# FrozenWolf-Cyber/Indic-CL-ASR

Measured on AMD Instinct MI355X. Metric: utterances/sec (15 s @16 kHz) Conformer-M RNNT-CTC+EWC train step, higher is better.
Workload: dtype bf16; 1 GPU; BASELINE configs[1]: Conformer-medium (d=256, 16L, H=640) hybrid RNNT-CTC + EWC, bs=32/GPU x 15 s, bf16 projections, freeze_encoder_till=12, 22x257 heads, fused_batch_size=4; global_batch=32, parallelism=dp1

## Files before the change

include/indicasr.h:

```cpp
#ifndef INDICASR_H
#define INDICASR_H

#include <stddef.h>
#include <stdint.h>

#ifdef __cplusplus
extern "C" {
#endif

typedef void* ia_stream_t;

enum ia_status {
    IA_OK = 0,
    IA_INVALID_VALUE = -1,
    IA_WORKSPACE_TOO_SMALL = -2,
    IA_LAUNCH_FAILED = -3,
    IA_UNSUPPORTED = -4,
};

const char* ia_version(void);

size_t ia_rnnt_workspace_bytes(int B, int T, int U1);
int ia_rnnt_loss(const float* logits, const int64_t* labels, const int64_t* act_lens, const int64_t* label_lens,
                 int B, int T, int U1, int V, int blank, float fastemit_lambda, float clamp,
// ... 76 lines not shown
int ia_quantize_mxfp8(const void* x, int is_f32, int ld, int64_t M, int K, void* q, int ldq, void* scales, int lds, ia_stream_t stream);
int ia_gemm_mxfp8(const void* Aq, int lda, const void* a_scales, int ldsa, const void* Wq, int ldw, const void* w_scales, int ldsw,
                  int M, int N, int K, const float* bias, int act, float dropout_p, unsigned seed, float alpha, const float* R, int ldr,
                  float* outF, int ldof, void* outH, int ldoh, ia_stream_t stream);

int ia_greedy_decode_lds_bytes(int Hp, int Hj, int V);
int ia_greedy_rnnt_decode(const float* f_all, const int64_t* out_len, const float* EW, const float* Whh, const float* Wpred,
                          const float* bpred, const float* Whead, const float* bhead, int B, int T, int Hp, int Hj, int V,
                          int blank, int row_blank, int row_sos, int max_symbols, int* tokens, int cap, int* counts,
                          int* overflow, ia_stream_t stream);
int ia_greedy_rnnt_decode_bf16w(const float* f_all, const int64_t* out_len, const float* EW, const void* Whh_bf16,
                                const void* Wpred_bf16, const float* bpred, const void* Whead_bf16, const float* bhead, int B, int T,
                                int Hp, int Hj, int V, int blank, int row_blank, int row_sos, int max_symbols, int* tokens, int cap,
                                int* counts, int* overflow, ia_stream_t stream);
size_t ia_greedy_decode_scratch_bytes(int B, int Hp, int Hj);
int ia_greedy_decode_cluster(int B, int Hp, int Hj);
int ia_greedy_rnnt_decode_bf16w_ex(const float* f_all, const int64_t* out_len, const float* EW, const void* Whh_bf16,
                                   const void* Wpred_bf16, const float* bpred, const void* Whead_bf16, const float* bhead, int B,
                                   int T, int Hp, int Hj, int V, int blank, int row_blank, int row_sos, int max_symbols, int* tokens,
                                   int cap, int* counts, int* overflow, int cluster, void* scratch, size_t scratch_bytes,
                                   ia_stream_t stream);

int ia_edit_distance_batch(const int32_t* a, const int64_t* a_off, const int32_t* b, const int64_t* b_off, int n, int64_t* out);

int ia_quantize_fp8_rows(const void* x, int is_f32, int ld, int64_t M, int K, void* q, int ldq, float* scale, ia_stream_t stream);
int ia_gemm_fp8(const void* Aq, int lda, const float* a_scale, const void* Wq, int ldw, const float* w_scale, int M, int N, int K,
                const float* bias, int act, float dropout_p, unsigned seed, float alpha, const float* R, int ldr, float* outF,
                int ldof, void* outH, int ldoh, ia_stream_t stream);
int ia_subsample_conv1(const float* feats, int B, int Fm, int Tm, int C, const float* w1, const float* b1, void* out,
                       ia_stream_t stream);
int ia_subsample_conv2(const void* in_cl, int B, int T1, int F1, int C, const void* w2r, const float* b2, int N, void* out,
                       ia_stream_t stream);
int ia_gemm_bf16_ln_supported(int N, int K);
int ia_gemm_bf16_ln(const void* A, int lda, const void* W, int ldw, int M, int N, int K, const float* bias, float dropout_p,
                    unsigned seed, float alpha, const float* R, int ldr, float* outF, int ldof, const float* ln_g,
                    const float* ln_b, float ln_eps, void* outH, int ldoh, ia_stream_t stream);
int ia_layernorm(const float* x, int ldx, int N, int d, const float* g1, const float* b1, float eps, float* outF,
                 int ldf, const float* g2, const float* b2, void* outH, int ldh, ia_stream_t stream);
int ia_glu_dwconv(const void* x2, const int64_t* lens, int B, int T, int d, int ksz, const float* w, const float* bias,
                  float* z, float* bn_sum, float* bn_sumsq, float* scratch, ia_stream_t stream);
int64_t ia_dwconv_scratch_elems(int B, int T, int d, int ksz);
int ia_colsum_bf16(const void* x, int M, int N, int ld, float* out, ia_stream_t stream);
int ia_dwconv_time(const float* x, int B, int T, int d, int ksz, const float* w, const float* bias, int flip, float* y,
                   ia_stream_t stream);
int ia_dwconv_time_wgrad(const float* x, const float* dy, int B, int T, int d, int ksz, float* dw, float* db,
                         float* scratch, ia_stream_t stream);
int ia_dwconv_glu_bwd(const float* dz, const void* c2, const int64_t* lens, int B, int T, int d, int ksz, const float* w, void* dc2,
                      ia_stream_t stream);
int ia_dwconv_glu_wgrad(const void* c2, const int64_t* lens, const float* dy, int B, int T, int d, int ksz, float* dw, float* db,
                        float* scratch, ia_stream_t stream);
int ia_bn_silu(const float* z, int64_t n_rows, int d, const float* bn_sum, const float* bn_sumsq, const float* gamma,
               const float* beta, float* running_mean, float* running_var, int64_t* num_batches_tracked,
               float momentum, float eps, int training, void* out, ia_stream_t stream);

int ia_gemm_bnsilu_supported(int K);
int ia_gemm_bnsilu_bf16(const float* z, int ldz, int64_t n_rows, const float* bn_sum, const float* bn_sumsq,
                        const float* gamma, const float* beta, float* running_mean, float* running_var,
                        int64_t* num_batches_tracked, float momentum, float eps, int training, const void* W, int ldw, int M,
                        int N, int K, const float* bias, float dropout_p, unsigned seed, float alpha, const float* R, int ldr,
                        float* outF, int ldof, void* outH, int ldoh, const long long* bn_sums_fixed, ia_stream_t stream);
int ia_gemm_bnsilu_bf16_keep(const float* z, int ldz, int64_t n_rows, const float* bn_sum, const float* bn_sumsq,
                             const float* gamma, const float* beta, float* running_mean, float* running_var,
                             int64_t* num_batches_tracked, float momentum, float eps, int training, const void* W, int ldw, int M,
                             int N, int K, const float* bias, float dropout_p, unsigned seed, float alpha, const float* R, int ldr,
                             float* outF, int ldof, void* outH, int ldoh, const long long* bn_sums_fixed, void* outA, int ldoa,
                             ia_stream_t stream);
int ia_dwconv_gated_fixed(const void* g, const int64_t* lens, int B, int T, int d, int ksz, const float* w, const float* bias,
                          float* z, long long* bn_sums_fixed, ia_stream_t stream);
int ia_glu_dwconv_fixed(const void* x2, const int64_t* lens, int B, int T, int d, int ksz, const float* w, const float* bias,
                        float* z, long long* bn_sums_fixed, ia_stream_t stream);

int ia_relpos_attention_flash_supported(int T, int dk);
int ia_relpos_attention_flash(const void* qkv, const void* pos_proj, const float* bias_u, const float* bias_v,
                              const int64_t* lens, int B, int T, int H, int dk, float dropout_p, unsigned seed, void* ctx,
                              ia_stream_t stream);
int ia_relpos_attention_flash_lse(const void* qkv, const void* pos_proj, const float* bias_u, const float* bias_v,
                                  const int64_t* lens, int B, int T, int H, int dk, float dropout_p, unsigned seed, void* ctx,
                                  float* lse, ia_stream_t stream);
int ia_relpos_attention_local_supported(int T, int dk, int window);
int ia_relpos_attention_local(const void* qkv, const void* pos_proj, const float* bias_u, const float* bias_v,
                              const int64_t* lens, int B, int T, int H, int dk, int window, float dropout_p, unsigned seed,
                              void* ctx, ia_stream_t stream);
int ia_relpos_attention_local_lse(const void* qkv, const void* pos_proj, const float* bias_u, const float* bias_v,
                                  const int64_t* lens, int B, int T, int H, int dk, int window, float dropout_p, unsigned seed,
                                  void* ctx, float* lse, ia_stream_t stream);
int ia_relpos_attention_flash_bwd_dims(int T, int* Rs, int* pad0);
int64_t ia_relpos_attention_flash_bwd_ws_elems(int B, int T, int H, int dk);
int ia_relpos_attention_flash_bwd(const void* qkv, const void* pos_proj, const float* bias_u, const float* bias_v,
                                  const int64_t* lens, const void* ctx, const void* dctx, const float* lse, int B, int T, int H,
                                  int dk, float dropout_p, unsigned seed, void* dqkv, void* dpl, int pl_rows, float* dbias_u,
                                  float* dbias_v, void* dBand, void* QvHM, float* ws, ia_stream_t stream);
int ia_relpos_attention_local_bwd_dims(int T, int window, int* Rs, int* pad0);
int64_t ia_relpos_attention_local_bwd_ws_elems(int B, int T, int H, int dk, int window);
int ia_relpos_attention_local_bwd(const void* qkv, const void* pos_proj, const float* bias_u, const float* bias_v,
                                  const int64_t* lens, const void* ctx, const void* dctx, const float* lse, int B, int T, int H,
                                  int dk, int window, float dropout_p, unsigned seed, void* dqkv, void* dpl, int pl_rows,
                                  float* dbias_u, float* dbias_v, void* dBand, void* QvHM, float* ws, ia_stream_t stream);
int ia_relpos_attention_context_supported(int T, int dk, int style, int left, int right);
int ia_relpos_attention_context(const void* qkv, const void* pos_proj, const float* bias_u, const float* bias_v,
                                const int64_t* lens, int B, int T, int H, int dk, int style, int left, int right,
                                float dropout_p, unsigned seed, void* ctx, ia_stream_t stream);
int ia_relpos_attention_context_lse(const void* qkv, const void* pos_proj, const float* bias_u, const float* bias_v,
                                    const int64_t* lens, int B, int T, int H, int dk, int style, int left, int right,
                                    float dropout_p, unsigned seed, void* ctx, float* lse, ia_stream_t stream);
int ia_relpos_attention_context_bwd_dims(int T, int style, int left, int right, int* Rs, int* pad0);
int64_t ia_relpos_attention_context_bwd_ws_elems(int B, int T, int H, int dk, int style, int left, int right);
int ia_relpos_attention_context_bwd(const void* qkv, const void* pos_proj, const float* bias_u, const float* bias_v,
                                    const int64_t* lens, const void* ctx, const void* dctx, const float* lse, int B, int T, int H,
                                    int dk, int style, int left, int right, float dropout_p, unsigned seed, void* dqkv, void* dpl,
                                    int pl_rows, float* dbias_u, float* dbias_v, void* dBand, void* QvHM, float* ws,
                                    ia_stream_t stream);
size_t ia_attn_vt_elems(int B, int T, int H);
int ia_relpos_attention(const void* qkv, const void* pos_proj, const float* bias_u, const float* bias_v,
                        const int64_t* lens, int B, int T, int H, int dk, float dropout_p, unsigned seed,
                        void* vt_scratch, void* ctx, ia_stream_t stream);

size_t ia_lstm_scratch_bytes(int B, int H);
int ia_lstm_lds_bytes(int H, int backward);
int ia_lstm_forward(const float* Gx, const void* Whh_bf16, float* Hout, float* gates, float* Cs, int U, int B, int H,
                    void* scratch, size_t scratch_bytes, ia_stream_t stream);
int ia_lstm_backward(const float* dHout, const float* gates, const float* Cs, const void* WhhT_bf16, float* dG, int U,
                     int B, int H, void* scratch, size_t scratch_bytes, ia_stream_t stream);

int ia_feat_frames(const float* audio, int B, int L, int Tm, int win, int n_fft, int hop, float preemph, float dither,
                   unsigned seed, float* frames, int ldf, ia_stream_t stream);
int ia_gemm_f32(const float* A, int lda, const float* W, int ldw, int M, int N, int K, float* C, int ldc,
                ia_stream_t stream);
int ia_feat_power(const float* spec, int64_t M, int lds, int half, int nbins, float* power, int ldp, ia_stream_t stream);
int ia_feat_logmel_t(const float* mel, int B, int Tm, int F, int ldm, float guard, float* out, ia_stream_t stream);
int ia_feat_preemph(const float* audio, int B, int L, float preemph, float dither, unsigned seed, float* y,
                    ia_stream_t stream);
int ia_feat_logmel_fft_supported(int n_fft, int win, int n_mels, int n_chunks);
int ia_feat_logmel_fft(const float* y, int B, int L, int Tm, const float* window, int win, int n_fft, int hop,
                       const float* twiddle, const int* chunk_start, const float* chunk_vals, const int* filt_chunks,
                       int n_mels, int n_chunks, float guard, float* out, ia_stream_t stream);
int ia_feat_normalize(const float* x, const int64_t* seq_len, int B, int F, int T, float eps, const int* freq_starts,
                      const int* freq_widths, int n_freq_masks, const int* time_starts, const int* time_widths,
                      int n_time_masks, float mask_value, float* y, ia_stream_t stream);

size_t ia_ctc_workspace_bytes(int B, int T, int S);
int ia_ctc_forward(const float* log_probs, const int64_t* targets, const int64_t* input_lens, const int64_t* target_lens,
                   int B, int T, int V, int S, int blank, int zero_infinity, float* nll, void* workspace,
                   size_t workspace_bytes, ia_stream_t stream);
int ia_ctc_backward(const float* log_probs, const int64_t* targets, const int64_t* input_lens, const int64_t* target_lens,
                    int B, int T, int V, int S, int blank, const float* nll_grad, float* grad, void* workspace,
                    size_t workspace_bytes, ia_stream_t stream);

typedef struct ia_tn_problem {
    const void* dY; const void* X; float* dW; float* db;
    int ldy, ldx, M, n, k;
} ia_tn_problem;
int64_t ia_gemm_tn_grouped_scratch_elems(const ia_tn_problem* problems, int count);
int ia_gemm_tn_bf16_grouped(const ia_tn_problem* problems, int count, float* scratch, ia_stream_t stream);
int64_t ia_gemm_tn_scratch_elems(int M, int n, int k);
int ia_gemm_tn_bf16(const void* dY, int ldy, const void* X, int ldx, int M, int n, int k, float* dW, float* db,
                    float* scratch, ia_stream_t stream);

int ia_ffn_fused_supported(int d, int d_ff);
int ia_ffn_fused(float* x, int N, int d, int d_ff, const float* ln_g, const float* ln_b, float eps, const void* W1,
                 const float* b1, const void* W2, const float* b2, float alpha, float p_ff, unsigned seed_ff, float p_res,
                 unsigned seed_res, const float* ln2_g, const float* ln2_b, void* y_out, int ln2_to_y_only,
                 ia_stream_t stream);
int ia_ffn_fused_tail_supported(int d, int d_ff, int nt);
int ia_ffn_fused_tail(float* x, int N, int d, int d_ff, const float* ln_g, const float* ln_b, float eps, const void* W1,
                      const float* b1, const void* W2, const float* b2, float alpha, float p_ff, unsigned seed_ff, float p_res,
                      unsigned seed_res, const float* ln2_g, const float* ln2_b, void* y_out, int ln2_to_y_only, const void* Wt,
                      const float* bt, void* t_out, int nt, ia_stream_t stream);

typedef struct ia_block_params {
    const void *w_ff1a, *w_ff1b, *w_qkv, *w_pos, *w_out, *w_pw1, *w_pw2, *w_ff2a, *w_ff2b;
    const float *b_ff1a, *b_ff1b, *b_qkv, *b_out, *b_pw1, *b_pw2, *b_ff2a, *b_ff2b;
    const float *ln_ff1_g, *ln_ff1_b, *ln_att_g, *ln_att_b, *ln_conv_g, *ln_conv_b, *ln_ff2_g, *ln_ff2_b, *ln_out_g, *ln_out_b;
    const float *pos_u, *pos_v, *dw_w, *dw_b, *bn_g, *bn_b;
    float *bn_rm, *bn_rv;
    int64_t* bn_nbt;
    float ln_eps, bn_eps, bn_momentum, p_drop, p_ff, p_att, fc_factor;
    int d, d_ff, n_heads, ksz;
    const void* pl_cached;
    const void* w_pw1_glu;
    const float* b_pw1_glu;
    int att_window;
    int att_style;
    int att_left, att_right;
} ia_block_params;
size_t ia_conformer_prefix_ws_bytes(int B, int T, int d, int d_ff, int H, int ksz, int pos_rows);
int ia_conformer_prefix_fwd(const ia_block_params* layers, int n_layers, float* x, const void* pos_emb, int pos_rows,
                            const int64_t* lens, int B, int T, unsigned seed_base, unsigned seed_stride, int training,
                            void* workspace, size_t workspace_bytes, ia_stream_t stream);
size_t ia_conformer_prefix_ws_sums_offset(int B, int T, int d, int d_ff, int H, int ksz, int pos_rows);
int ia_conformer_prefix_fwd_seg(const ia_block_params* layers, int n_layers, float* x, const void* pos_emb, int pos_rows,
                                const int64_t* lens, int B, int T, unsigned seed_base, unsigned seed_stride, int training,
                                int seg_begin, int seg_end, int bn_synced, void* workspace, size_t workspace_bytes,
                                ia_stream_t stream);

typedef struct ia_block_saved {
    void *y1, *h1p, *h1; float* x1;
    void *y2, *qkv, *pl, *ctxv; float* x2;
    void *y3, *c2; float *z, *sums; void* c3; float* x3;
    void *y4, *h4p, *h4; float* x4;
    float* lse;
} ia_block_saved;
typedef struct ia_block_grads {
    float *w_ff1a, *b_ff1a, *w_ff1b, *b_ff1b, *w_qkv, *b_qkv, *w_pos, *w_out, *b_out, *w_pw1, *b_pw1, *w_pw2, *b_pw2;
    float *w_ff2a, *b_ff2a, *w_ff2b, *b_ff2b;
    float *ln_ff1_g, *ln_ff1_b, *ln_att_g, *ln_att_b, *ln_conv_g, *ln_conv_b, *ln_ff2_g, *ln_ff2_b, *ln_out_g, *ln_out_b;
    float *dw_w, *dw_b, *bn_g, *bn_b;
} ia_block_grads;
struct ia_block_params;
int ia_conformer_block_supported(int d, int d_ff, int H, int ksz, int T);
size_t ia_conformer_block_bwd_ws_bytes(int B, int T, int d, int d_ff, int ksz);
int ia_conformer_block_fwd(const struct ia_block_params* layer, const float* x0, const void* pos_emb, int pos_rows,
                           const int64_t* lens, int B, int T, unsigned seed, const ia_block_saved* saved, float* out,
                           float* dw_scratch, ia_stream_t stream);
int ia_conformer_block_bwd_a(const struct ia_block_params* layer, const ia_block_saved* saved, const ia_block_grads* grads,
                             const float* dout, const int64_t* lens, int B, int T, unsigned seed, void* workspace,
                             size_t workspace_bytes, float** dx2_out, void** dctx_out, ia_stream_t stream);
int ia_conformer_block_fwd_phase(const struct ia_block_params* layer, const float* x0, const void* pos_emb, int pos_rows,
                                 const int64_t* lens, int B, int T, unsigned seed, const ia_block_saved* saved, float* out,
                                 float* dw_scratch, int phase, ia_stream_t stream);
int ia_conformer_block_bwd_a_phase(const struct ia_block_params* layer, const ia_block_saved* saved, const ia_block_grads* grads,
                                   const float* dout, const int64_t* lens, int B, int T, unsigned seed, void* workspace,
                                   size_t workspace_bytes, float** dx2_out, void** dctx_out, int phase, const float* bn_S12,
                                   ia_stream_t stream);
int ia_conformer_block_bwd_b(const struct ia_block_params* layer, const ia_block_saved* saved, const ia_block_grads* grads,
                             const float* x0, const void* pos_emb, int pos_rows, const void* dqkv, const void* dpl, int B,
                             int T, unsigned seed, void* workspace, size_t workspace_bytes, float* dx0,
                             const void* add_table, int n_add, ia_stream_t stream);

int ia_layernorm_bwd(const float* x, int ldx, const float* dy_f32, const void* dy_bf16, int ldy, int N, int d,
                     const float* gamma, float eps, const float* dx_in, float* dx_out, int lddx, float* dgamma,
                     float* dbeta, float* scratch, ia_stream_t stream);
int ia_layernorm_bwd_drop(const float* x, int ldx, const float* dy_f32, const void* dy_bf16, int ldy, int N, int d,
                          const float* gamma, float eps, const float* dx_in, float* dx_out, int lddx, float* dgamma,
                          float* dbeta, float alpha, float dropout_p, unsigned seed, void* dx_bf16, int lddxh, float* scratch,
                          ia_stream_t stream);
typedef struct ia_finish_job { const float* part; int G, C, C0; float* out0; float* out1; } ia_finish_job;
int ia_layernorm_bwd_partial_rows(int N);
int ia_partials_finish_multi(const ia_finish_job* jobs, int count, ia_stream_t stream);
int64_t ia_layernorm_bwd_scratch_elems(int N, int d);
int ia_silu_dropout(const void* h_pre, int64_t M, int N, float dropout_p, unsigned seed, void* out, ia_stream_t stream);
int ia_silu_dropout_bwd(const void* h_pre, const void* dh, int64_t M, int N, float dropout_p, unsigned seed, void* out,
                        ia_stream_t stream);
int ia_scale_dropout_bf16(const float* dy, int64_t M, int N, float alpha, float dropout_p, unsigned seed, void* out,
                          ia_stream_t stream);
int ia_cast_pad_bf16(const float* src, int lds, int64_t M, int N, void* dst, int ldd, ia_stream_t stream);
int ia_bn_silu_bwd(const float* z, const void* dc3, int64_t n_rows, int d, const float* bn_sum, const float* bn_sumsq,
                   const float* gamma, const float* beta, float eps, float* S1, float* S2, float* dz, float* scratch,
                   ia_stream_t stream);
int64_t ia_bn_silu_bwd_scratch_elems(int64_t n_rows, int d);
int ia_bn_sync_finish(float* sums_and_count, int d, int64_t n_local_rows, float* running_mean, float* running_var,
                      int64_t* num_batches_tracked, float momentum, ia_stream_t stream);
int ia_bn_silu_bwd_reduce(const float* z, const void* dc3, int64_t n_rows, int d, const float* bn_sum, const float* bn_sumsq,
                          const float* gamma, const float* beta, float eps, float* S1, float* S2, float* scratch,
                          ia_stream_t stream);
int ia_bn_silu_bwd_apply(const float* z, const void* dc3, int64_t n_rows, int d, const float* bn_sum, const float* bn_sumsq,
                         const float* gamma, const float* beta, float eps, const float* S1, const float* S2, float* dz,
                         ia_stream_t stream);
int ia_glu_mask(const void* c2, const int64_t* lens, int B, int T, int d, float* G, ia_stream_t stream);
int ia_glu_bwd(const void* c2, const float* dG, const int64_t* lens, int B, int T, int d, void* dc2, ia_stream_t stream);

int ia_cl_chunk_elems(void);
int ia_cl_penalty(const float* theta, const float* theta_star, const float* weight, float coef, float* grad,
                  int accumulate, const int32_t* chunk_table, int nchunks, const float* seg_inv_numel,
                  float* seg_abs_mean, float* penalty_sum, ia_stream_t stream);
int ia_cl_fisher_accumulate(float* fisher, const float* grad, const float* loss_scalar, int64_t n, ia_stream_t stream);
int ia_cl_abs_accumulate(float* omega, const float* grad, int64_t n, ia_stream_t stream);
int ia_adamw_step(float* theta, const float* grad, float* exp_avg, float* exp_avg_sq, int64_t n, float lr, float beta1,
                  float beta2, float eps, float weight_decay, int step, float grad_scale, void* shadow_bf16,
                  ia_stream_t stream);
int ia_adamw_step_segmented(float* theta, const float* grad, float* exp_avg, float* exp_avg_sq, const int32_t* chunk_table,
                            int nchunks, int32_t* seg_active, int32_t* seg_step, int nseg, int all_active, float lr,
                            float beta1, float beta2, float eps, float weight_decay, float grad_scale, void* shadow_bf16,
                            ia_stream_t stream);
size_t ia_grad_norm_workspace_bytes(int nchunks);
int ia_grad_norm(const float* grad, const int32_t* chunk_table, int nchunks, const int32_t* seg_chunk_begin, int nseg,
                 float grad_scale, float max_norm, int32_t* seg_active, float* seg_norm, float* norm_state, void* workspace,
                 size_t workspace_bytes, ia_stream_t stream);
int ia_adamw_step_segmented_clipped(float* theta, const float* grad, float* exp_avg, float* exp_avg_sq,
                                    const int32_t* chunk_table, int nchunks, int32_t* seg_active, int32_t* seg_step, int nseg,
                                    int all_active, float lr, float beta1, float beta2, float eps, float weight_decay,
                                    float grad_scale, void* shadow_bf16, const float* norm_state, int skip_nonfinite,
                                    int32_t* counters, ia_stream_t stream);
int ia_adamw_step_segmented_si(float* theta, const float* grad, float* exp_avg, float* exp_avg_sq, const int32_t* chunk_table,
                               int nchunks, int32_t* seg_active, int32_t* seg_step, int nseg, int all_active, float lr,
                               float beta1, float beta2, float eps, float weight_decay, float grad_scale, void* shadow_bf16,
                               const float* norm_state, int skip_nonfinite, int32_t* counters, float* path_w,
                               const float* omega, const float* theta_star, float penalty_coef, ia_stream_t stream);
int ia_si_consolidate(const float* theta, float* theta_star, float* path_w, float* omega, float xi, int64_t n,
                      ia_stream_t stream);
size_t ia_agem_workspace_bytes(int nchunks);
int ia_agem_dots(const float* grad, const float* ref, const int32_t* chunk_table, int nchunks, int nseg, float grad_scale,
                 int32_t* seg_active, float* proj_state, void* workspace, size_t workspace_bytes, ia_stream_t stream);
int ia_grad_norm_projected(const float* grad, const int32_t* chunk_table, int nchunks, const int32_t* seg_chunk_begin, int nseg,
                           float grad_scale, float max_norm, const int32_t* seg_active, float* seg_norm, float* norm_state,
                           void* workspace, size_t workspace_bytes, const float* ref, const float* proj_state,
                           ia_stream_t stream);
int ia_adamw_step_segmented_projected(float* theta, const float* grad, float* exp_avg, float* exp_avg_sq,
                                      const int32_t* chunk_table, int nchunks, int32_t* seg_active, int32_t* seg_step, int nseg,
                                      int all_active, float lr, float beta1, float beta2, float eps, float weight_decay,
                                      float grad_scale, void* shadow_bf16, const float* norm_state, int skip_nonfinite,
                                      int32_t* counters, const float* ref, const float* proj_state, int32_t* proj_counters,
                                      ia_stream_t stream);
#define IA_GEM_MAX_TASKS 16
#define IA_GEM_STATE_FLOATS 20
#define IA_GEM_SUMS_DOUBLES 272
size_t ia_gem_workspace_bytes(int nchunks, int max_tasks);
int ia_gem_dots(const float* x, const float* refs, int64_t stride, int ntasks, const int32_t* chunk_table, int nchunks, int nseg,
                float grad_scale, int32_t* seg_active, int gram_row, double* gem_sums, void* workspace, size_t workspace_bytes,
                ia_stream_t stream);
int ia_gem_solve(const double* gem_sums, float* gem_state, int ntasks, float memory_strength, float eps, ia_stream_t stream);
int ia_grad_norm_gem(const float* grad, const int32_t* chunk_table, int nchunks, const int32_t* seg_chunk_begin, int nseg,
                     float grad_scale, float max_norm, const int32_t* seg_active, float* seg_norm, float* norm_state,
                     void* workspace, size_t workspace_bytes, const float* refs, int64_t stride, int ntasks,
                     const float* gem_state, ia_stream_t stream);
int ia_adamw_step_segmented_gem(float* theta, const float* grad, float* exp_avg, float* exp_avg_sq, const int32_t* chunk_table,
                                int nchunks, int32_t* seg_active, int32_t* seg_step, int nseg, int all_active, float beta1,
                                float beta2, float eps, float grad_scale, void* shadow_bf16, const int32_t* seg_group, int ngroups,
                                const float* group_lr, const float* group_weight_decay, const float* norm_state,
                                int skip_nonfinite, int32_t* counters, const float* refs, int64_t stride, int ntasks,
                                const float* gem_state, int32_t* gem_counters, ia_stream_t stream);
#define IA_MAX_PARAM_GROUPS 64
int ia_adamw_step_segmented_grouped(float* theta, const float* grad, float* exp_avg, float* exp_avg_sq,
                                    const int32_t* chunk_table, int nchunks, int32_t* seg_active, int32_t* seg_step, int nseg,
                                    int all_active, float beta1, float beta2, float eps, float grad_scale, void* shadow_bf16,
                                    const int32_t* seg_group, int ngroups, const float* group_lr,
                                    const float* group_weight_decay, const float* norm_state, int skip_nonfinite,
                                    int32_t* counters, float* path_w, const float* omega, const float* theta_star,
                                    float penalty_coef, const float* ref, const float* proj_state, int32_t* proj_counters,
                                    ia_stream_t stream);
#define IA_MASK_FREE 0
#define IA_MASK_MASKED 1
#define IA_MASK_FROZEN 2
int ia_adamw_step_segmented_masked(float* theta, const float* grad, float* exp_avg, float* exp_avg_sq, const int32_t* chunk_table,
                                   int nchunks, int32_t* seg_active, int32_t* seg_step, int nseg, int all_active, float beta1,
                                   float beta2, float eps, float grad_scale, void* shadow_bf16, const int32_t* seg_group,
                                   int ngroups, const float* group_lr, const float* group_weight_decay, const float* norm_state,
                                   int skip_nonfinite, int32_t* counters, const float* base, float* scores,
                                   const int32_t* seg_kind, float threshold, ia_stream_t stream);
int ia_mask_pack(const float* scores, const int32_t* chunk_table, int nchunks, const int32_t* seg_kind, int nseg, float threshold,
                 uint64_t* bits, int64_t nwords, int32_t* seg_kept, ia_stream_t stream);
int ia_mask_apply(float* theta, const float* base, const uint64_t* bits, int64_t nwords, const int32_t* chunk_table, int nchunks,
                  const int32_t* seg_kind, int nseg, void* shadow_bf16, ia_stream_t stream);
int ia_adamw_step_segmented_packed(float* theta, const float* grad, float* exp_avg, float* exp_avg_sq, const int32_t* chunk_table,
                                   int nchunks, int32_t* seg_active, int32_t* seg_step, int nseg, int all_active, float beta1,
                                   float beta2, float eps, float grad_scale, void* shadow_bf16, const int32_t* seg_group,
                                   int ngroups, const float* group_lr, const float* group_weight_decay, const float* norm_state,
                                   int skip_nonfinite, int32_t* counters, const uint8_t* owner, const int32_t* seg_kind,
                                   int train_owner, ia_stream_t stream);
int ia_grad_norm_packed(const float* grad, const int32_t* chunk_table, int nchunks, const int32_t* seg_chunk_begin, int nseg,
                        float grad_scale, float max_norm, int32_t* seg_active, float* seg_norm, float* norm_state,
                        void* workspace, size_t workspace_bytes, const uint8_t* owner, const int32_t* seg_kind, int train_owner,
                        ia_stream_t stream);
size_t ia_pack_prune_workspace_bytes(int nseg);
int ia_pack_prune(float* theta, float* exp_avg, float* exp_avg_sq, uint8_t* owner, const int32_t* chunk_table, int nchunks,
                  const int32_t* seg_kind, int nseg, float fraction, int task, void* shadow_bf16, int32_t* seg_counts,
                  void* workspace, size_t workspace_bytes, ia_stream_t stream);
int ia_pack_apply(float* theta, const float* base, const uint8_t* owner, const int32_t* chunk_table, int nchunks,
                  const int32_t* seg_kind, int nseg, int lo, int hi, void* shadow_bf16, ia_stream_t stream);
#define IA_LORA_MAX_RANK 64
int ia_lora_tile_rows(void);
int ia_lora_tile_cols(void);
size_t ia_lora_workspace_bytes(int64_t m, int64_t n, int rank);
int ia_lora_grad(const float* grad, const float* factors, float* factor_grad, const int64_t* tensors, int ntensors,
                 const int32_t* tiles, int ntiles, const int32_t* factor_chunk_table, int nfchunks, int rank, float scale,
                 float grad_scale, const float* norm_state, int skip_nonfinite, int all_active, int32_t* factor_active,
                 void* workspace, size_t workspace_bytes, size_t workspace_needed, ia_stream_t stream);
int ia_lora_apply(float* theta, const float* base, const float* factors, const int64_t* tensors, int ntensors,
                  const int32_t* seg_tensor, const int32_t* chunk_table, int nchunks, int nseg, int rank, float scale,
                  void* shadow_bf16, const float* norm_state, int skip_nonfinite, ia_stream_t stream);
int ia_adamw_step_segmented_kinds(float* theta, const float* grad, float* exp_avg, float* exp_avg_sq, const int32_t* chunk_table,
                                  int nchunks, int32_t* seg_active, int32_t* seg_step, int nseg, int all_active, float beta1,
                                  float beta2, float eps, float grad_scale, void* shadow_bf16, const int32_t* seg_group,
                                  int ngroups, const float* group_lr, const float* group_weight_decay, const float* norm_state,
                                  int skip_nonfinite, int32_t* counters, const int32_t* seg_kind, int flags_preset,
                                  ia_stream_t stream);
#define IA_MERGE_MAX_TASKS 32
int ia_merge_linear(float* theta, const float* base, const float* vectors, int64_t stride, int ntasks, const float* coef,
                    float scale, const int32_t* chunk_table, int nchunks, void* shadow_bf16, ia_stream_t stream);
size_t ia_merge_trim_workspace_bytes(int ntasks, int nscope);
int ia_merge_trim(const float* vectors, int64_t stride, int ntasks, const int32_t* chunk_table, int nchunks,
// ... 70 lines not shown
```

indic_cl_asr_amd/_lib.py:

```python
import ctypes
import os
import subprocess

_HERE = os.path.dirname(os.path.abspath(__file__))
LIB_PATH = os.environ.get("IA_LIB_PATH") or os.path.join(_HERE, "libindicasr_hip.so")

IA_OK = 0
_STATUS = {-1: "IA_INVALID_VALUE", -2: "IA_WORKSPACE_TOO_SMALL", -3: "IA_LAUNCH_FAILED", -4: "IA_UNSUPPORTED"}

_c = ctypes
_vp, _i, _f, _sz = _c.c_void_p, _c.c_int, _c.c_float, _c.c_size_t
_i64 = _c.c_int64

class BlockParams(_c.Structure):
    _fields_ = ([(n, _c.c_void_p) for n in (
        "w_ff1a", "w_ff1b", "w_qkv", "w_pos", "w_out", "w_pw1", "w_pw2", "w_ff2a", "w_ff2b",
        "b_ff1a", "b_ff1b", "b_qkv", "b_out", "b_pw1", "b_pw2", "b_ff2a", "b_ff2b",
        "ln_ff1_g", "ln_ff1_b", "ln_att_g", "ln_att_b", "ln_conv_g", "ln_conv_b", "ln_ff2_g", "ln_ff2_b", "ln_out_g", "ln_out_b",
        "pos_u", "pos_v", "dw_w", "dw_b", "bn_g", "bn_b", "bn_rm", "bn_rv", "bn_nbt")]
        + [(n, _c.c_float) for n in ("ln_eps", "bn_eps", "bn_momentum", "p_drop", "p_ff", "p_att", "fc_factor")]
        + [(n, _c.c_int) for n in ("d", "d_ff", "n_heads", "ksz")]
        + [("pl_cached", _c.c_void_p), ("w_pw1_glu", _c.c_void_p), ("b_pw1_glu", _c.c_void_p), ("att_window", _c.c_int),
           ("att_style", _c.c_int), ("att_left", _c.c_int), ("att_right", _c.c_int)])


class BlockSaved(_c.Structure):
    _fields_ = [(n, _c.c_void_p) for n in ("y1", "h1p", "h1", "x1", "y2", "qkv", "pl", "ctxv", "x2", "y3", "c2", "z", "sums",
                                           "c3", "x3", "y4", "h4p", "h4", "x4", "lse")]


class TnProblem(_c.Structure):
    _fields_ = [("dY", _c.c_void_p), ("X", _c.c_void_p), ("dW", _c.c_void_p), ("db", _c.c_void_p),
                ("ldy", _c.c_int), ("ldx", _c.c_int), ("M", _c.c_int), ("n", _c.c_int), ("k", _c.c_int)]


class BlockGrads(_c.Structure):
    _fields_ = [(n, _c.c_void_p) for n in (
        "w_ff1a", "b_ff1a", "w_ff1b", "b_ff1b", "w_qkv", "b_qkv", "w_pos", "w_out", "b_out", "w_pw1", "b_pw1", "w_pw2", "b_pw2",
        "w_ff2a", "b_ff2a", "w_ff2b", "b_ff2b",
        "ln_ff1_g", "ln_ff1_b", "ln_att_g", "ln_att_b", "ln_conv_g", "ln_conv_b", "ln_ff2_g", "ln_ff2_b", "ln_out_g", "ln_out_b",
        "dw_w", "dw_b", "bn_g", "bn_b")]


class WaveParams(_c.Structure):
    _fields_ = ([(n, _c.c_int32) for n in ("n_in", "n_out", "new_sr", "shift_pre", "shift_post", "noise_shift", "noise_stage")]
                + [("noise_seed", _c.c_uint32), ("gain", _c.c_float), ("noise_amp", _c.c_float), ("pad", _c.c_int32 * 2)])


SIGNATURES = {
    "ia_version": (_c.c_char_p, []),
    "ia_wave_augment_tile": (_i, []),
    "ia_wave_augment": (_i, [_vp, _i, _i, _vp, _i, _vp, _vp, _i, _i, _i, _vp]),
    "ia_gemm_bf16_ex2": (_i, [_vp, _i, _vp, _i, _i, _i, _i, _vp, _i, _f, _c.c_uint, _f, _vp, _i, _vp, _i, _vp, _i, _vp, _i, _vp, _i, _i, _vp]),
    "ia_transpose16_multi": (_i, [_vp, _i, _vp]),
    "ia_swap01_cast": (_i, [_vp, _i, _i, _i, _i, _vp, _i, _vp]),
    "ia_ctc_row_lse": (_i, [_vp, _i, _i64, _i, _vp, _vp]),
    "ia_ctc_forward_logits": (_i, [_vp, _i, _vp, _vp, _vp, _vp, _i, _i, _i, _i, _i, _i, _vp, _vp, _sz, _vp]),
    "ia_ctc_backward_logits": (_i, [_vp, _i, _vp, _vp, _vp, _vp, _i, _i, _i, _i, _i, _vp, _f, _vp, _i, _vp, _sz, _vp]),
    "ia_select_rows_cast": (_i, [_vp, _i, _vp, _i, _i, _i, _i, _i, _f, _i, _vp, _vp, _i, _vp, _vp]),
    "ia_rows_scatter_add": (_i, [_vp, _i, _vp, _i, _i, _i, _i, _i, _f, _vp, _vp, _vp]),
    "ia_loss_combine": (_i, [_vp, _vp, _i, _f, _vp, _vp, _vp, _vp, _vp, _vp, _vp]),
    "ia_loss_combine_bwd": (_i, [_vp, _i, _f, _vp, _vp, _vp]),
    "ia_embed_sos": (_i, [_vp, _vp, _i, _i, _i, _i, _i, _i, _vp, _vp]),
    "ia_embed_sos_bwd": (_i, [_vp, _i, _vp, _i, _i, _i, _i, _i, _i, _f, _vp, _vp]),
    "ia_multi_axpy": (_i, [_vp, _i, _i, _vp]),
    "ia_peak_stream_copy": (_i, [_vp, _vp, _sz, _vp]),
    "ia_peak_mfma_bf16": (_i, [_vp, _i, _i, _vp]),
    "ia_peak_mfma_bf16_flops": (_c.c_double, [_i, _i]),
    "ia_rnnt_workspace_bytes": (_sz, [_i, _i, _i]),
    "ia_rnnt_loss": (_i, [_vp, _vp, _vp, _vp, _i, _i, _i, _i, _i, _f, _f, _vp, _vp, _vp, _sz, _vp]),
    "ia_rnnt_forward": (_i, [_vp, _vp, _vp, _vp, _i, _i, _i, _i, _i, _f, _i, _vp, _vp, _sz, _vp]),
    "ia_rnnt_backward": (_i, [_vp, _vp, _vp, _vp, _i, _i, _i, _i, _i, _f, _f, _vp, _vp, _vp, _sz, _vp, _vp, _vp]),
    "ia_rnnt_export_alphas_betas": (_i, [_vp, _sz, _vp, _vp, _i, _i, _i, _vp, _vp, _vp]),
    "ia_joint_ld": (_i, [_i]),
    "ia_joint_fwd": (_i, [_vp, _vp, _vp, _vp, _vp, _vp, _vp, _i, _i, _i, _i, _i, _i, _f, _c.c_uint, _vp, _i, _vp, _sz, _vp]),
    "ia_joint_fwd_box": (_i, [_vp, _vp, _vp, _vp, _vp, _vp, _vp, _vp, _vp, _i, _i, _i, _i, _i, _i, _f, _c.c_uint, _vp, _i, _vp, _sz, _vp]),
    "ia_joint_extra_scratch_elems": (_i64, []),
    "ia_joint_extra_reduce": (_i, [_vp, _vp, _vp, _vp, _vp, _vp, _i, _i, _i, _i, _i, _vp, _vp, _vp]),
    "ia_joint_extra_grad": (_i, [_vp, _vp, _vp, _vp, _vp, _vp, _vp, _i, _i, _i, _i, _i, _vp, _vp]),
    "ia_lattice_add_f16": (_i, [_vp, _vp, _i64, _vp]),
    "ia_relpos_attention_flash_lse": (_i, [_vp, _vp, _vp, _vp, _vp, _i, _i, _i, _i, _f, _c.c_uint, _vp, _vp, _vp]),
    "ia_relpos_attention_flash_bwd_dims": (_i, [_i, _c.POINTER(_c.c_int), _c.POINTER(_c.c_int)]),
    "ia_relpos_attention_flash_bwd_ws_elems": (_i64, [_i, _i, _i, _i]),
    "ia_relpos_attention_flash_bwd": (_i, [_vp, _vp, _vp, _vp, _vp, _vp, _vp, _vp, _i, _i, _i, _i, _f, _c.c_uint, _vp, _vp, _i, _vp,
                                           _vp, _vp, _vp, _vp, _vp]),
    "ia_relpos_attention_local_lse": (_i, [_vp, _vp, _vp, _vp, _vp, _i, _i, _i, _i, _i, _f, _c.c_uint, _vp, _vp, _vp]),
    "ia_relpos_attention_local_bwd_dims": (_i, [_i, _i, _c.POINTER(_c.c_int), _c.POINTER(_c.c_int)]),
    "ia_relpos_attention_local_bwd_ws_elems": (_i64, [_i, _i, _i, _i, _i]),
    "ia_relpos_attention_local_bwd": (_i, [_vp, _vp, _vp, _vp, _vp, _vp, _vp, _vp, _i, _i, _i, _i, _i, _f, _c.c_uint, _vp, _vp, _i, _vp,
                                           _vp, _vp, _vp, _vp, _vp]),
    "ia_relpos_attention_context_lse": (_i, [_vp, _vp, _vp, _vp, _vp, _i, _i, _i, _i, _i, _i, _i, _f, _c.c_uint, _vp, _vp, _vp]),
    "ia_relpos_attention_context_bwd_dims": (_i, [_i, _i, _i, _i, _c.POINTER(_c.c_int), _c.POINTER(_c.c_int)]),
    "ia_relpos_attention_context_bwd_ws_elems": (_i64, [_i, _i, _i, _i, _i, _i, _i]),
    "ia_relpos_attention_context_bwd": (_i, [_vp, _vp, _vp, _vp, _vp, _vp, _vp, _vp, _i, _i, _i, _i, _i, _i, _i, _f, _c.c_uint, _vp, _vp,
                                             _i, _vp, _vp, _vp, _vp, _vp, _vp]),
    "ia_quantize_fp8_rows": (_i, [_vp, _i, _i, _i64, _i, _vp, _i, _vp, _vp]),
    "ia_gemm_fp8": (_i, [_vp, _i, _vp, _vp, _i, _vp, _i, _i, _i, _vp, _i, _f, _c.c_uint, _f, _vp, _i, _vp, _i, _vp, _i, _vp]),
    "ia_gemm_tn_grouped_scratch_elems": (_i64, [_vp, _i]),
    "ia_gemm_tn_bf16_grouped": (_i, [_vp, _i, _vp, _vp]),
    "ia_greedy_decode_lds_bytes": (_i, [_i, _i, _i]),
    "ia_greedy_rnnt_decode": (_i, [_vp, _vp, _vp, _vp, _vp, _vp, _vp, _vp, _i, _i, _i, _i, _i, _i, _i, _i, _i, _vp, _i, _vp, _vp, _vp]),
    "ia_greedy_rnnt_decode_bf16w": (_i, [_vp, _vp, _vp, _vp, _vp, _vp, _vp, _vp, _i, _i, _i, _i, _i, _i, _i, _i, _i, _vp, _i, _vp, _vp, _vp]),
    "ia_edit_distance_batch": (_i, [_vp, _vp, _vp, _vp, _i, _vp]),
    "ia_greedy_decode_scratch_bytes": (_sz, [_i, _i, _i]),
    "ia_greedy_decode_cluster": (_i, [_i, _i, _i]),
    "ia_greedy_rnnt_decode_bf16w_ex": (_i, [_vp, _vp, _vp, _vp, _vp, _vp, _vp, _vp, _i, _i, _i, _i, _i, _i, _i, _i, _i, _vp, _i, _vp, _vp, _i, _vp, _sz, _vp]),
    "ia_quantize_mxfp8": (_i, [_vp, _i, _i, _i64, _i, _vp, _i, _vp, _i, _vp]),
    "ia_gemm_mxfp8": (_i, [_vp, _i, _vp, _i, _vp, _i, _vp, _i, _i, _i, _i, _vp, _i, _f, _c.c_uint, _f, _vp, _i, _vp, _i, _vp, _i, _vp]),
    "ia_cast_pad_bf16": (_i, [_vp, _i, _i64, _i, _vp, _i, _vp]),
    "ia_rnnt_lattice": (_i, [_vp, _vp, _i, _i, _i, _f, _i, _vp, _vp, _sz, _vp]),
    "ia_joint_backward_g": (_i, [_vp, _vp, _vp, _vp, _i, _i, _i, _i, _i, _i, _f, _vp, _f, _vp, _i, _i, _vp, _vp, _vp, _sz, _vp, _vp,
                                 _vp]),
    "ia_joint_backward_g_skip": (_i, [_vp, _vp, _vp, _vp, _i, _i, _i, _i, _i, _i, _f, _vp, _f, _vp, _i, _i, _vp, _vp, _vp, _sz, _i, _vp,
                                      _vp, _vp]),
    "ia_joint_backward_g_dbias_scratch_elems": (_i64, [_i]),
    "ia_joint_hidden_t": (_i, [_vp, _vp, _vp, _i, _i, _i, _i, _i, _i, _i, _f, _c.c_uint, _vp]),
    "ia_joint_hidden": (_i, [_vp, _vp, _vp, _i, _i, _i, _i, _i, _f, _c.c_uint, _vp]),
    "ia_joint_dh_reduce": (_i, [_vp, _vp, _vp, _vp, _vp, _vp, _vp, _i, _i, _i, _i, _f, _f, _c.c_uint, _vp, _vp]),
    "ia_joint_dh_reduce_scratch_bytes": (_sz, [_i, _i, _i, _i]),
    "ia_joint_dh_fused_supported": (_i, [_i, _i, _i]),
    "ia_joint_dh_k": (_i, []),
    "ia_joint_dh_fused": (_i, [_vp, _vp, _vp, _vp, _vp, _vp, _vp, _vp, _i, _i, _i, _i, _i, _f, _f, _c.c_uint, _vp, _vp]),
    "ia_joint_dh_fused_ex": (_i, [_vp, _vp, _vp, _vp, _vp, _vp, _vp, _vp, _vp, _vp, _i, _i, _i, _i, _i, _i, _f, _f, _c.c_uint, _vp, _vp]),
    "ia_joint_dh_fused_scratch_bytes": (_sz, [_i, _i, _i, _i]),
    "ia_joint_dw_fused_supported": (_i, [_i, _i, _i]),
    "ia_joint_dw_fused_scratch_elems": (_i64, [_i, _i, _i, _i, _i]),
    "ia_joint_dw_fused": (_i, [_vp, _vp, _vp, _vp, _i, _i, _i, _i, _i, _f, _c.c_uint, _vp, _vp, _vp]),
    "ia_gemm_bf16_ln_supported": (_i, [_i, _i]),
    "ia_gemm_bf16_ln": (_i, [_vp, _i, _vp, _i, _i, _i, _i, _vp, _f, _c.c_uint, _f, _vp, _i, _vp, _i, _vp, _vp, _f, _vp, _i, _vp]),
    "ia_joint_dw_fused_ex": (_i, [_vp, _vp, _vp, _vp, _vp, _i, _i, _i, _i, _i, _f, _c.c_uint, _vp, _vp, _vp]),
    "ia_gemm_bf16": (_i, [_vp, _i, _vp, _i, _i, _i, _i, _vp, _i, _f, _c.c_uint, _f, _vp, _i, _vp, _i, _vp, _i, _vp]),
    "ia_gemm_bf16_ex": (_i, [_vp, _i, _vp, _i, _i, _i, _i, _vp, _i, _f, _c.c_uint, _f, _vp, _i, _vp, _i, _vp, _i, _vp, _i, _vp, _i, _vp]),
    "ia_subsample_conv1": (_i, [_vp, _i, _i, _i, _i, _vp, _vp, _vp, _vp]),
    "ia_subsample_conv2": (_i, [_vp, _i, _i, _i, _i, _vp, _vp, _i, _vp, _vp]),
    "ia_layernorm": (_i, [_vp, _i, _i, _i, _vp, _vp, _f, _vp, _i, _vp, _vp, _vp, _i, _vp]),
    "ia_glu_dwconv": (_i, [_vp, _vp, _i, _i, _i, _i, _vp, _vp, _vp, _vp, _vp, _vp, _vp]),
    "ia_dwconv_scratch_elems": (_i64, [_i, _i, _i, _i]),
    "ia_colsum_bf16": (_i, [_vp, _i, _i, _i, _vp, _vp]),
    "ia_dwconv_time": (_i, [_vp, _i, _i, _i, _i, _vp, _vp, _i, _vp, _vp]),
    "ia_dwconv_time_wgrad": (_i, [_vp, _vp, _i, _i, _i, _i, _vp, _vp, _vp, _vp]),
    "ia_dwconv_glu_bwd": (_i, [_vp, _vp, _vp, _i, _i, _i, _i, _vp, _vp, _vp]),
    "ia_dwconv_glu_wgrad": (_i, [_vp, _vp, _vp, _i, _i, _i, _i, _vp, _vp, _vp, _vp]),
    "ia_bn_silu": (_i, [_vp, _i64, _i, _vp, _vp, _vp, _vp, _vp, _vp, _vp, _f, _f, _i, _vp, _vp]),
    "ia_gemm_bnsilu_supported": (_i, [_i]),
    "ia_gemm_bnsilu_bf16": (_i, [_vp, _i, _i64, _vp, _vp, _vp, _vp, _vp, _vp, _vp, _f, _f, _i, _vp, _i, _i, _i, _i, _vp, _f, _c.c_uint, _f,
                                 _vp, _i, _vp, _i, _vp, _i, _vp, _vp]),
    "ia_gemm_bnsilu_bf16_keep": (_i, [_vp, _i, _i64, _vp, _vp, _vp, _vp, _vp, _vp, _vp, _f, _f, _i, _vp, _i, _i, _i, _i, _vp, _f, _c.c_uint,
                                      _f, _vp, _i, _vp, _i, _vp, _i, _vp, _vp, _i, _vp]),
    "ia_glu_dwconv_fixed": (_i, [_vp, _vp, _i, _i, _i, _i, _vp, _vp, _vp, _vp, _vp]),
    "ia_dwconv_gated_fixed": (_i, [_vp, _vp, _i, _i, _i, _i, _vp, _vp, _vp, _vp, _vp]),
    "ia_attn_vt_elems": (_sz, [_i, _i, _i]),
    "ia_relpos_attention": (_i, [_vp, _vp, _vp, _vp, _vp, _i, _i, _i, _i, _f, _c.c_uint, _vp, _vp, _vp]),
    "ia_relpos_attention_flash_supported": (_i, [_i, _i]),
    "ia_relpos_attention_flash": (_i, [_vp, _vp, _vp, _vp, _vp, _i, _i, _i, _i, _f, _c.c_uint, _vp, _vp]),
    "ia_relpos_attention_local_supported": (_i, [_i, _i, _i]),
    "ia_relpos_attention_context_supported": (_i, [_i, _i, _i, _i, _i]),
    "ia_relpos_attention_context": (_i, [_vp, _vp, _vp, _vp, _vp, _i, _i, _i, _i, _i, _i, _i, _f, _c.c_uint, _vp, _vp]),
    "ia_relpos_attention_local": (_i, [_vp, _vp, _vp, _vp, _vp, _i, _i, _i, _i, _i, _f, _c.c_uint, _vp, _vp]),
    "ia_lstm_scratch_bytes": (_sz, [_i, _i]),
    "ia_lstm_lds_bytes": (_i, [_i, _i]),
    "ia_lstm_forward": (_i, [_vp, _vp, _vp, _vp, _vp, _i, _i, _i, _vp, _sz, _vp]),
    "ia_lstm_backward": (_i, [_vp, _vp, _vp, _vp, _vp, _i, _i, _i, _vp, _sz, _vp]),
    "ia_feat_frames": (_i, [_vp, _i, _i, _i, _i, _i, _i, _f, _f, _c.c_uint, _vp, _i, _vp]),
    "ia_gemm_f32": (_i, [_vp, _i, _vp, _i, _i, _i, _i, _vp, _i, _vp]),
    "ia_feat_power": (_i, [_vp, _i64, _i, _i, _i, _vp, _i, _vp]),
    "ia_feat_logmel_t": (_i, [_vp, _i, _i, _i, _i, _f, _vp, _vp]),
    "ia_feat_preemph": (_i, [_vp, _i, _i, _f, _f, _c.c_uint, _vp, _vp]),
    "ia_feat_logmel_fft_supported": (_i, [_i, _i, _i, _i]),
    "ia_feat_logmel_fft": (_i, [_vp, _i, _i, _i, _vp, _i, _i, _i, _vp, _vp, _vp, _vp, _i, _i, _f, _vp, _vp]),
    "ia_feat_normalize": (_i, [_vp, _vp, _i, _i, _i, _f, _vp, _vp, _i, _vp, _vp, _i, _f, _vp, _vp]),
    "ia_ctc_workspace_bytes": (_sz, [_i, _i, _i]),
    "ia_ctc_forward": (_i, [_vp, _vp, _vp, _vp, _i, _i, _i, _i, _i, _i, _vp, _vp, _sz, _vp]),
    "ia_ctc_backward": (_i, [_vp, _vp, _vp, _vp, _i, _i, _i, _i, _i, _vp, _vp, _vp, _sz, _vp]),
    "ia_ctc_align_max_targets": (_i, []),
    "ia_ctc_align_workspace_bytes": (_sz, [_i, _i, _i]),
    "ia_ctc_align": (_i, [_vp, _i, _vp, _vp, _vp, _vp, _i, _i, _i, _i, _i, _vp, _vp, _vp, _vp, _sz, _vp]),
    "ia_gemm_tn_scratch_elems": (_i64, [_i, _i, _i]),
    "ia_gemm_tn_bf16": (_i, [_vp, _i, _vp, _i, _i, _i, _i, _vp, _vp, _vp, _vp]),
    "ia_ffn_fused_supported": (_i, [_i, _i]),
    "ia_ffn_fused": (_i, [_vp, _i, _i, _i, _vp, _vp, _f, _vp, _vp, _vp, _vp, _f, _f, _c.c_uint, _f, _c.c_uint, _vp, _vp, _vp, _i, _vp]),
    "ia_ffn_fused_tail_supported": (_i, [_i, _i, _i]),
    "ia_ffn_fused_tail": (_i, [_vp, _i, _i, _i, _vp, _vp, _f, _vp, _vp, _vp, _vp, _f, _f, _c.c_uint, _f, _c.c_uint, _vp, _vp, _vp, _i,
                               _vp, _vp, _vp, _i, _vp]),
    "ia_conformer_prefix_ws_bytes": (_sz, [_i, _i, _i, _i, _i, _i, _i]),
    "ia_conformer_prefix_ws_sums_offset": (_sz, [_i, _i, _i, _i, _i, _i, _i]),
    "ia_conformer_prefix_fwd_seg": (_i, [_vp, _i, _vp, _vp, _i, _vp, _i, _i, _c.c_uint, _c.c_uint, _i, _i, _i, _i, _vp, _sz, _vp]),
    "ia_conformer_prefix_fwd": (_i, [_vp, _i, _vp, _vp, _i, _vp, _i, _i, _c.c_uint, _c.c_uint, _i, _vp, _sz, _vp]),
    "ia_conformer_block_supported": (_i, [_i, _i, _i, _i, _i]),
    "ia_conformer_block_bwd_ws_bytes": (_sz, [_i, _i, _i, _i, _i]),
    "ia_conformer_block_fwd": (_i, [_vp, _vp, _vp, _i, _vp, _i, _i, _c.c_uint, _vp, _vp, _vp, _vp]),
    "ia_conformer_block_fwd_phase": (_i, [_vp, _vp, _vp, _i, _vp, _i, _i, _c.c_uint, _vp, _vp, _vp, _i, _vp]),
    "ia_conformer_block_bwd_a": (_i, [_vp, _vp, _vp, _vp, _vp, _i, _i, _c.c_uint, _vp, _sz, _vp, _vp, _vp]),
    "ia_conformer_block_bwd_a_phase": (_i, [_vp, _vp, _vp, _vp, _vp, _i, _i, _c.c_uint, _vp, _sz, _vp, _vp, _i, _vp, _vp]),
    "ia_conformer_block_bwd_b": (_i, [_vp, _vp, _vp, _vp, _vp, _i, _vp, _vp, _i, _i, _c.c_uint, _vp, _sz, _vp, _vp, _i, _vp]),
    "ia_layernorm_bwd": (_i, [_vp, _i, _vp, _vp, _i, _i, _i, _vp, _f, _vp, _vp, _i, _vp, _vp, _vp, _vp]),
    "ia_layernorm_bwd_drop": (_i, [_vp, _i, _vp, _vp, _i, _i, _i, _vp, _f, _vp, _vp, _i, _vp, _vp, _f, _f, _c.c_uint, _vp, _i, _vp, _vp]),
    "ia_layernorm_bwd_partial_rows": (_i, [_i]),
    "ia_partials_finish_multi": (_i, [_vp, _i, _vp]),
    "ia_layernorm_bwd_scratch_elems": (_i64, [_i, _i]),
    "ia_silu_dropout": (_i, [_vp, _i64, _i, _f, _c.c_uint, _vp, _vp]),
    "ia_silu_dropout_bwd": (_i, [_vp, _vp, _i64, _i, _f, _c.c_uint, _vp, _vp]),
    "ia_scale_dropout_bf16": (_i, [_vp, _i64, _i, _f, _f, _c.c_uint, _vp, _vp]),
    "ia_bn_silu_bwd": (_i, [_vp, _vp, _i64, _i, _vp, _vp, _vp, _vp, _f, _vp, _vp, _vp, _vp, _vp]),
    "ia_bn_silu_bwd_scratch_elems": (_i64, [_i64, _i]),
    "ia_bn_sync_finish": (_i, [_vp, _i, _i64, _vp, _vp, _vp, _f, _vp]),
    "ia_bn_silu_bwd_reduce": (_i, [_vp, _vp, _i64, _i, _vp, _vp, _vp, _vp, _f, _vp, _vp, _vp, _vp]),
    "ia_bn_silu_bwd_apply": (_i, [_vp, _vp, _i64, _i, _vp, _vp, _vp, _vp, _f, _vp, _vp, _vp, _vp]),
    "ia_glu_mask": (_i, [_vp, _vp, _i, _i, _i, _vp, _vp]),
    "ia_glu_bwd": (_i, [_vp, _vp, _vp, _i, _i, _i, _vp, _vp]),
    "ia_cl_chunk_elems": (_i, []),
    "ia_cl_penalty": (_i, [_vp, _vp, _vp, _f, _vp, _i, _vp, _i, _vp, _vp, _vp, _vp]),
    "ia_cl_fisher_accumulate": (_i, [_vp, _vp, _vp, _i64, _vp]),
    "ia_cl_abs_accumulate": (_i, [_vp, _vp, _i64, _vp]),
    "ia_adamw_step": (_i, [_vp, _vp, _vp, _vp, _i64, _f, _f, _f, _f, _f, _i, _f, _vp, _vp]),
    "ia_adamw_step_segmented": (_i, [_vp, _vp, _vp, _vp, _vp, _i, _vp, _vp, _i, _i, _f, _f, _f, _f, _f, _f, _vp, _vp]),
    "ia_grad_norm_workspace_bytes": (_sz, [_i]),
    "ia_grad_norm": (_i, [_vp, _vp, _i, _vp, _i, _f, _f, _vp, _vp, _vp, _vp, _sz, _vp]),
    "ia_adamw_step_segmented_clipped": (_i, [_vp, _vp, _vp, _vp, _vp, _i, _vp, _vp, _i, _i, _f, _f, _f, _f, _f, _f, _vp, _vp, _i,
                                             _vp, _vp]),
    "ia_adamw_step_segmented_si": (_i, [_vp, _vp, _vp, _vp, _vp, _i, _vp, _vp, _i, _i, _f, _f, _f, _f, _f, _f, _vp, _vp, _i,
                                        _vp, _vp, _vp, _vp, _f, _vp]),
    "ia_si_consolidate": (_i, [_vp, _vp, _vp, _vp, _f, _i64, _vp]),
    "ia_agem_workspace_bytes": (_sz, [_i]),
    "ia_agem_dots": (_i, [_vp, _vp, _vp, _i, _i, _f, _vp, _vp, _vp, _sz, _vp]),
    "ia_grad_norm_projected": (_i, [_vp, _vp, _i, _vp, _i, _f, _f, _vp, _vp, _vp, _vp, _sz, _vp, _vp, _vp]),
    "ia_adamw_step_segmented_projected": (_i, [_vp, _vp, _vp, _vp, _vp, _i, _vp, _vp, _i, _i, _f, _f, _f, _f, _f, _f, _vp, _vp, _i,
                                               _vp, _vp, _vp, _vp, _vp]),
    "ia_gem_workspace_bytes": (_sz, [_i, _i]),
    "ia_gem_dots": (_i, [_vp, _vp, _i64, _i, _vp, _i, _i, _f, _vp, _i, _vp, _vp, _sz, _vp]),
    "ia_gem_solve": (_i, [_vp, _vp, _i, _f, _f, _vp]),
    "ia_grad_norm_gem": (_i, [_vp, _vp, _i, _vp, _i, _f, _f, _vp, _vp, _vp, _vp, _sz, _vp, _i64, _i, _vp, _vp]),
    "ia_adamw_step_segmented_gem": (_i, [_vp, _vp, _vp, _vp, _vp, _i, _vp, _vp, _i, _i, _f, _f, _f, _f, _vp, _vp, _i, _vp, _vp,
                                         _vp, _i, _vp, _vp, _i64, _i, _vp, _vp, _vp]),
    "ia_adamw_step_segmented_grouped": (_i, [_vp, _vp, _vp, _vp, _vp, _i, _vp, _vp, _i, _i, _f, _f, _f, _f, _vp, _vp, _i, _vp, _vp,
                                             _vp, _i, _vp, _vp, _vp, _vp, _f, _vp, _vp, _vp, _vp]),
    "ia_adamw_step_segmented_masked": (_i, [_vp, _vp, _vp, _vp, _vp, _i, _vp, _vp, _i, _i, _f, _f, _f, _f, _vp, _vp, _i, _vp, _vp,
                                            _vp, _i, _vp, _vp, _vp, _vp, _f, _vp]),
    "ia_mask_pack": (_i, [_vp, _vp, _i, _vp, _i, _f, _vp, _i64, _vp, _vp]),
    "ia_mask_apply": (_i, [_vp, _vp, _vp, _i64, _vp, _i, _vp, _i, _vp, _vp]),
    "ia_adamw_step_segmented_packed": (_i, [_vp, _vp, _vp, _vp, _vp, _i, _vp, _vp, _i, _i, _f, _f, _f, _f, _vp, _vp, _i, _vp, _vp,
                                            _vp, _i, _vp, _vp, _vp, _i, _vp]),
    "ia_grad_norm_packed": (_i, [_vp, _vp, _i, _vp, _i, _f, _f, _vp, _vp, _vp, _vp, _sz, _vp, _vp, _i, _vp]),
    "ia_pack_prune_workspace_bytes": (_sz, [_i]),
    "ia_pack_prune": (_i, [_vp, _vp, _vp, _vp, _vp, _i, _vp, _i, _f, _i, _vp, _vp, _vp, _sz, _vp]),
    "ia_pack_apply": (_i, [_vp, _vp, _vp, _vp, _i, _vp, _i, _i, _i, _vp, _vp]),
    "ia_lora_tile_rows": (_i, []),
    "ia_lora_tile_cols": (_i, []),
    "ia_lora_workspace_bytes": (_sz, [_i64, _i64, _i]),
    "ia_lora_grad": (_i, [_vp, _vp, _vp, _vp, _i, _vp, _i, _vp, _i, _i, _f, _f, _vp, _i, _i, _vp, _vp, _sz, _sz, _vp]),
    "ia_lora_apply": (_i, [_vp, _vp, _vp, _vp, _i, _vp, _vp, _i, _i, _i, _f, _vp, _vp, _i, _vp]),
    "ia_adamw_step_segmented_kinds": (_i, [_vp, _vp, _vp, _vp, _vp, _i, _vp, _vp, _i, _i, _f, _f, _f, _f, _vp, _vp, _i, _vp, _vp,
                                           _vp, _i, _vp, _vp, _i, _vp]),
    "ia_merge_linear": (_i, [_vp, _vp, _vp, _i64, _i, _vp, _f, _vp, _i, _vp, _vp]),
    "ia_merge_trim_workspace_bytes": (_sz, [_i, _i]),
    "ia_merge_trim": (_i, [_vp, _i64, _i, _vp, _i, _vp, _i, _f, _vp, _vp, _sz, _vp]),
    "ia_merge_ties": (_i, [_vp, _vp, _vp, _i64, _i, _vp, _vp, _i, _f, _vp, _i, _i, _vp, _vp, _vp]),
    "ia_merge_fisher": (_i, [_vp, _vp, _vp, _vp, _i64, _i, _vp, _f, _f, _vp, _i, _i, _vp, _vp, _vp]),
    "ia_merge_linear_dare": (_i, [_vp, _vp, _vp, _i64, _i, _vp, _f, _vp, _i, _vp, _c.c_uint32, _c.c_uint32, _f, _vp]),
    "ia_merge_ties_dare": (_i, [_vp, _vp, _vp, _i64, _i, _f, _vp, _i, _i, _vp, _vp, _c.c_uint32, _c.c_uint32, _f, _vp]),
}

_lib = None


def build(verbose=False):
    out = None if verbose else subprocess.DEVNULL
    subprocess.check_call(["make", "-C", os.path.join(_HERE, "csrc")], stdout=out)


def lib():
    global _lib
    if _lib is None:
        if not os.path.exists(LIB_PATH):
            raise RuntimeError(
                f"{LIB_PATH} is missing: the HIP extension is the product path and has no fallback. "
                "Build it with `python -c 'import __graft_entry__ as g; g.build()'` or `make -C indic_cl_asr_amd/csrc`.")
        import torch
        l = ctypes.CDLL(LIB_PATH)
        for name, (res, args) in SIGNATURES.items():
            fn = getattr(l, name)
            fn.restype, fn.argtypes = res, args
        _lib = l
    return _lib


def check(status, what):
    if status != IA_OK:
        raise RuntimeError(f"{what} failed with status {status} ({_STATUS.get(status, 'unknown')})")


def version():
    return lib().ia_version().decode()


def stream_ptr():
    import torch
    return ctypes.c_void_p(torch.cuda.current_stream().cuda_stream)


def ptr(t):
    return ctypes.c_void_p(t.data_ptr()) if t is not None else None
```

indic_cl_asr_amd/csrc/block_train.hip:

```cpp
#include <hip/hip_bf16.h>
#include <hip/hip_runtime.h>

#include <cstdint>

#include <cstdlib>

#include "ia_common.h"

namespace {

inline size_t up256(size_t x) { return (x + 255) / 256 * 256; }

#define IA_TRY(call)                  \
    do {                              \
        const int rc_ = (call);       \
        if (rc_ != IA_OK) return rc_; \
    } while (0)

__global__ __launch_bounds__(256) void transpose_bf16_kernel(const unsigned short* __restrict__ in, int rows, int cols,
                                                             unsigned short* __restrict__ out) {
    __shared__ unsigned short tile[64][72];
    const int tiles_c = (cols + 63) / 64;
    const int tr = blockIdx.x / tiles_c, tc = blockIdx.x - tr * tiles_c;
    const int r0 = tr * 64, c0 = tc * 64;
    for (int i = threadIdx.x; i < 64 * 8; i += 256) {
        const int r = i >> 3, v = i & 7;
        uint4 x = make_uint4(0, 0, 0, 0);
        if (r0 + r < rows && c0 + v * 8 < cols) x = *reinterpret_cast<const uint4*>(in + (size_t)(r0 + r) * cols + c0 + v * 8);
        *reinterpret_cast<uint4*>(&tile[r][v * 8]) = x;
    }
    __syncthreads();
    for (int i = threadIdx.x; i < 64 * 8; i += 256) {
        const int c = i >> 3, v = i & 7;
        if (c0 + c < cols && r0 + v * 8 < rows) {
            union { uint4 u; unsigned short h[8]; } o;
#pragma unroll
            for (int j = 0; j < 8; ++j) o.h[j] = tile[v * 8 + j][c];
            *reinterpret_cast<uint4*>(out + (size_t)(c0 + c) * rows + r0 + v * 8) = o.u;
        }
    }
}

int transpose_bf16(const void* in, int rows, int cols, void* out, hipStream_t st) {
    if (rows % 8 != 0 || cols % 8 != 0) return IA_UNSUPPORTED;
    const int grid = ((rows + 63) / 64) * ((cols + 63) / 64);
    hipLaunchKernelGGL(transpose_bf16_kernel, dim3(grid), dim3(256), 0, st, (const unsigned short*)in, rows, cols, (unsigned short*)out);
    IA_RETURN_IF_LAUNCH_FAILED();
    return IA_OK;
}

struct TrJob { const unsigned short* in; unsigned short* out; int rows, cols, tile_begin, tiles_c; };
struct TrJobs { TrJob j[8]; int count; };
__global__ __launch_bounds__(256) void transpose_bf16_multi_kernel(TrJobs jobs) {
    __shared__ unsigned short tile[64][72];
    int ji = 0;
#pragma unroll
    for (int i = 1; i < 8; ++i)
        if (i < jobs.count && (int)blockIdx.x >= jobs.j[i].tile_begin) ji = i;
    const TrJob& J = jobs.j[ji];
    const int local = blockIdx.x - J.tile_begin;
    const int tr = local / J.tiles_c, tc = local - tr * J.tiles_c;
    const int r0 = tr * 64, c0 = tc * 64, rows = J.rows, cols = J.cols;
    for (int i = threadIdx.x; i < 64 * 8; i += 256) {
        const int r = i >> 3, v = i & 7;
        uint4 x = make_uint4(0, 0, 0, 0);
        if (r0 + r < rows && c0 + v * 8 < cols) x = *reinterpret_cast<const uint4*>(J.in + (size_t)(r0 + r) * cols + c0 + v * 8);
        *reinterpret_cast<uint4*>(&tile[r][v * 8]) = x;
    }
    __syncthreads();
    for (int i = threadIdx.x; i < 64 * 8; i += 256) {
        const int c = i >> 3, v = i & 7;
        if (c0 + c < cols && r0 + v * 8 < rows) {
            union { uint4 u; unsigned short h[8]; } o;
#pragma unroll
            for (int j = 0; j < 8; ++j) o.h[j] = tile[v * 8 + j][c];
            *reinterpret_cast<uint4*>(J.out + (size_t)(c0 + c) * rows + r0 + v * 8) = o.u;
        }
    }
}
struct TrList { TrJobs jobs; int tiles; };
inline void tr_add(TrList* l, const void* in, int rows, int cols, void* out) {
    TrJob& J = l->jobs.j[l->jobs.count++];
    J.in = (const unsigned short*)in; J.out = (unsigned short*)out; J.rows = rows; J.cols = cols;
    J.tile_begin = l->tiles; J.tiles_c = (cols + 63) / 64;
    l->tiles += ((rows + 63) / 64) * J.tiles_c;
}
int tr_launch(const TrList& l, hipStream_t st) {
    for (int i = 0; i < l.jobs.count; ++i)
        if (l.jobs.j[i].rows % 8 != 0 || l.jobs.j[i].cols % 8 != 0) return IA_UNSUPPORTED;
    hipLaunchKernelGGL(transpose_bf16_multi_kernel, dim3(l.tiles), dim3(256), 0, st, l.jobs);
    IA_RETURN_IF_LAUNCH_FAILED();
    return IA_OK;
}

struct AddRow { float* dst; const float* src; int64_t n; };
__global__ __launch_bounds__(256) void multi_add_kernel(const AddRow* __restrict__ table, int rows) {
    for (int k = blockIdx.y; k < rows; k += gridDim.y) {
        const AddRow r = table[k];
        const int64_t n4 = ((reinterpret_cast<uintptr_t>(r.dst) | reinterpret_cast<uintptr_t>(r.src)) & 15) ? 0 : (r.n >> 2);
        for (int64_t i = (int64_t)blockIdx.x * 256 + threadIdx.x; i < n4; i += (int64_t)gridDim.x * 256) {
            float4 a = reinterpret_cast<float4*>(r.dst)[i];
            const float4 b = reinterpret_cast<const float4*>(r.src)[i];
            a.x += b.x; a.y += b.y; a.z += b.z; a.w += b.w;
            reinterpret_cast<float4*>(r.dst)[i] = a;
        }
        for (int64_t i = (n4 << 2) + (int64_t)blockIdx.x * 256 + threadIdx.x; i < r.n; i += (int64_t)gridDim.x * 256) r.dst[i] += r.src[i];
    }
}

struct BwdWs {
    size_t dxa, dxb, dB, dB1, dB2, dB3, dh, dhp, dy, dc3, dz, dG, dc2, dctx, wt, scr, total;
};

size_t max3(size_t a, size_t b, size_t c) { return a > b ? (a > c ? a : c) : (b > c ? b : c); }

BwdWs bwd_ws(int B, int T, int d, int d_ff, int ksz) {
    const size_t N = (size_t)B * T;
    BwdWs w;
    size_t o = 0;
    w.dxa = o;  o = up256(o + N * d * 4);
    w.dxb = o;  o = up256(o + N * d * 4);
    w.dB = o;   o = up256(o + N * d * 2);
    w.dB1 = o;  o = up256(o + N * d * 2);
    w.dB2 = o;  o = up256(o + N * d * 2);
    w.dB3 = o;  o = up256(o + N * d * 2);
    w.dh = o;   o = up256(o + N * d_ff * 2);
    w.dhp = o;  o = up256(o + N * d_ff * 2);
    w.dy = o;   o = up256(o + N * d * 2);
    w.dc3 = o;  o = up256(o + N * d * 2);
    w.dz = o;   o = up256(o + N * d * 4);
    w.dG = o;   o = up256(o + (size_t)5 * (size_t)ia_layernorm_bwd_scratch_elems((int)N, d) * 4);
    w.dc2 = o;  o = up256(o + N * 2 * d * 2);
    w.dctx = o; o = up256(o + N * d * 2);
    w.wt = o;   o = up256(o + ((size_t)4 * d_ff * d + (size_t)7 * d * d) * 2);
    size_t scr = (size_t)ia_layernorm_bwd_scratch_elems((int)N, d);
    const int shapes[5][2] = {{d, d_ff}, {d_ff, d}, {d, d}, {2 * d, d}, {3 * d, d}};
    for (int i = 0; i < 5; ++i) {
        const size_t e = (size_t)ia_gemm_tn_scratch_elems((int)N, shapes[i][0], shapes[i][1]);
        scr = e > scr ? e : scr;
    }
    scr = max3(scr, (size_t)ia_bn_silu_bwd_scratch_elems((int64_t)N, d), (size_t)ia_dwconv_scratch_elems(B, T, d, ksz));
    {
        const ia_tn_problem ga[5] = {{nullptr, nullptr, nullptr, nullptr, d, d_ff, (int)N, d, d_ff},
                                     {nullptr, nullptr, nullptr, nullptr, d_ff, d, (int)N, d_ff, d},
                                     {nullptr, nullptr, nullptr, nullptr, d, d, (int)N, d, d},
                                     {nullptr, nullptr, nullptr, nullptr, 2 * d, d, (int)N, 2 * d, d},
                                     {nullptr, nullptr, nullptr, nullptr, d, d, (int)N, d, d}};
        const ia_tn_problem gb[4] = {{nullptr, nullptr, nullptr, nullptr, 3 * d, d, (int)N, 3 * d, d},
                                     {nullptr, nullptr, nullptr, nullptr, d, d, (int)(N > (size_t)64 * 512 ? N : (size_t)64 * 512), d, d},
                                     {nullptr, nullptr, nullptr, nullptr, d, d_ff, (int)N, d, d_ff},
                                     {nullptr, nullptr, nullptr, nullptr, d_ff, d, (int)N, d_ff, d}};
        scr = max3(scr, (size_t)ia_gemm_tn_grouped_scratch_elems(ga, 5), (size_t)ia_gemm_tn_grouped_scratch_elems(gb, 4));
        scr = max3(scr, (size_t)ia_gemm_tn_grouped_scratch_elems(gb, 2), (size_t)ia_gemm_tn_grouped_scratch_elems(gb + 2, 2));
        ia_tn_problem gall[9];
        for (int i = 0; i < 5; ++i) gall[i] = ga[i];
        for (int i = 0; i < 4; ++i) gall[5 + i] = gb[i];
        scr = scr > (size_t)ia_gemm_tn_grouped_scratch_elems(gall, 9) ? scr : (size_t)ia_gemm_tn_grouped_scratch_elems(gall, 9);
    }
    w.scr = o;  o = up256(o + scr * 4);
    w.total = o;
    return w;
}

int linear_bwd(const void* dY, const void* X, const void* W, int M, int n, int k, void* dX, float* dW, float* db, void* wt,
               float* scr, ia_stream_t stream) {
    if (dX) {
        IA_TRY(transpose_bf16(W, n, k, wt, (hipStream_t)stream));
        IA_TRY(ia_gemm_bf16(dY, n, wt, n, M, k, n, nullptr, 0, 0.f, 0, 1.f, nullptr, 0, nullptr, 0, dX, k, stream));
    }
    return ia_gemm_tn_bf16(dY, n, X, k, M, n, k, dW, db, scr, stream);
}

bool tn_grouping_enabled() {
    static const bool on = [] { const char* e = getenv("IA_TN_GROUPED"); return !(e && e[0] == '0'); }();
    return on;
}
int flush_group(const ia_tn_problem* grp, int ngrp, float* scr, ia_stream_t stream) {
    if (tn_grouping_enabled()) return ia_gemm_tn_bf16_grouped(grp, ngrp, scr, stream);
    for (int i = 0; i < ngrp; ++i)
        IA_TRY(ia_gemm_tn_bf16(grp[i].dY, grp[i].ldy, grp[i].X, grp[i].ldx, grp[i].M, grp[i].n, grp[i].k, grp[i].dW, grp[i].db, scr, stream));
    return IA_OK;
}
int linear_bwd_deferred(const void* dY, const void* X, const void* W, int M, int n, int k, void* dX, float* dW, float* db, const void* wt,
                        ia_tn_problem* grp, int* ngrp, ia_stream_t stream) {
    (void)W;
    if (dX) IA_TRY(ia_gemm_bf16(dY, n, wt, n, M, k, n, nullptr, 0, 0.f, 0, 1.f, nullptr, 0, nullptr, 0, dX, k, stream));
    grp[*ngrp] = ia_tn_problem{dY, X, dW, db, n, k, M, n, k};
    ++*ngrp;
    return IA_OK;
}

struct SideCtx {
    hipStream_t s = nullptr;
    hipEvent_t ev[8] = {};
    bool ok = false, tried = false;
    bool a_pending = false;
};
SideCtx* side_ctx() {
    static SideCtx ctx[16];
    const char* e = getenv("IA_WGRAD_SIDE");
    if (!(e && e[0] == '1')) return nullptr;
    int dev = 0;
    if (hipGetDevice(&dev) != hipSuccess || dev < 0 || dev >= 16) return nullptr;
    SideCtx& c = ctx[dev];
    if (!c.tried) {
        c.tried = true;
        bool ok = hipStreamCreateWithFlags(&c.s, hipStreamNonBlocking) == hipSuccess;
        for (int i = 0; ok && i < 8; ++i) ok = hipEventCreateWithFlags(&c.ev[i], hipEventDisableTiming) == hipSuccess;
        c.ok = ok;
    }
    return c.ok ? &c : nullptr;
}
struct PendingGroup { ia_tn_problem grp[8]; int n = 0; const void* ws = nullptr; };
PendingGroup* pending_group() {
    static PendingGroup pg[16];
    int dev = 0;
    if (hipGetDevice(&dev) != hipSuccess || dev < 0 || dev >= 16) return nullptr;
    return &pg[dev];
}
bool merged_wgrads() {
    const char* e = getenv("IA_TN_MERGE");
    return !(e && e[0] == '0') && tn_grouping_enabled();
}

int stream_after(hipStream_t from, hipStream_t to, hipEvent_t ev) {
    if (hipEventRecord(ev, from) != hipSuccess || hipStreamWaitEvent(to, ev, 0) != hipSuccess) return IA_LAUNCH_FAILED;
    return IA_OK;
}

}

extern "C" size_t ia_conformer_block_bwd_ws_bytes(int B, int T, int d, int d_ff, int ksz) {
    if (B <= 0 || T <= 0 || d <= 0 || d_ff <= 0 || ksz <= 0) return 0;
    return bwd_ws(B, T, d, d_ff, ksz).total;
}

extern "C" int ia_conformer_block_supported(int d, int d_ff, int H, int ksz, int T) {
    if (d <= 0 || H <= 0 || d % H != 0) return 0;
    const int dk = d / H;
    return (d % 8 == 0 && d <= 1024 && d_ff % 8 == 0 && ksz <= 31 && (ksz & 1) == 1 && dk <= 64 && dk % 4 == 0 && T >= 1) ? 1 : 0;
}

extern "C" int ia_conformer_block_fwd(const ia_block_params* Lp, const float* x0, const void* pos_emb, int pos_rows,
                                      const int64_t* lens, int B, int T, unsigned seed, const ia_block_saved* Sp, float* out,
                                      float* dw_scratch, ia_stream_t stream) {
    return ia_conformer_block_fwd_phase(Lp, x0, pos_emb, pos_rows, lens, B, T, seed, Sp, out, dw_scratch, 0, stream);
}

extern "C" int ia_conformer_block_fwd_phase(const ia_block_params* Lp, const float* x0, const void* pos_emb, int pos_rows,
                                            const int64_t* lens, int B, int T, unsigned seed, const ia_block_saved* Sp,
                                            float* out, float* dw_scratch, int phase, ia_stream_t stream) {
    if (phase < 0 || phase > 2) return IA_INVALID_VALUE;
    if (!Lp || !x0 || !pos_emb || !lens || !Sp || !out || !dw_scratch || B <= 0 || T <= 0) return IA_INVALID_VALUE;
    const ia_block_params& L = *Lp;
    const ia_block_saved& S = *Sp;
    const int d = L.d, d_ff = L.d_ff, H = L.n_heads, dk = d / (H > 0 ? H : 1), ksz = L.ksz, N = B * T;
    if (!ia_conformer_block_supported(d, d_ff, H, ksz, T) || pos_rows < 2 * T - 1 || L.att_window != 0 || L.att_style != 0) return IA_UNSUPPORTED;
    const float p = L.p_drop, pff = L.p_ff, patt = L.p_att;
    if (phase != 2) {
    IA_TRY(ia_layernorm(x0, d, N, d, L.ln_ff1_g, L.ln_ff1_b, L.ln_eps, nullptr, 0, nullptr, nullptr, S.y1, d, stream));
    IA_TRY(ia_gemm_bf16_ex(S.y1, d, L.w_ff1a, d, N, d_ff, d, L.b_ff1a, 1, pff, seed + 1, 1.f, nullptr, 0, nullptr, 0, S.h1, d_ff,
                           S.h1p, d_ff, nullptr, 0, stream));
    IA_TRY(ia_gemm_bf16(S.h1, d_ff, L.w_ff1b, d_ff, N, d, d_ff, L.b_ff1b, 0, p, seed + 2, L.fc_factor, x0, d, S.x1, d, nullptr, 0, stream));
    IA_TRY(ia_layernorm(S.x1, d, N, d, L.ln_att_g, L.ln_att_b, L.ln_eps, nullptr, 0, nullptr, nullptr, S.y2, d, stream));
    IA_TRY(ia_gemm_bf16(S.y2, d, L.w_qkv, d, N, 3 * d, d, L.b_qkv, 0, 0.f, 0, 1.f, nullptr, 0, nullptr, 0, S.qkv, 3 * d, stream));
    IA_TRY(ia_gemm_bf16(pos_emb, d, L.w_pos, d, pos_rows, d, d, nullptr, 0, 0.f, 0, 1.f, nullptr, 0, nullptr, 0, S.pl, d, stream));
    IA_TRY(ia_relpos_attention_flash_lse(S.qkv, S.pl, L.pos_u, L.pos_v, lens, B, T, H, dk, patt, seed + 7, S.ctxv, S.lse, stream));
    IA_TRY(ia_gemm_bf16(S.ctxv, d, L.w_out, d, N, d, d, L.b_out, 0, p, seed + 3, 1.f, S.x1, d, S.x2, d, nullptr, 0, stream));
    IA_TRY(ia_layernorm(S.x2, d, N, d, L.ln_conv_g, L.ln_conv_b, L.ln_eps, nullptr, 0, nullptr, nullptr, S.y3, d, stream));
    IA_TRY(ia_gemm_bf16(S.y3, d, L.w_pw1, d, N, 2 * d, d, L.b_pw1, 0, 0.f, 0, 1.f, nullptr, 0, nullptr, 0, S.c2, 2 * d, stream));
    IA_TRY(ia_glu_dwconv(S.c2, lens, B, T, d, ksz, L.dw_w, L.dw_b, S.z, S.sums, S.sums + d, dw_scratch, stream));
    }
    if (phase == 1) return IA_OK;
    const bool synced = phase == 2;
    if (ia_gemm_bnsilu_supported(d)) {
        IA_TRY(ia_gemm_bnsilu_bf16_keep(S.z, d, N, S.sums, S.sums + d, L.bn_g, L.bn_b, synced ? nullptr : L.bn_rm,
                                        synced ? nullptr : L.bn_rv, synced ? nullptr : L.bn_nbt, L.bn_momentum, L.bn_eps, 1, L.w_pw2,
                                        d, N, d, d, L.b_pw2, p, seed + 4, 1.f, S.x2, d, S.x3, d, nullptr, 0, nullptr, S.c3, d, stream));
    } else {
        IA_TRY(ia_bn_silu(S.z, N, d, S.sums, S.sums + d, L.bn_g, L.bn_b, synced ? nullptr : L.bn_rm, synced ? nullptr : L.bn_rv,
                          synced ? nullptr : L.bn_nbt, L.bn_momentum, L.bn_eps, 1, S.c3, stream));
        IA_TRY(ia_gemm_bf16(S.c3, d, L.w_pw2, d, N, d, d, L.b_pw2, 0, p, seed + 4, 1.f, S.x2, d, S.x3, d, nullptr, 0, stream));
    }
    IA_TRY(ia_layernorm(S.x3, d, N, d, L.ln_ff2_g, L.ln_ff2_b, L.ln_eps, nullptr, 0, nullptr, nullptr, S.y4, d, stream));
    IA_TRY(ia_gemm_bf16_ex(S.y4, d, L.w_ff2a, d, N, d_ff, d, L.b_ff2a, 1, pff, seed + 5, 1.f, nullptr, 0, nullptr, 0, S.h4, d_ff,
                           S.h4p, d_ff, nullptr, 0, stream));
    IA_TRY(ia_gemm_bf16(S.h4, d_ff, L.w_ff2b, d_ff, N, d, d_ff, L.b_ff2b, 0, p, seed + 6, L.fc_factor, S.x3, d, S.x4, d, nullptr, 0, stream));
    return ia_layernorm(S.x4, d, N, d, L.ln_out_g, L.ln_out_b, L.ln_eps, out, d, nullptr, nullptr, nullptr, 0, stream);
}

extern "C" int ia_conformer_block_bwd_a(const ia_block_params* Lp, const ia_block_saved* Sp, const ia_block_grads* Gp,
                                        const float* dout, const int64_t* lens, int B, int T, unsigned seed, void* workspace,
                                        size_t workspace_bytes, float** dx2_out, void** dctx_out, ia_stream_t stream) {
    return ia_conformer_block_bwd_a_phase(Lp, Sp, Gp, dout, lens, B, T, seed, workspace, workspace_bytes, dx2_out, dctx_out, 0, nullptr,
                                          stream);
}

extern "C" int ia_conformer_block_bwd_a_phase(const ia_block_params* Lp, const ia_block_saved* Sp, const ia_block_grads* Gp,
                                              const float* dout, const int64_t* lens, int B, int T, unsigned seed,
                                              void* workspace, size_t workspace_bytes, float** dx2_out, void** dctx_out,
                                              int phase, const float* bn_S12, ia_stream_t stream) {
    if (phase < 0 || phase > 2 || (phase == 2 && !bn_S12)) return IA_INVALID_VALUE;
    if (!Lp || !Sp || !Gp || !dout || !lens || !workspace || !dx2_out || !dctx_out || B <= 0 || T <= 0) return IA_INVALID_VALUE;
    const ia_block_params& L = *Lp;
    const ia_block_saved& S = *Sp;
    const ia_block_grads& G = *Gp;
    const int d = L.d, d_ff = L.d_ff, ksz = L.ksz, N = B * T;
    const BwdWs w = bwd_ws(B, T, d, d_ff, ksz);
    if (workspace_bytes < w.total) return IA_WORKSPACE_TOO_SMALL;
    char* ws = (char*)workspace;
    float *dxa = (float*)(ws + w.dxa), *dxb = (float*)(ws + w.dxb), *dz = (float*)(ws + w.dz), *scr = (float*)(ws + w.scr);
    float* lnp = (float*)(ws + w.dG);
    const size_t lnp_set = (size_t)ia_layernorm_bwd_scratch_elems(N, d);
    void *dB = ws + w.dB, *dB1 = ws + w.dB1, *dB2 = ws + w.dB2, *dhp = ws + w.dhp, *dy = ws + w.dy, *dc3 = ws + w.dc3, *dc2 = ws + w.dc2,
         *dctx = ws + w.dctx, *wt = ws + w.wt;
    const float p = L.p_drop, pff = L.p_ff;
    ia_tn_problem grp[8];
    int ngrp = 0;
    char* wtb = (char*)wt;
    void *wt_ff2b = wtb, *wt_ff2a = wtb + (size_t)d * d_ff * 2, *wt_pw2 = wtb + (size_t)2 * d * d_ff * 2,
         *wt_pw1 = wtb + ((size_t)2 * d * d_ff + (size_t)d * d) * 2, *wt_out = wtb + ((size_t)2 * d * d_ff + (size_t)3 * d * d) * 2;
    if (phase != 2) {
        TrList tl{};
        tr_add(&tl, L.w_ff2b, d, d_ff, wt_ff2b); tr_add(&tl, L.w_ff2a, d_ff, d, wt_ff2a); tr_add(&tl, L.w_pw2, d, d, wt_pw2);
        tr_add(&tl, L.w_pw1, 2 * d, d, wt_pw1); tr_add(&tl, L.w_out, d, d, wt_out);
        IA_TRY(tr_launch(tl, (hipStream_t)stream));
    }
    if (phase != 2) {
    IA_TRY(ia_layernorm_bwd_drop(S.x4, d, dout, nullptr, d, N, d, L.ln_out_g, L.ln_eps, nullptr, dxa, d, nullptr, nullptr,
                                 L.fc_factor, p, seed + 6, dB, d, lnp + 0 * lnp_set, stream));
    IA_TRY(ia_gemm_bf16_ex(dB, d, wt_ff2b, d, N, d_ff, d, nullptr, 3, pff, seed + 5, 1.f, nullptr, 0, nullptr, 0, dhp, d_ff, nullptr, 0,
                           S.h4p, d_ff, stream));
    IA_TRY(linear_bwd_deferred(dB, S.h4, L.w_ff2b, N, d, d_ff, nullptr, G.w_ff2b, G.b_ff2b, wt_ff2b, grp, &ngrp, stream));
    IA_TRY(linear_bwd_deferred(dhp, S.y4, L.w_ff2a, N, d_ff, d, dy, G.w_ff2a, G.b_ff2a, wt_ff2a, grp, &ngrp, stream));
    IA_TRY(ia_layernorm_bwd_drop(S.x3, d, nullptr, dy, d, N, d, L.ln_ff2_g, L.ln_eps, dxa, dxb, d, nullptr, nullptr, 1.f, p,
                                 seed + 4, dB1, d, lnp + 1 * lnp_set, stream));
    IA_TRY(linear_bwd_deferred(dB1, S.c3, L.w_pw2, N, d, d, dc3, G.w_pw2, G.b_pw2, wt_pw2, grp, &ngrp, stream));
    if (phase == 0)
        IA_TRY(ia_bn_silu_bwd(S.z, dc3, N, d, S.sums, S.sums + d, L.bn_g, L.bn_b, L.bn_eps, G.bn_b, G.bn_g, dz, scr, stream));
    else
        IA_TRY(ia_bn_silu_bwd_reduce(S.z, dc3, N, d, S.sums, S.sums + d, L.bn_g, L.bn_b, L.bn_eps, G.bn_b, G.bn_g, scr, stream));
    }
    if (phase == 1) {
        IA_TRY(flush_group(grp, ngrp, scr, stream));
        return IA_OK;
    }
    if (phase == 2)
        IA_TRY(ia_bn_silu_bwd_apply(S.z, dc3, N, d, S.sums, S.sums + d, L.bn_g, L.bn_b, L.bn_eps, bn_S12, bn_S12 + d, dz, stream));
    IA_TRY(ia_dwconv_glu_bwd(dz, S.c2, lens, B, T, d, ksz, L.dw_w, dc2, stream));
    SideCtx* side = phase == 0 ? side_ctx() : nullptr;
    hipStream_t main = (hipStream_t)stream;
    if (side) {
        IA_TRY(stream_after(main, side->s, side->ev[0]));
        IA_TRY(ia_dwconv_glu_wgrad(S.c2, lens, dz, B, T, d, ksz, G.dw_w, G.dw_b, scr, (ia_stream_t)side->s));
    } else {
        IA_TRY(ia_dwconv_glu_wgrad(S.c2, lens, dz, B, T, d, ksz, G.dw_w, G.dw_b, scr, stream));
    }
    IA_TRY(linear_bwd_deferred(dc2, S.y3, L.w_pw1, N, 2 * d, d, dy, G.w_pw1, G.b_pw1, wt_pw1, grp, &ngrp, stream));
    IA_TRY(ia_layernorm_bwd_drop(S.x2, d, nullptr, dy, d, N, d, L.ln_conv_g, L.ln_eps, dxb, dxa, d, nullptr, nullptr, 1.f, p,
                                 seed + 3, dB2, d, lnp + 2 * lnp_set, stream));
    IA_TRY(linear_bwd_deferred(dB2, S.ctxv, L.w_out, N, d, d, dctx, G.w_out, G.b_out, wt_out, grp, &ngrp, stream));
    if (side) {
        IA_TRY(stream_after(main, side->s, side->ev[1]));
        IA_TRY(flush_group(grp, ngrp, scr, (ia_stream_t)side->s));
        if (hipEventRecord(side->ev[2], side->s) != hipSuccess) return IA_LAUNCH_FAILED;
        side->a_pending = true;
    } else if (phase == 0 && merged_wgrads() && pending_group()) {
        PendingGroup* pg = pending_group();
        for (int i = 0; i < ngrp; ++i) pg->grp[i] = grp[i];
        pg->n = ngrp; pg->ws = workspace;
    } else {
        IA_TRY(flush_group(grp, ngrp, scr, stream));
    }
    *dx2_out = dxa;
    *dctx_out = dctx;
    return IA_OK;
}

extern "C" int ia_conformer_block_bwd_b(const ia_block_params* Lp, const ia_block_saved* Sp, const ia_block_grads* Gp,
                                        const float* x0, const void* pos_emb, int pos_rows, const void* dqkv, const void* dpl,
                                        int B, int T, unsigned seed, void* workspace, size_t workspace_bytes, float* dx0,
                                        const void* add_table, int n_add, ia_stream_t stream) {
    if (!Lp || !Sp || !Gp || !x0 || !pos_emb || !dqkv || !dpl || !workspace || !dx0 || B <= 0 || T <= 0) return IA_INVALID_VALUE;
    const ia_block_params& L = *Lp;
    const ia_block_saved& S = *Sp;
    const ia_block_grads& G = *Gp;
    const int d = L.d, d_ff = L.d_ff, ksz = L.ksz, N = B * T;
    const BwdWs w = bwd_ws(B, T, d, d_ff, ksz);
    if (workspace_bytes < w.total) return IA_WORKSPACE_TOO_SMALL;
    char* ws = (char*)workspace;
    float *dxa = (float*)(ws + w.dxa), *dxb = (float*)(ws + w.dxb), *scr = (float*)(ws + w.scr);
    float* lnp = (float*)(ws + w.dG);
    const size_t lnp_set = (size_t)ia_layernorm_bwd_scratch_elems(N, d);
    PendingGroup* pg = pending_group();
    const bool carried = pg && pg->n > 0 && pg->ws == workspace;
    void *dB = ws + (carried ? w.dB3 : w.dB), *dhp = ws + (carried ? w.dh : w.dhp), *dy = ws + w.dy, *wt = ws + w.wt;
    const float p = L.p_drop, pff = L.p_ff;
    ia_tn_problem grp[12];
    int ngrp = 0;
    if (carried) {
        for (int i = 0; i < pg->n; ++i) grp[ngrp++] = pg->grp[i];
        pg->n = 0;
    }
    char* wtb = (char*)wt + ((size_t)2 * d * d_ff + (size_t)4 * d * d) * 2;
    void *wt_qkv = wtb, *wt_ff1b = wtb + (size_t)3 * d * d * 2, *wt_ff1a = wtb + ((size_t)3 * d * d + (size_t)d * d_ff) * 2;
    {
        TrList tl{};
        tr_add(&tl, L.w_qkv, 3 * d, d, wt_qkv); tr_add(&tl, L.w_ff1b, d, d_ff, wt_ff1b); tr_add(&tl, L.w_ff1a, d_ff, d, wt_ff1a);
        IA_TRY(tr_launch(tl, (hipStream_t)stream));
    }
    SideCtx* side = carried ? nullptr : side_ctx();
    hipStream_t main = (hipStream_t)stream;
    IA_TRY(linear_bwd_deferred(dqkv, S.y2, L.w_qkv, N, 3 * d, d, dy, G.w_qkv, G.b_qkv, wt_qkv, grp, &ngrp, stream));
    grp[ngrp++] = ia_tn_problem{dpl, pos_emb, G.w_pos, nullptr, d, d, pos_rows, d, d};
    if (side) {
        IA_TRY(stream_after(main, side->s, side->ev[3]));
        IA_TRY(flush_group(grp, ngrp, scr, (ia_stream_t)side->s));
        ngrp = 0;
        if (side->a_pending) {
            if (hipStreamWaitEvent(main, side->ev[2], 0) != hipSuccess) return IA_LAUNCH_FAILED;
            side->a_pending = false;
        }
    }
    IA_TRY(ia_layernorm_bwd_drop(S.x1, d, nullptr, dy, d, N, d, L.ln_att_g, L.ln_eps, dxa, dxb, d, nullptr, nullptr, L.fc_factor,
                                 p, seed + 2, dB, d, lnp + 3 * lnp_set, stream));
    IA_TRY(ia_gemm_bf16_ex(dB, d, wt_ff1b, d, N, d_ff, d, nullptr, 3, pff, seed + 1, 1.f, nullptr, 0, nullptr, 0, dhp, d_ff, nullptr, 0,
                           S.h1p, d_ff, stream));
    IA_TRY(linear_bwd_deferred(dB, S.h1, L.w_ff1b, N, d, d_ff, nullptr, G.w_ff1b, G.b_ff1b, wt_ff1b, grp, &ngrp, stream));
    if (side) {
        grp[ngrp++] = ia_tn_problem{dhp, S.y1, G.w_ff1a, G.b_ff1a, d_ff, d, N, d_ff, d};
        IA_TRY(stream_after(main, side->s, side->ev[4]));
        IA_TRY(flush_group(grp, ngrp, scr, (ia_stream_t)side->s));
        ngrp = 0;
        IA_TRY(ia_gemm_bf16(dhp, d_ff, wt_ff1a, d_ff, N, d, d_ff, nullptr, 0, 0.f, 0, 1.f, nullptr, 0, nullptr, 0, dy, d, stream));
    } else {
        IA_TRY(linear_bwd_deferred(dhp, S.y1, L.w_ff1a, N, d_ff, d, dy, G.w_ff1a, G.b_ff1a, wt_ff1a, grp, &ngrp, stream));
    }
    IA_TRY(ia_layernorm_bwd(x0, d, nullptr, dy, d, N, d, L.ln_ff1_g, L.ln_eps, dxb, dx0, d, nullptr, nullptr, lnp + 4 * lnp_set, stream));
    if (side) {
        IA_TRY(stream_after(main, side->s, side->ev[5]));
        stream = (ia_stream_t)side->s;
    } else {
        IA_TRY(flush_group(grp, ngrp, scr, stream));
    }
    {
        const int rows = ia_layernorm_bwd_partial_rows(N);
        const ia_finish_job jobs[5] = {{lnp + 0 * lnp_set, rows, 2 * d, d, G.ln_out_g, G.ln_out_b},
                                       {lnp + 1 * lnp_set, rows, 2 * d, d, G.ln_ff2_g, G.ln_ff2_b},
                                       {lnp + 2 * lnp_set, rows, 2 * d, d, G.ln_conv_g, G.ln_conv_b},
                                       {lnp + 3 * lnp_set, rows, 2 * d, d, G.ln_att_g, G.ln_att_b},
                                       {lnp + 4 * lnp_set, rows, 2 * d, d, G.ln_ff1_g, G.ln_ff1_b}};
        IA_TRY(ia_partials_finish_multi(jobs, 5, stream));
    }
    if (add_table && n_add > 0) {
        hipLaunchKernelGGL(multi_add_kernel, dim3(64, n_add < 64 ? n_add : 64), dim3(256), 0, (hipStream_t)stream,
                           (const AddRow*)add_table, n_add);
        IA_RETURN_IF_LAUNCH_FAILED();
    }
    if (side) IA_TRY(stream_after(side->s, main, side->ev[6]));
    return IA_OK;
}
```

indic_cl_asr_amd/csrc/gemm_tn.hip:

```cpp
#include <hip/hip_bf16.h>

#include "ia_common.h"
#include "lds_transpose.h"
#include "partials.h"

namespace {

typedef __bf16 bf8 __attribute__((ext_vector_type(8)));
typedef __bf16 bf4 __attribute__((ext_vector_type(4)));
typedef float f4 __attribute__((ext_vector_type(4)));

constexpr int TN_BN = 128;
constexpr int TN_BK = 128;
constexpr int TN_MS = 64;
constexpr int TN_ROWB = 256;
constexpr int TN_TILE = TN_MS * TN_ROWB;


__device__ __forceinline__ bool tn_map(int local, int tiles, int S, int* tile, int* split) {
    const int xcd = local & 7, slot = local >> 3;
    if (S >= 8) {
        *split = (slot / tiles) * 8 + xcd; *tile = slot % tiles;
        return *split < S;
    }
// ... 18 lines not shown
                                             int n, int k, int rows_per_split, float* __restrict__ part,
                                             float* __restrict__ part_b, size_t row_stride, int tile, int split,
                                             unsigned char* smem) {
    unsigned char* sY = smem;
    unsigned char* sX = smem + TN_TILE;
    const unsigned ldsY = (unsigned)(size_t)((__attribute__((address_space(3))) unsigned char*)sY);
    const unsigned ldsX = ldsY + TN_TILE;
    const int tid = threadIdx.x, lane = tid & 63, wave = tid >> 6;
    const int c = lane & 15, q4 = lane >> 4;
    const int wn = wave >> 1, wk = wave & 1;
    const int ntk = (k + TN_BK - 1) / TN_BK;
    const int n0 = (tile / ntk) * TN_BN, k0 = (tile % ntk) * TN_BK;
    const int m_beg = split * rows_per_split;
    int m_end = m_beg + rows_per_split; m_end = m_end < M ? m_end : M;
    const bool do_bias = part_b != nullptr && k0 == 0 && wk == 0;

    f4 acc[4][4], accb[4];
#pragma unroll
    for (int i = 0; i < 4; ++i) {
        accb[i] = (f4){0.f, 0.f, 0.f, 0.f};
#pragma unroll
        for (int j = 0; j < 4; ++j) acc[i][j] = (f4){0.f, 0.f, 0.f, 0.f};
    }
    bf8 ones;
#pragma unroll
    for (int j = 0; j < 8; ++j) ones[j] = (__bf16)1.f;

    auto multiply_stage = [&](unsigned lY, unsigned lX) {
#pragma unroll
        for (int ks = 0; ks < TN_MS / 32; ++ks) {
            bf4 alo[4], ahi[4], blo[4], bhi[4];
#pragma unroll
            for (int i = 0; i < 4; ++i) {
                unsigned a0, a1;
                trl_frag_addr<false>(lY, TN_ROWB, ks * 32 + q4 * 8, wn * 64 + i * 16, lane, &a0, &a1);
                alo[i] = trl_read<bf4>(a0); ahi[i] = trl_read<bf4>(a1);
                trl_frag_addr<false>(lX, TN_ROWB, ks * 32 + q4 * 8, wk * 64 + i * 16, lane, &a0, &a1);
                blo[i] = trl_read<bf4>(a0); bhi[i] = trl_read<bf4>(a1);
            }
            asm volatile("s_waitcnt lgkmcnt(0)"
                         : "+v"(alo[0]), "+v"(alo[1]), "+v"(alo[2]), "+v"(alo[3]), "+v"(ahi[0]), "+v"(ahi[1]), "+v"(ahi[2]),
                           "+v"(ahi[3]), "+v"(blo[0]), "+v"(blo[1]), "+v"(blo[2]), "+v"(blo[3]), "+v"(bhi[0]), "+v"(bhi[1]),
                           "+v"(bhi[2]), "+v"(bhi[3])
                         :
                         : "memory");
            bf8 af[4], bfr[4];
#pragma unroll
            for (int i = 0; i < 4; ++i) { af[i] = trl_join(alo[i], ahi[i]); bfr[i] = trl_join(blo[i], bhi[i]); }
#pragma unroll
            for (int i = 0; i < 4; ++i) {
#pragma unroll
                for (int j = 0; j < 4; ++j) acc[i][j] = __builtin_amdgcn_mfma_f32_16x16x32_bf16(af[i], bfr[j], acc[i][j], 0, 0, 0);
                if (do_bias) accb[i] = __builtin_amdgcn_mfma_f32_16x16x32_bf16(af[i], ones, accb[i], 0, 0, 0);
            }
        }
    };

    const bool dma_path = n0 + TN_BN <= n && k0 + TN_BK <= k && (m_end - m_beg) % TN_MS == 0 && m_end > m_beg;
    if (dma_path) {
        const unsigned char* gy = reinterpret_cast<const unsigned char*>(dY + (size_t)m_beg * ldy + n0);
        const unsigned char* gx = reinterpret_cast<const unsigned char*>(X + (size_t)m_beg * ldx + k0);
        const int wv = __builtin_amdgcn_readfirstlane(wave);
        unsigned oy[4], ox[4];
#pragma unroll
        for (int i = 0; i < 4; ++i) {
            const int row = 4 * (wv * 4 + i) + (lane >> 4);
            const unsigned ch = (unsigned)((lane & 15) ^ (((lane >> 4) << 2) | i));
            oy[i] = (unsigned)row * (unsigned)(ldy * 2) + ch * 16u;
            ox[i] = (unsigned)row * (unsigned)(ldx * 2) + ch * 16u;
        }
        auto issue = [&](int st, int buf) {
            const unsigned char* py = gy + (size_t)st * TN_MS * ldy * 2;
            const unsigned char* px = gx + (size_t)st * TN_MS * ldx * 2;
            unsigned char* dy_ = smem + buf * 2 * TN_TILE + wv * 4096;
#pragma unroll
            for (int i = 0; i < 4; ++i) ia_lds_dma16(py + oy[i], dy_ + i * 1024);
#pragma unroll
            for (int i = 0; i < 4; ++i) ia_lds_dma16(px + ox[i], dy_ + TN_TILE + i * 1024);
        };
        const int nst = (m_end - m_beg) / TN_MS;
        issue(0, 0);
        for (int st = 0; st < nst; ++st) {
            asm volatile("s_waitcnt vmcnt(0)" ::: "memory");
            __builtin_amdgcn_s_barrier();
            if (st + 1 < nst) issue(st + 1, (st + 1) & 1);
            const unsigned base = ldsY + (unsigned)((st & 1) * 2 * TN_TILE);
            multiply_stage(base, base + TN_TILE);
        }
    } else {
    uint4 ry[4], rx[4];
#define TN_LOAD(m0_)                                                                                               \
    do {                                                                                                           \
        _Pragma("unroll") for (int i = 0; i < 4; ++i) {                                                            \
            const int idx_ = tid + 256 * i, row_ = idx_ >> 4, ch_ = idx_ & 15;                                     \
            const int m_ = (m0_) + row_;                                                                           \
            const bool okm_ = m_ < m_end;                                                                          \
            const int cy_ = n0 + ch_ * 8, cx_ = k0 + ch_ * 8;                                                      \
            ry[i] = (okm_ && cy_ < n) ? *reinterpret_cast<const uint4*>(dY + (size_t)m_ * ldy + cy_) : make_uint4(0, 0, 0, 0); \
            rx[i] = (okm_ && cx_ < k) ? *reinterpret_cast<const uint4*>(X + (size_t)m_ * ldx + cx_) : make_uint4(0, 0, 0, 0);  \
        }                                                                                                          \
    } while (0)
#define TN_STORE()                                                                                                 \
    do {                                                                                                           \
        _Pragma("unroll") for (int i = 0; i < 4; ++i) {                                                            \
            const int idx_ = tid + 256 * i, row_ = idx_ >> 4, ch_ = idx_ & 15;                                     \
            *reinterpret_cast<uint4*>(sY + trl_off<false>(TN_ROWB, row_, ch_)) = ry[i];                                             \
            *reinterpret_cast<uint4*>(sX + trl_off<false>(TN_ROWB, row_, ch_)) = rx[i];                                             \
        }                                                                                                          \
    } while (0)

    TN_LOAD(m_beg);
    for (int m0 = m_beg; m0 < m_end; m0 += TN_MS) {
        __syncthreads();
        TN_STORE();
        __syncthreads();
        if (m0 + TN_MS < m_end) TN_LOAD(m0 + TN_MS);
        multiply_stage(ldsY, ldsX);
    }
    }
#undef TN_LOAD
#undef TN_STORE
    float* prow = part + (size_t)split * row_stride;
#pragma unroll
    for (int i = 0; i < 4; ++i)
#pragma unroll
        for (int r = 0; r < 4; ++r) {
            const int gn = n0 + wn * 64 + i * 16 + q4 * 4 + r;
            if (gn < n) {
#pragma unroll
                for (int j = 0; j < 4; ++j) {
                    const int gk = k0 + wk * 64 + j * 16 + c;
                    if (gk < k) prow[(size_t)gn * k + gk] = acc[i][j][r];
                }
                if (do_bias && c == 0) part_b[(size_t)split * row_stride + gn] = accb[i][r];
            }
        }
}

__global__ __launch_bounds__(256, 2) void gemm_tn_kernel(const __bf16* __restrict__ dY, int ldy, const __bf16* __restrict__ X,
                                                         int ldx, int M, int n, int k, int rows_per_split,
                                                         float* __restrict__ part, float* __restrict__ part_b,
                                                         size_t row_stride) {
    __shared__ __attribute__((aligned(16))) unsigned char smem[4 * TN_TILE];
    const int tiles = ((n + TN_BN - 1) / TN_BN) * ((k + TN_BK - 1) / TN_BK);
    const int S = (M + rows_per_split - 1) / rows_per_split;
    int tile, split;
    if (!tn_map((int)blockIdx.x, tiles, S, &tile, &split)) return;
    tn_tile_body(dY, ldy, X, ldx, M, n, k, rows_per_split, part, part_b, row_stride, tile, split, smem);
}

constexpr int TN_MAX_GROUP = 12;
struct TnProblem {
    const __bf16* dY; const __bf16* X; float* part; float* part_b; float* dW; float* db;
    size_t row_stride; int ldy, ldx, M, n, k, rps, S, tiles, wg_begin; int64_t out_begin;
};
struct TnGroup { TnProblem p[TN_MAX_GROUP]; int count; };

__global__ __launch_bounds__(256, 2) void gemm_tn_grouped_kernel(TnGroup g) {
    __shared__ __attribute__((aligned(16))) unsigned char smem[4 * TN_TILE];
    int pi = 0;
#pragma unroll
    for (int i = 1; i < TN_MAX_GROUP; ++i)
        if (i < g.count && (int)blockIdx.x >= g.p[i].wg_begin) pi = i;
    pi = __builtin_amdgcn_readfirstlane(pi);
    const TnProblem& P = g.p[pi];
    int tile, split;
    if (!tn_map((int)blockIdx.x - P.wg_begin, P.tiles, P.S, &tile, &split)) return;
    tn_tile_body(P.dY, P.ldy, P.X, P.ldx, P.M, P.n, P.k, P.rps, P.part, P.part_b, P.row_stride, tile, split, smem);
}

__global__ __launch_bounds__(256) void gemm_tn_grouped_finish_kernel(TnGroup g, int64_t total4) {
    for (int64_t i = (int64_t)blockIdx.x * 256 + threadIdx.x; i < total4; i += (int64_t)gridDim.x * 256) {
        const int64_t e = i * 4;
        int pi = 0;
#pragma unroll
        for (int j = 1; j < TN_MAX_GROUP; ++j)
            if (j < g.count && e >= g.p[j].out_begin) pi = j;
        const TnProblem& P = g.p[pi];
        const int64_t off = e - P.out_begin;
        const int64_t nk = (int64_t)P.n * P.k;
        if (off >= nk && !P.db) continue;
        float4 a = make_float4(0.f, 0.f, 0.f, 0.f);
        const float* src = P.part + off;
        for (int s_ = 0; s_ < P.S; ++s_) {
            const float4 x = *reinterpret_cast<const float4*>(src + (size_t)s_ * P.row_stride);
            a.x += x.x; a.y += x.y; a.z += x.z; a.w += x.w;
        }
        float* dst = off < nk ? P.dW + off : P.db + (off - nk);
        *reinterpret_cast<float4*>(dst) = a;
    }
}

inline int tn_splits(int M, int n, int k) {
    const int tiles = ((n + TN_BN - 1) / TN_BN) * ((k + TN_BK - 1) / TN_BK);
    int s = (320 + tiles - 1) / tiles;
    const int cap = (M + TN_MS - 1) / TN_MS;
    s = s < 1 ? 1 : (s > cap ? cap : s);
    return s;
}
}

extern "C" int64_t ia_gemm_tn_scratch_elems(int M, int n, int k) {
    if (M <= 0 || n <= 0 || k <= 0) return 0;
    return (int64_t)tn_splits(M, n, k) * ((int64_t)n * k + n);
}

extern "C" int ia_gemm_tn_bf16(const void* dY, int ldy, const void* X, int ldx, int M, int n, int k, float* dW, float* db,
                               float* scratch, ia_stream_t stream) {
    if (!dY || !X || !dW || !scratch || M <= 0 || n <= 0 || k <= 0) return IA_INVALID_VALUE;
    if (n % 8 != 0 || k % 8 != 0 || ldy % 8 != 0 || ldx % 8 != 0 || !ia_is_aligned(dY, 16) || !ia_is_aligned(X, 16)) return IA_UNSUPPORTED;
    int rps;
    const int Seff = tn_plan_splits(M, tn_splits(M, n, k), &rps);
    const size_t row_stride = (size_t)n * k + n;
    float* part = scratch;
    float* part_b = db ? scratch + (size_t)n * k : nullptr;
    hipStream_t st = (hipStream_t)stream;
    const dim3 grid(tn_wgs(((n + TN_BN - 1) / TN_BN) * ((k + TN_BK - 1) / TN_BK), Seff)), blk(256);
    hipLaunchKernelGGL(gemm_tn_kernel, grid, blk, 0, st, (const __bf16*)dY, ldy, (const __bf16*)X, ldx, M, n, k, rps, part, part_b,
                       row_stride);
    IA_RETURN_IF_LAUNCH_FAILED();
    if (db == dW + (size_t)n * k) {
        ia_partials_finish_wide(part, Seff, (int64_t)row_stride, dW, st);
    } else {
        ia_partials_finish_wide_strided(part, Seff, (int64_t)n * k, (int64_t)row_stride, dW, st);
        if (db) {
            IA_RETURN_IF_LAUNCH_FAILED();
            ia_partials_finish_wide_strided(part_b, Seff, (int64_t)n, (int64_t)row_stride, db, st);
        }
    }
    IA_RETURN_IF_LAUNCH_FAILED();
    return IA_OK;
}

namespace {
inline int tn_group_plan(const ia_tn_problem* pr, int count, TnGroup* g, int64_t* scratch_elems, int64_t* out_elems, int* blocks) {
    if (!pr || count <= 0 || count > TN_MAX_GROUP) return IA_INVALID_VALUE;
    int tiles_total = 0;
    for (int i = 0; i < count; ++i) {
        const ia_tn_problem& q = pr[i];
        if (q.M <= 0 || q.n <= 0 || q.k <= 0) return IA_INVALID_VALUE;
        if (q.n % 8 != 0 || q.k % 8 != 0 || q.ldy % 8 != 0 || q.ldx % 8 != 0) return IA_UNSUPPORTED;
        tiles_total += ((q.n + TN_BN - 1) / TN_BN) * ((q.k + TN_BK - 1) / TN_BK);
    }
    int S0 = 512 / tiles_total;
    S0 = S0 < 1 ? 1 : S0;
    int64_t so = 0, oo = 0;
    int wg = 0;
    g->count = count;
    for (int i = 0; i < count; ++i) {
        const ia_tn_problem& q = pr[i];
        TnProblem& P = g->p[i];
        const int cap = (q.M + TN_MS - 1) / TN_MS;
        int rps;
        const int S = tn_plan_splits(q.M, S0 > cap ? cap : S0, &rps);
        P.dY = (const __bf16*)q.dY; P.X = (const __bf16*)q.X; P.ldy = q.ldy; P.ldx = q.ldx; P.M = q.M; P.n = q.n; P.k = q.k;
        P.rps = rps; P.S = S; P.tiles = ((q.n + TN_BN - 1) / TN_BN) * ((q.k + TN_BK - 1) / TN_BK);
        P.row_stride = (size_t)q.n * q.k + q.n;
        P.part = nullptr; P.part_b = nullptr;
        P.dW = q.dW; P.db = q.db;
        P.wg_begin = wg; wg += tn_wgs(P.tiles, S);
        P.out_begin = oo; oo += (int64_t)P.row_stride;
        P.part = reinterpret_cast<float*>(so * sizeof(float));
        so += (int64_t)S * (int64_t)P.row_stride;
        so = (so + 3) / 4 * 4;
    }
    *scratch_elems = so; *out_elems = oo; *blocks = wg;
    return IA_OK;
}
}

extern "C" int64_t ia_gemm_tn_grouped_scratch_elems(const ia_tn_problem* problems, int count) {
    TnGroup g; int64_t so = 0, oo = 0; int blocks = 0;
    if (tn_group_plan(problems, count, &g, &so, &oo, &blocks) != IA_OK) return 0;
    return so;
}

extern "C" int ia_gemm_tn_bf16_grouped(const ia_tn_problem* problems, int count, float* scratch, ia_stream_t stream) {
    if (!scratch) return IA_INVALID_VALUE;
    TnGroup g; int64_t so = 0, oo = 0; int blocks = 0;
    const int rc = tn_group_plan(problems, count, &g, &so, &oo, &blocks);
    if (rc != IA_OK) return rc;
    for (int i = 0; i < count; ++i) {
        TnProblem& P = g.p[i];
        if (!P.dY || !P.X || !P.dW || !ia_is_aligned(P.dY, 16) || !ia_is_aligned(P.X, 16) || !ia_is_aligned(P.dW, 16) ||
            (P.db && !ia_is_aligned(P.db, 16)))
            return IA_INVALID_VALUE;
        P.part = scratch + reinterpret_cast<size_t>(P.part) / sizeof(float);
        P.part_b = P.db ? P.part + (size_t)P.n * P.k : nullptr;
    }
    hipStream_t st = (hipStream_t)stream;
    hipLaunchKernelGGL(gemm_tn_grouped_kernel, dim3(blocks), dim3(256), 0, st, g);
    IA_RETURN_IF_LAUNCH_FAILED();
    const int64_t total4 = oo / 4;
    const int64_t fb = (total4 + 255) / 256;
    hipLaunchKernelGGL(gemm_tn_grouped_finish_kernel, dim3((unsigned)(fb < 2048 ? fb : 2048)), dim3(256), 0, st, g, total4);
    IA_RETURN_IF_LAUNCH_FAILED();
    return IA_OK;
}
```

indic_cl_asr_amd/ops/block.py:

```python
import torch

from .. import _lib
from . import fast


def _ptr(t):
    return _lib.ptr(t)


def _ln_bwd(x, ln, dy_f32=None, dy_bf16=None, dx_in=None):
    N, d = x.shape
    dev = x.device
    dx = torch.empty(N, d, dtype=torch.float32, device=dev)
    dgb = torch.empty(2, d, dtype=torch.float32, device=dev)
    dy = dy_f32 if dy_f32 is not None else dy_bf16
    L = _lib.lib()
    st = L.ia_layernorm_bwd(_ptr(x), x.stride(0), _ptr(dy_f32), _ptr(dy_bf16), dy.stride(0), N, d, _ptr(ln.weight),
                            float(ln.eps), _ptr(dx_in), _ptr(dx), d, _ptr(dgb[0]), _ptr(dgb[1]),
                            _ptr(fast.scratch(dev, L.ia_layernorm_bwd_scratch_elems(N, d))), _lib.stream_ptr())
    _lib.check(st, "ia_layernorm_bwd")
    return dx, dgb[0], dgb[1]


def _branch_grad(dxr, alpha, p, seed):
# ... 86 lines not shown
        elif window is None:
            ctxv, lse = fast.relpos_attention_flash(qkv, pl, att.pos_bias_u, att.pos_bias_v, lens, B, T, att.h, att.d_k, patt, seed + 7,
                                                    want_lse=True)
        else:
            ctxv, lse = fast.relpos_attention_local(qkv, pl, att.pos_bias_u, att.pos_bias_v, lens, B, T, att.h, att.d_k, window, patt,
                                                    seed + 7, want_lse=True)
        x2, _ = fast.gemm(ctxv, W["wo"], att.linear_out.bias, dropout_p=p, seed=seed + 3, residual=x1, out_f32=new(),
                          want_bf16=False)
        y3 = fast.layernorm(x2, layer.norm_conv.weight, layer.norm_conv.bias, layer.norm_conv.eps)
        _, c2 = fast.gemm(y3, W["wp1"], cv.pointwise_conv1.bias)
        bn = cv.batch_norm
        use_batch = bool(tr or not bn.track_running_stats)
        c3, z, sums = fast.glu_dwconv_bn_silu_fast(c2, lens, B, T, d, cv.depthwise_conv.weight, cv.depthwise_conv.bias, bn, tr,
                                                   keep=True)
        x3, _ = fast.gemm(c3, W["wp2"], cv.pointwise_conv2.bias, dropout_p=p, seed=seed + 4, residual=x2, out_f32=new(),
                          want_bf16=False)
        y4 = fast.layernorm(x3, layer.norm_feed_forward2.weight, layer.norm_feed_forward2.bias, layer.norm_feed_forward2.eps)
        _, h4p = fast.gemm(y4, W["w1b"], ff2.linear1.bias)
        h4 = _silu_dropout(h4p, pff2, seed + 5)
        x4, _ = fast.gemm(h4, W["w2b"], ff2.linear2.bias, dropout_p=p, seed=seed + 6, alpha=layer.fc_factor, residual=x3,
                          out_f32=new(), want_bf16=False)
        out = new()
        fast.layernorm(x4, layer.norm_out.weight, layer.norm_out.bias, layer.norm_out.eps, out_f32=out, want_bf16=False)
        if not use_batch:
            raise RuntimeError("trainable fused block expects train-mode BatchNorm (batch statistics)")
        ctx.S = dict(x0=x0, y1=y1, h1p=h1p, h1=h1, x1=x1, y2=y2, qkv=qkv, pl=pl, ctxv=ctxv, lse=lse, x2=x2, y3=y3, c2=c2, z=z, sums=sums,
                     c3=c3, x3=x3, y4=y4, h4p=h4p, h4=h4, x4=x4, W=W, pe=pe, lens=lens)
        ctx.meta = (layer, B, T, seed, p, pff1, pff2, patt, (window, context), [n for n, _ in layer.named_parameters()],
                    [q.requires_grad for q in params], params)
        return out

    @staticmethod
    def backward(ctx, dout):
        L = _lib.lib()
        S = ctx.S
        ctx.S = None
        layer, B, T, seed, p, pff1, pff2, patt, (window, context), names, req, params = ctx.meta
        W = S["W"]
        ff1, ff2, att, cv = layer.feed_forward1, layer.feed_forward2, layer.self_attn, layer.conv
        d = S["x0"].shape[1]
        N = B * T
        dev = dout.device
        G = {}
        dout = dout.float().contiguous()
        dx4, G["norm_out.weight"], G["norm_out.bias"] = _ln_bwd(S["x4"], layer.norm_out, dy_f32=dout)
        dB = _branch_grad(dx4, layer.fc_factor, p, seed + 6)
        dh, G["feed_forward2.linear2.weight"], G["feed_forward2.linear2.bias"] = _lin_bwd(dB, S["h4"], W["w2b"])
        dhp = _silu_dropout_bwd(S["h4p"], dh, pff2, seed + 5)
        dy, G["feed_forward2.linear1.weight"], G["feed_forward2.linear1.bias"] = _lin_bwd(dhp, S["y4"], W["w1b"])
        dx3, G["norm_feed_forward2.weight"], G["norm_feed_forward2.bias"] = _ln_bwd(S["x3"], layer.norm_feed_forward2,
                                                                                  dy_bf16=dy, dx_in=dx4)
        del dx4, dh, dhp
        dB = _branch_grad(dx3, 1.0, p, seed + 4)
        dc3, dWp2, G["conv.pointwise_conv2.bias"] = _lin_bwd(dB, S["c3"], W["wp2"])
        G["conv.pointwise_conv2.weight"] = dWp2.unsqueeze(-1)
        bn = cv.batch_norm
        S12 = torch.empty(2, d, dtype=torch.float32, device=dev)
        dz = torch.empty(N, d, dtype=torch.float32, device=dev)
        sums = S["sums"]
        group = fast.bn_sync_group(bn)
        bn_scr = _ptr(fast.scratch(dev, L.ia_bn_silu_bwd_scratch_elems(N, d)))
        if group is None:
            _lib.check(L.ia_bn_silu_bwd(_ptr(S["z"]), _ptr(dc3), N, d, _ptr(sums[:d]), _ptr(sums[d:2 * d]), _ptr(bn.weight),
                                        _ptr(bn.bias), float(bn.eps), _ptr(S12[0]), _ptr(S12[1]), _ptr(dz), bn_scr,
                                        _lib.stream_ptr()), "ia_bn_silu_bwd")
        else:
            import torch.distributed as dist
            _lib.check(L.ia_bn_silu_bwd_reduce(_ptr(S["z"]), _ptr(dc3), N, d, _ptr(sums[:d]), _ptr(sums[d:2 * d]), _ptr(bn.weight),
                                               _ptr(bn.bias), float(bn.eps), _ptr(S12[0]), _ptr(S12[1]), bn_scr,
                                               _lib.stream_ptr()), "ia_bn_silu_bwd_reduce")
            Sg = torch.cat([S12.reshape(-1), torch.full((1,), float(N), dtype=torch.float32, device=dev)])
            dist.all_reduce(Sg, group=group)
            Sg = Sg[:2 * d] * (float(N) / Sg[2 * d])
            _lib.check(L.ia_bn_silu_bwd_apply(_ptr(S["z"]), _ptr(dc3), N, d, _ptr(sums[:d]), _ptr(sums[d:2 * d]), _ptr(bn.weight),
                                              _ptr(bn.bias), float(bn.eps), _ptr(Sg[:d]), _ptr(Sg[d:]), _ptr(dz),
                                              _lib.stream_ptr()), "ia_bn_silu_bwd_apply")
        G["conv.batch_norm.bias"], G["conv.batch_norm.weight"] = S12[0], S12[1]
        ksz = cv.depthwise_conv.weight.shape[-1]
        w2 = cv.depthwise_conv.weight.detach().float().reshape(d, ksz).contiguous()
        dG = torch.empty(N, d, dtype=torch.float32, device=dev)
        _lib.check(L.ia_dwconv_time(_ptr(dz), B, T, d, ksz, _ptr(w2), None, 1, _ptr(dG), _lib.stream_ptr()), "ia_dwconv_time")
        Gm = torch.empty(N, d, dtype=torch.float32, device=dev)
        _lib.check(L.ia_glu_mask(_ptr(S["c2"]), _ptr(S["lens"]), B, T, d, _ptr(Gm), _lib.stream_ptr()), "ia_glu_mask")
        dwd = torch.empty(d, ksz, dtype=torch.float32, device=dev)
        dbd = torch.empty(d, dtype=torch.float32, device=dev)
        _lib.check(L.ia_dwconv_time_wgrad(_ptr(Gm), _ptr(dz), B, T, d, ksz, _ptr(dwd), _ptr(dbd),
                                          _ptr(fast.scratch(dev, L.ia_dwconv_scratch_elems(B, T, d, ksz))), _lib.stream_ptr()),
                   "ia_dwconv_time_wgrad")
        G["conv.depthwise_conv.weight"], G["conv.depthwise_conv.bias"] = dwd.view(d, 1, ksz), dbd
        dc2 = torch.empty(N, 2 * d, dtype=torch.bfloat16, device=dev)
        _lib.check(L.ia_glu_bwd(_ptr(S["c2"]), _ptr(dG), _ptr(S["lens"]), B, T, d, _ptr(dc2), _lib.stream_ptr()), "ia_glu_bwd")
        dy, dWp1, G["conv.pointwise_conv1.bias"] = _lin_bwd(dc2, S["y3"], W["wp1"])
        G["conv.pointwise_conv1.weight"] = dWp1.unsqueeze(-1)
        dx2, G["norm_conv.weight"], G["norm_conv.bias"] = _ln_bwd(S["x2"], layer.norm_conv, dy_bf16=dy, dx_in=dx3)
        del dx3, dz, dG, Gm, dc2, dc3
        dB = _branch_grad(dx2, 1.0, p, seed + 3)
        dctx, G["self_attn.linear_out.weight"], G["self_attn.linear_out.bias"] = _lin_bwd(dB, S["ctxv"], W["wo"])
        if context is not None:
            dqkv, dpl, du, dv = fast.relpos_attention_context_bwd(S["qkv"], S["pl"], att.pos_bias_u, att.pos_bias_v, S["lens"], S["ctxv"],
                                                                  dctx, S["lse"], B, T, att.h, att.d_k, context, patt, seed + 7)
        elif window is None:
            dqkv, dpl, du, dv = fast.relpos_attention_flash_bwd(S["qkv"], S["pl"], att.pos_bias_u, att.pos_bias_v, S["lens"], S["ctxv"],
                                                                dctx, S["lse"], B, T, att.h, att.d_k, patt, seed + 7)
        else:
            dqkv, dpl, du, dv = fast.relpos_attention_local_bwd(S["qkv"], S["pl"], att.pos_bias_u, att.pos_bias_v, S["lens"], S["ctxv"],
                                                                dctx, S["lse"], B, T, att.h, att.d_k, window, patt, seed + 7)
        G["self_attn.pos_bias_u"], G["self_attn.pos_bias_v"] = du, dv
        dy, dWqkv, dbqkv = _lin_bwd(dqkv, S["y2"], W["wqkv"])
        for i, nm in enumerate(("q", "k", "v")):
            G[f"self_attn.linear_{nm}.weight"] = dWqkv[i * d:(i + 1) * d]
            G[f"self_attn.linear_{nm}.bias"] = dbqkv[i * d:(i + 1) * d]
        G["self_attn.linear_pos.weight"] = _lin_bwd(dpl, S["pe"], None, need_dx=False)[1]
        dx1, G["norm_self_att.weight"], G["norm_self_att.bias"] = _ln_bwd(S["x1"], layer.norm_self_att, dy_bf16=dy, dx_in=dx2)
        del dx2, dqkv, dctx
        dB = _branch_grad(dx1, layer.fc_factor, p, seed + 2)
        dh, G["feed_forward1.linear2.weight"], G["feed_forward1.linear2.bias"] = _lin_bwd(dB, S["h1"], W["w2"])
        dhp = _silu_dropout_bwd(S["h1p"], dh, pff1, seed + 1)
        dy, G["feed_forward1.linear1.weight"], G["feed_forward1.linear1.bias"] = _lin_bwd(dhp, S["y1"], W["w1"])
        dx0, G["norm_feed_forward1.weight"], G["norm_feed_forward1.bias"] = _ln_bwd(S["x0"], layer.norm_feed_forward1,
                                                                                  dy_bf16=dy, dx_in=dx1)
        outs, dst, src = [], [], []
        for n, r, q in zip(names, req, params):
            if not r:
                outs.append(None)
            elif DIRECT_ACCUMULATE and q.grad is not None and q.grad.dtype == torch.float32:
                dst.append(q.grad); src.append(G[n].reshape(q.grad.shape)); outs.append(None)
            else:
                outs.append(G[n].reshape(q.shape))
        if dst:
            torch._foreach_add_(dst, src)
        return (dx0, None, None, None, None, None, None) + tuple(outs)


def pad_pos_emb(pos_emb, d):
    pe = pos_emb.detach().reshape(-1, d)
    rows = (pe.shape[0] + 7) // 8 * 8
    out = torch.zeros(rows, d, dtype=torch.bfloat16, device=pe.device)
    out[:pe.shape[0]] = pe
    return out


def conformer_block(x2d, layer, lens, pe_bf16, B, T, seed):
    if (USE_NATIVE_BLOCKS and layer.training and getattr(layer.self_attn, "att_window", None) is None
            and getattr(layer.self_attn, "att_context", None) is None):
        att = layer.self_attn
        if _lib.lib().ia_conformer_block_supported(x2d.shape[-1], layer.feed_forward1.linear1.weight.shape[0], att.h,
                                                   layer.conv.depthwise_conv.weight.shape[-1], T):
            return conformer_block_native(x2d, layer, lens, pe_bf16, B, T, seed)
    return _ConformerBlockFn.apply(x2d, layer, lens, pe_bf16, B, T, seed, *list(layer.parameters()))


USE_NATIVE_BLOCKS = True

_SAVED_FIELDS = ("y1", "h1p", "h1", "x1", "y2", "qkv", "pl", "ctxv", "x2", "y3", "c2", "z", "sums", "c3", "x3", "y4", "h4p", "h4", "x4", "lse")


def _saved_layout(N, d, dff, pos_rows, H):
    sizes = dict(y1=N * d * 2, h1p=N * dff * 2, h1=N * dff * 2, x1=N * d * 4, y2=N * d * 2, qkv=N * 3 * d * 2, pl=pos_rows * d * 2,
                 ctxv=N * d * 2, x2=N * d * 4, y3=N * d * 2, c2=N * 2 * d * 2, z=N * d * 4, sums=(2 * d + 64) * 4, c3=N * d * 2,
                 x3=N * d * 4, y4=N * d * 2, h4p=N * dff * 2, h4=N * dff * 2, x4=N * d * 4, lse=N * H * 4)
    lay, o = {}, 0
    for f in _SAVED_FIELDS:
        lay[f] = (o, sizes[f])
        o = (o + sizes[f] + 255) // 256 * 256
    return lay, o


class _BlockRuntime:

    def __init__(self, layer, dev):
        import ctypes
        d = layer.norm_out.weight.shape[0]
        dff = layer.feed_forward1.linear1.weight.shape[0]
        ksz = layer.conv.depthwise_conv.weight.shape[-1]
        self.d, self.dff, self.ksz = d, dff, ksz
        blocks = [("w_ff1a", dff * d), ("b_ff1a", dff), ("w_ff1b", d * dff), ("b_ff1b", d), ("w_qkv", 3 * d * d), ("b_qkv", 3 * d),
                  ("w_pos", d * d), ("w_out", d * d), ("b_out", d), ("w_pw1", 2 * d * d), ("b_pw1", 2 * d), ("w_pw2", d * d), ("b_pw2", d),
                  ("w_ff2a", dff * d), ("b_ff2a", dff), ("w_ff2b", d * dff), ("b_ff2b", d)]
        for nm in ("ln_ff1", "ln_att", "ln_conv", "ln_ff2", "ln_out"):
            blocks += [(nm + "_g", d), (nm + "_b", d)]
        blocks += [("dw_w", d * ksz), ("dw_b", d), ("bn_g", d), ("bn_b", d), ("pos_u", d), ("pos_v", d)]
        off, o = {}, 0
        for nm, n in blocks:
            off[nm] = (o, n)
            o += (n + 3) // 4 * 4
        self.arena = torch.zeros(o, dtype=torch.float32, device=dev)
        self.off = off
        base = self.arena.data_ptr()
        self.grads = _lib.BlockGrads()
        for nm, _ in _lib.BlockGrads._fields_:
            setattr(self.grads, nm, base + 4 * off[nm][0])
        self.pos_u = self.arena[off["pos_u"][0]:off["pos_u"][0] + d]
        self.pos_v = self.arena[off["pos_v"][0]:off["pos_v"][0] + d]
        att, cv, ff1, ff2 = layer.self_attn, layer.conv, layer.feed_forward1, layer.feed_forward2
        self.param_src = [
            (ff1.linear1.weight, "w_ff1a", 0), (ff1.linear1.bias, "b_ff1a", 0), (ff1.linear2.weight, "w_ff1b", 0), (ff1.linear2.bias, "b_ff1b", 0),
            (att.linear_q.weight, "w_qkv", 0), (att.linear_k.weight, "w_qkv", d * d), (att.linear_v.weight, "w_qkv", 2 * d * d),
            (att.linear_q.bias, "b_qkv", 0), (att.linear_k.bias, "b_qkv", d), (att.linear_v.bias, "b_qkv", 2 * d),
            (att.linear_pos.weight, "w_pos", 0), (att.linear_out.weight, "w_out", 0), (att.linear_out.bias, "b_out", 0),
            (att.pos_bias_u, "pos_u", 0), (att.pos_bias_v, "pos_v", 0),
            (cv.pointwise_conv1.weight, "w_pw1", 0), (cv.pointwise_conv1.bias, "b_pw1", 0), (cv.pointwise_conv2.weight, "w_pw2", 0),
            (cv.pointwise_conv2.bias, "b_pw2", 0), (cv.depthwise_conv.weight, "dw_w", 0), (cv.depthwise_conv.bias, "dw_b", 0),
            (cv.batch_norm.weight, "bn_g", 0), (cv.batch_norm.bias, "bn_b", 0),
            (ff2.linear1.weight, "w_ff2a", 0), (ff2.linear1.bias, "b_ff2a", 0), (ff2.linear2.weight, "w_ff2b", 0), (ff2.linear2.bias, "b_ff2b", 0),
            (layer.norm_feed_forward1.weight, "ln_ff1_g", 0), (layer.norm_feed_forward1.bias, "ln_ff1_b", 0),
            (layer.norm_self_att.weight, "ln_att_g", 0), (layer.norm_self_att.bias, "ln_att_b", 0),
            (layer.norm_conv.weight, "ln_conv_g", 0), (layer.norm_conv.bias, "ln_conv_b", 0),
            (layer.norm_feed_forward2.weight, "ln_ff2_g", 0), (layer.norm_feed_forward2.bias, "ln_ff2_b", 0),
            (layer.norm_out.weight, "ln_out_g", 0), (layer.norm_out.bias, "ln_out_b", 0)]
        self._table_key, self._table = None, None

    def add_table(self):
        key = tuple((q.grad.data_ptr() if (q.requires_grad and q.grad is not None) else 0) for q, _, _ in self.param_src)
        if key != self._table_key:
            rows = []
            base = self.arena.data_ptr()
            for (q, blk, sub), gp in zip(self.param_src, key):
                if gp:
                    rows.append((gp, base + 4 * (self.off[blk][0] + sub), q.numel()))
            self._table = torch.tensor(rows, dtype=torch.int64).to(self.arena.device) if rows else None
            self._table_key = key
            self._n_rows = len(rows)
        return self._table, (self._n_rows if self._table is not None else 0)


_RUNTIMES = {}
_BWD_WS = {}


def _runtime(layer, dev):
    rt = _RUNTIMES.get(id(layer))
    if rt is None or rt.arena.device != dev:
        import weakref
        rt = _RUNTIMES[id(layer)] = _BlockRuntime(layer, dev)
        weakref.finalize(layer, _RUNTIMES.pop, id(layer), None)
    return rt


class _ConformerBlockNativeFn(torch.autograd.Function):
    @staticmethod
    def forward(ctx, x, layer, lens, pe, B, T, seed, *params):
        import ctypes
        L = _lib.lib()
        N, d = x.shape
        dev = x.device
        rt = _runtime(layer, dev)
        tr = layer.training
        if not tr:
            raise RuntimeError("trainable fused block expects train-mode BatchNorm (batch statistics)")
        bp = fast._block_params(layer)
        x0 = x.contiguous()
        lay, nbytes = _saved_layout(N, d, rt.dff, pe.shape[0], layer.self_attn.h)
        arena = torch.empty(nbytes, dtype=torch.uint8, device=dev)
        saved = _lib.BlockSaved()
        base = arena.data_ptr()
        for f in _SAVED_FIELDS:
            setattr(saved, f, base + lay[f][0])
        out = torch.empty(N, d, dtype=torch.float32, device=dev)
        dw_scr = fast.scratch(dev, L.ia_dwconv_scratch_elems(B, T, d, rt.ksz))
        bn = layer.conv.batch_norm
        group = fast.bn_sync_group(bn)
        fwd_args = (ctypes.addressof(bp), _ptr(x0), _ptr(pe), pe.shape[0], _ptr(lens), B, T, int(seed) & 0xFFFFFFFF,
                    ctypes.addressof(saved), _ptr(out), _ptr(dw_scr))
        if group is None:
            _lib.check(L.ia_conformer_block_fwd(*fwd_args, _lib.stream_ptr()), "ia_conformer_block_fwd")
        else:
            _lib.check(L.ia_conformer_block_fwd_phase(*fwd_args, 1, _lib.stream_ptr()), "ia_conformer_block_fwd_phase")
            o = lay["sums"][0]
            fast.bn_sync_sums(arena[o:o + (2 * d + 1) * 4].view(torch.float32), N, d, bn, group)
            _lib.check(L.ia_conformer_block_fwd_phase(*fwd_args, 2, _lib.stream_ptr()), "ia_conformer_block_fwd_phase")
        ctx.group = group
        ctx.keep = (x0, arena, saved, lay, pe, lens, bp)
        ctx.meta = (layer, B, T, seed, [q.requires_grad for q in params], params)
        return out

    @staticmethod
    def backward(ctx, dout):
        import ctypes
        if ctx.keep is None:
            raise RuntimeError("fused Conformer block: trying to backward through the graph a second time (its saved "
                               "activations were released by the first backward)")
        L = _lib.lib()
        x0, arena, saved, lay, pe, lens, bp = ctx.keep
        ctx.keep = None
        layer, B, T, seed, req, params = ctx.meta
        N, d = x0.shape
        dev = x0.device
        rt = _runtime(layer, dev)
        att = layer.self_attn
        n_ws = L.ia_conformer_block_bwd_ws_bytes(B, T, d, rt.dff, rt.ksz)
        key = (dev.index, torch.cuda.current_stream(dev).cuda_stream)
        ws = _BWD_WS.get(key)
        if ws is None or ws.numel() < n_ws:
            ws = _BWD_WS[key] = torch.empty(n_ws, dtype=torch.uint8, device=dev)
        dout = dout.float().contiguous()
        dx2_p, dctx_p = ctypes.c_void_p(), ctypes.c_void_p()
        sp = _lib.stream_ptr()
        a_args = (ctypes.addressof(bp), ctypes.addressof(saved), ctypes.addressof(rt.grads), _ptr(dout), _ptr(lens), B, T,
                  int(seed) & 0xFFFFFFFF, _ptr(ws), n_ws, ctypes.addressof(dx2_p), ctypes.addressof(dctx_p))
        if ctx.group is None:
            _lib.check(L.ia_conformer_block_bwd_a(*a_args, sp), "ia_conformer_block_bwd_a")
        else:
            import torch.distributed as dist
            _lib.check(L.ia_conformer_block_bwd_a_phase(*a_args, 1, None, sp), "ia_conformer_block_bwd_a_phase")
            ob, og = rt.off["bn_b"][0], rt.off["bn_g"][0]
            Sg = torch.cat([rt.arena[ob:ob + d], rt.arena[og:og + d], torch.full((1,), float(N), dtype=torch.float32, device=dev)])
            fast.SYNC_BN_COLLECTIVES += 1
            dist.all_reduce(Sg, group=ctx.group)
            Sg = (Sg[:2 * d] * (float(N) / Sg[2 * d])).contiguous()
            _lib.check(L.ia_conformer_block_bwd_a_phase(*a_args, 2, _ptr(Sg), sp), "ia_conformer_block_bwd_a_phase")
        def view(buf, off, shape, dtype):
            n = 1
            for s_ in shape:
                n *= s_
            return buf[off:off + n * torch.empty(0, dtype=dtype).element_size()].view(dtype).view(*shape)
        qkv = view(arena, lay["qkv"][0], (N, 3 * d), torch.bfloat16)
        pl = view(arena, lay["pl"][0], (pe.shape[0], d), torch.bfloat16)
        ctxv = view(arena, lay["ctxv"][0], (N, d), torch.bfloat16)
        dctx = view(ws, dctx_p.value - ws.data_ptr(), (N, d), torch.bfloat16)
        lse = view(arena, lay["lse"][0], (B * att.h, T), torch.float32)
        patt = float(att.dropout_rate)
        dqkv, dpl, du, dv = fast.relpos_attention_flash_bwd(qkv, pl, att.pos_bias_u, att.pos_bias_v, lens, ctxv, dctx, lse, B, T, att.h,
                                                            att.d_k, patt, seed + 7, dub_out=(rt.pos_u, rt.pos_v))
        dx0 = torch.empty(N, d, dtype=torch.float32, device=dev)
        table, n_rows = rt.add_table() if DIRECT_ACCUMULATE else (None, 0)
        st = L.ia_conformer_block_bwd_b(ctypes.addressof(bp), ctypes.addressof(saved), ctypes.addressof(rt.grads), _ptr(x0), _ptr(pe), pe.shape[0],
                                        _ptr(dqkv), _ptr(dpl), B, T, int(seed) & 0xFFFFFFFF, _ptr(ws), n_ws, _ptr(dx0), _ptr(table),
                                        n_rows, sp)
        _lib.check(st, "ia_conformer_block_bwd_b")
        outs = []
        by_id = {id(q): (blk, sub) for q, blk, sub in rt.param_src}
        for r, q in zip(req, params):
            if not r:
                outs.append(None)
            elif DIRECT_ACCUMULATE and q.grad is not None and q.grad.dtype == torch.float32:
                outs.append(None)
            else:
                blk, sub = by_id[id(q)]
                o = rt.off[blk][0] + sub
                outs.append(rt.arena[o:o + q.numel()].view(q.shape).clone())
        return (dx0, None, None, None, None, None, None) + tuple(outs)


def conformer_block_native(x2d, layer, lens, pe_bf16, B, T, seed):
    return _ConformerBlockNativeFn.apply(x2d, layer, lens, pe_bf16, B, T, seed, *list(layer.parameters()))
```

indic_cl_asr_amd/ops/fast.py:

```python
import ctypes
import weakref

import torch

from .. import _lib

_SHADOW = {}
WEIGHT_EPOCH = 0


def bump_weight_epoch():
    global WEIGHT_EPOCH
    WEIGHT_EPOCH += 1


def invalidate_weight_caches():
    _SHADOW.clear(); _FLAT16.clear(); _BLOCK_PARAMS.clear(); _POS_PROJ.clear()
    bump_weight_epoch()


def _refs(cache, key, params):
    def drop(_ref, cache=cache, key=key):
        cache.pop(key, None)
    return tuple(weakref.ref(p, drop) for p in params)
# ... 352 lines not shown
    if keep:
        return out, z, sums
    return out


def attention_flash_supported(T, dk):
    return bool(_lib.lib().ia_relpos_attention_flash_supported(int(T), int(dk)))


def attention_local_supported(T, dk, window):
    return bool(_lib.lib().ia_relpos_attention_local_supported(int(T), int(dk), int(window)))


CONTEXT_STYLES = {"regular": 0, "chunked_limited": 1}


def context_args(context):
    style, left, right = context
    if isinstance(style, str):
        if style not in CONTEXT_STYLES:
            raise ValueError(f"Invalid att_context_style: {style}")
        style = CONTEXT_STYLES[style]
    return int(style), int(left), int(right)


def attention_context_supported(T, dk, context):
    return bool(_lib.lib().ia_relpos_attention_context_supported(int(T), int(dk), *context_args(context)))


def _span(window):
    if window is None:
        return "flash", ()
    if isinstance(window, (tuple, list)):
        return "context", context_args(window)
    return "local", (int(window),)


def _attention_fwd(window, qkv_bf16, pos_proj_bf16, bias_u, bias_v, lens, B, T, H, dk, dropout_p, seed, want_lse):
    kind, win = _span(window)
    ctx = torch.empty(B * T, H * dk, dtype=torch.bfloat16, device=qkv_bf16.device)
    lse = torch.empty(B * H, T, dtype=torch.float32, device=qkv_bf16.device) if want_lse else None
    name = f"ia_relpos_attention_{kind}_lse"
    st = getattr(_lib.lib(), name)(_lib.ptr(qkv_bf16), _lib.ptr(pos_proj_bf16), _lib.ptr(bias_u), _lib.ptr(bias_v), _lib.ptr(lens),
                                   B, T, H, dk, *win, float(dropout_p), int(seed) & 0xFFFFFFFF, _lib.ptr(ctx), _lib.ptr(lse),
                                   _lib.stream_ptr())
    _lib.check(st, name)
    return (ctx, lse) if want_lse else ctx


def relpos_attention_flash(qkv_bf16, pos_proj_bf16, bias_u, bias_v, lens, B, T, H, dk, dropout_p=0.0, seed=0, want_lse=False):
    return _attention_fwd(None, qkv_bf16, pos_proj_bf16, bias_u, bias_v, lens, B, T, H, dk, dropout_p, seed, want_lse)


def relpos_attention_local(qkv_bf16, pos_proj_bf16, bias_u, bias_v, lens, B, T, H, dk, window, dropout_p=0.0, seed=0, want_lse=False):
    if pos_proj_bf16.shape[0] < 2 * int(window) + 1:
        raise ValueError(f"relpos_attention_local: {pos_proj_bf16.shape[0]} position rows < 2 * {window} + 1")
    return _attention_fwd(window, qkv_bf16, pos_proj_bf16, bias_u, bias_v, lens, B, T, H, dk, dropout_p, seed, want_lse)


def relpos_attention_context(qkv_bf16, pos_proj_bf16, bias_u, bias_v, lens, B, T, H, dk, context, dropout_p=0.0, seed=0,
                             want_lse=False):
    if pos_proj_bf16.shape[0] < 2 * int(T) - 1:
        raise ValueError(f"relpos_attention_context: {pos_proj_bf16.shape[0]} position rows < 2 * {T} - 1")
    return _attention_fwd(tuple(context), qkv_bf16, pos_proj_bf16, bias_u, bias_v, lens, B, T, H, dk, dropout_p, seed, want_lse)


def _attention_bwd_dims(window, T):
    kind, win = _span(window)
    rs, p0 = ctypes.c_int(), ctypes.c_int()
    _lib.check(getattr(_lib.lib(), f"ia_relpos_attention_{kind}_bwd_dims")(int(T), *win, ctypes.byref(rs), ctypes.byref(p0)), "dims")
    return rs.value, p0.value


def attention_flash_bwd_dims(T):
    return _attention_bwd_dims(None, T)


def attention_local_bwd_dims(T, window):
    return _attention_bwd_dims(window, T)


def attention_context_bwd_dims(T, context):
    return _attention_bwd_dims(tuple(context), T)


def _attention_bwd(window, qkv, pl, bias_u, bias_v, lens, ctx, dctx, lse, B, T, H, dk, dropout_p, seed, dub_out):
    kind, win = _span(window)
    L = _lib.lib()
    dev = qkv.device
    d = H * dk
    bf = torch.bfloat16
    Rs, pad0 = _attention_bwd_dims(window, T)
    dqkv = torch.empty(B * T, 3 * d, dtype=bf, device=dev)
    dpl = torch.empty_like(pl)
    dBand = torch.empty(H * B * T * Rs, dtype=bf, device=dev)
    QvHM = torch.empty(H * B * T * 64, dtype=bf, device=dev)
    ws = torch.empty(getattr(L, f"ia_relpos_attention_{kind}_bwd_ws_elems")(B, T, H, dk, *win), dtype=torch.float32, device=dev)
    dub = dub_out if dub_out is not None else torch.empty(2, H, dk, dtype=torch.float32, device=dev)
    dctx = dctx.contiguous()
    name = f"ia_relpos_attention_{kind}_bwd"
    st = getattr(L, name)(_lib.ptr(qkv), _lib.ptr(pl), _lib.ptr(bias_u), _lib.ptr(bias_v), _lib.ptr(lens), _lib.ptr(ctx), _lib.ptr(dctx),
                          _lib.ptr(lse), B, T, H, dk, *win, float(dropout_p), int(seed) & 0xFFFFFFFF, _lib.ptr(dqkv), _lib.ptr(dpl),
                          pl.shape[0], _lib.ptr(dub[0]), _lib.ptr(dub[1]), _lib.ptr(dBand), _lib.ptr(QvHM), _lib.ptr(ws),
                          _lib.stream_ptr())
    _lib.check(st, name)
    return dqkv, dpl, dub[0], dub[1]


def relpos_attention_flash_bwd(qkv, pl, bias_u, bias_v, lens, ctx, dctx, lse, B, T, H, dk, dropout_p=0.0, seed=0, dub_out=None):
    return _attention_bwd(None, qkv, pl, bias_u, bias_v, lens, ctx, dctx, lse, B, T, H, dk, dropout_p, seed, dub_out)


def relpos_attention_local_bwd(qkv, pl, bias_u, bias_v, lens, ctx, dctx, lse, B, T, H, dk, window, dropout_p=0.0, seed=0, dub_out=None):
    return _attention_bwd(window, qkv, pl, bias_u, bias_v, lens, ctx, dctx, lse, B, T, H, dk, dropout_p, seed, dub_out)


def relpos_attention_context_bwd(qkv, pl, bias_u, bias_v, lens, ctx, dctx, lse, B, T, H, dk, context, dropout_p=0.0, seed=0, dub_out=None):
    return _attention_bwd(tuple(context), qkv, pl, bias_u, bias_v, lens, ctx, dctx, lse, B, T, H, dk, dropout_p, seed, dub_out)


def relpos_attention(qkv_bf16, pos_proj_bf16, bias_u, bias_v, lens, B, T, H, dk, dropout_p=0.0, seed=0):
    L = _lib.lib()
    dev = qkv_bf16.device
    vt = torch.empty(L.ia_attn_vt_elems(B, T, H), dtype=torch.bfloat16, device=dev)
    ctx = torch.empty(B * T, H * dk, dtype=torch.bfloat16, device=dev)
    st = L.ia_relpos_attention(_lib.ptr(qkv_bf16), _lib.ptr(pos_proj_bf16), _lib.ptr(bias_u), _lib.ptr(bias_v),
                               _lib.ptr(lens), B, T, H, dk, float(dropout_p), int(seed) & 0xFFFFFFFF, _lib.ptr(vt),
                               _lib.ptr(ctx), _lib.stream_ptr())
    _lib.check(st, "ia_relpos_attention")
    return ctx


def colsum(x_bf16):
    M, N = x_bf16.shape
    out = torch.zeros(N, dtype=torch.float32, device=x_bf16.device)
    st = _lib.lib().ia_colsum_bf16(_lib.ptr(x_bf16), M, N, x_bf16.stride(0), _lib.ptr(out), _lib.stream_ptr())
    _lib.check(st, "ia_colsum_bf16")
    return out


def gemm_tn(dy_bf16, x_bf16):
    L = _lib.lib()
    M, N = dy_bf16.shape
    K = x_bf16.shape[1]
    buf = torch.empty(N * K + N, dtype=torch.float32, device=dy_bf16.device)
    dW, db = buf[:N * K].view(N, K), buf[N * K:]
    st = L.ia_gemm_tn_bf16(_lib.ptr(dy_bf16), dy_bf16.stride(0), _lib.ptr(x_bf16), x_bf16.stride(0), M, N, K, _lib.ptr(dW),
                           _lib.ptr(db), _lib.ptr(scratch(dy_bf16.device, L.ia_gemm_tn_scratch_elems(M, N, K))),
                           _lib.stream_ptr())
    _lib.check(st, "ia_gemm_tn_bf16")
    return dW, db


def gemm_tn_grouped(pairs):
    import ctypes
    L = _lib.lib()
    n_ = len(pairs)
    arr = (_lib.TnProblem * n_)()
    outs = []
    dev = pairs[0][0].device
    for i, (dy, x) in enumerate(pairs):
        M, N = dy.shape
        K = x.shape[1]
        buf = torch.empty(N * K + N, dtype=torch.float32, device=dev)
        outs.append((buf[:N * K].view(N, K), buf[N * K:]))
        arr[i].dY, arr[i].X, arr[i].dW, arr[i].db = dy.data_ptr(), x.data_ptr(), buf.data_ptr(), buf.data_ptr() + 4 * N * K
        arr[i].ldy, arr[i].ldx, arr[i].M, arr[i].n, arr[i].k = dy.stride(0), x.stride(0), M, N, K
    scr = scratch(dev, L.ia_gemm_tn_grouped_scratch_elems(ctypes.addressof(arr), n_))
    st = L.ia_gemm_tn_bf16_grouped(ctypes.addressof(arr), n_, _lib.ptr(scr), _lib.stream_ptr())
    _lib.check(st, "ia_gemm_tn_bf16_grouped")
    return outs


def weight_t_shadow(weight):
    return _cached(("wT", id(weight)), (weight,), lambda: bf16_shadow(weight).t().contiguous())


def gemm_data_grad(dy_bf16, weight):
    return gemm(dy_bf16, weight_t_shadow(weight))[1]


class _LinearHip(torch.autograd.Function):

    @staticmethod
    def forward(ctx, x, weight, bias):
        shp = x.shape
        if x.dtype == torch.bfloat16 and x.is_contiguous():
            xb = x.detach().view(-1, shp[-1])
        elif x.is_contiguous():
            from . import tail
            xb = tail.bf16_of(x)
        else:
            xb = torch.empty(shp, dtype=torch.bfloat16, device=x.device)
            xb.copy_(x.detach())
            xb = xb.view(-1, shp[-1])
        wb = bf16_shadow(weight)
        _, y = gemm(xb, wb, bias.detach().float() if bias is not None else None)
        ctx.save_for_backward(xb, wb)
        ctx.weight = weight
        ctx.meta = (shp, x.dtype, weight.dtype, weight.shape, bias.dtype if bias is not None else None)
        return y.view(*shp[:-1], wb.shape[0])

    @staticmethod
    def backward(ctx, dy):
        xb, wb = ctx.saved_tensors
        shp, xdt, wdt, wshape, bdt = ctx.meta
        dyb = dy.reshape(-1, wb.shape[0]).to(torch.bfloat16).contiguous()
        M, N = dyb.shape
        K = xb.shape[1]
        dx = dW = db = None
        if ctx.needs_input_grad[0]:
            if gemm_supported(N, K):
                dx = gemm_data_grad(dyb, ctx.weight).view(shp).to(xdt)
            else:
                dx = torch.mm(dyb, wb).view(shp).to(xdt)
        if ctx.needs_input_grad[1] or (bdt is not None and ctx.needs_input_grad[2]):
            if N % 8 == 0 and K % 8 == 0:
                dWf, dbf = gemm_tn(dyb, xb)
            else:
                dWf = torch.mm(dyb.t(), xb, out_dtype=torch.float32)
                dbf = dyb.float().sum(0)
            if ctx.needs_input_grad[1]:
                dW = dWf.view(wshape).to(wdt)
            if bdt is not None and ctx.needs_input_grad[2]:
                db = dbf.to(bdt)
        return dx, dW, db


def linear(x, weight, bias=None):
    w2 = weight if weight.dim() == 2 else weight.reshape(weight.shape[0], -1)
    if (x.is_cuda and torch.is_autocast_enabled() and gemm_supported(w2.shape[1], w2.shape[0])
            and (x.requires_grad or weight.requires_grad)):
        return _LinearHip.apply(x, weight, bias)
    return torch.nn.functional.linear(x, w2, bias)


def _cached(key, params, make):
    ver = tuple(p._version for p in params) + tuple(p.data_ptr() for p in params) + \
        ((WEIGHT_EPOCH,) if any(p.requires_grad for p in params) else ())
    hit = _SHADOW.get(key)
    if hit is not None and hit[0] == ver and _same(hit[2], params):
        return hit[1]
    with torch.no_grad():
        val = make()
    _SHADOW[key] = (ver, val, _refs(_SHADOW, key, params))
    return val


def subsample_supported(C, d, feat_in):
    return (C % 8 == 0 and C <= 2048 and d % 8 == 0
            and (C * (((feat_in - 1) // 2 + 1 - 1) // 2 + 1)) % 8 == 0)


def conv_subsampling(feats_bft, conv1, conv2, lin, alpha=1.0, dropout_p=0.0, seed=0):
    L = _lib.lib()
    x = feats_bft.float().contiguous()
    B, Fm, Tm = x.shape
    C = conv1.weight.shape[0]
    T1, F1 = (Tm - 1) // 2 + 1, (Fm - 1) // 2 + 1
    T2, F2 = (T1 - 1) // 2 + 1, (F1 - 1) // 2 + 1
    dev = x.device
    w1 = _cached(("sub_w1", id(conv1.weight)), [conv1.weight], lambda: conv1.weight.detach().float().reshape(C, 9).contiguous())
    o1 = torch.empty(B * T1 * F1, C, dtype=torch.bfloat16, device=dev)
    _lib.check(L.ia_subsample_conv1(_lib.ptr(x), B, Fm, Tm, C, _lib.ptr(w1), _lib.ptr(conv1.bias), _lib.ptr(o1),
                                    _lib.stream_ptr()), "ia_subsample_conv1")
    N = conv2.weight.shape[0]
    w2r = _cached(("sub_w2", id(conv2.weight)), [conv2.weight],
                  lambda: conv2.weight.detach().permute(0, 2, 3, 1).reshape(N, 9 * C).to(torch.bfloat16).contiguous())
    o2 = torch.empty(B * T2 * F2, N, dtype=torch.bfloat16, device=dev)
    _lib.check(L.ia_subsample_conv2(_lib.ptr(o1), B, T1, F1, C, _lib.ptr(w2r), _lib.ptr(conv2.bias), N, _lib.ptr(o2),
                                    _lib.stream_ptr()), "ia_subsample_conv2")
    d = lin.weight.shape[0]
    wl = _cached(("sub_wl", id(lin.weight)), [lin.weight],
                 lambda: lin.weight.detach().view(d, N, F2).permute(0, 2, 1).reshape(d, F2 * N).to(torch.bfloat16).contiguous())
    y = torch.empty(B * T2, d, dtype=torch.float32, device=dev)
    gemm(o2.view(B * T2, F2 * N), wl, lin.bias, out_f32=y, want_bf16=False, alpha=float(alpha), dropout_p=float(dropout_p), seed=seed)
    return y.view(B, T2, d)


_BLOCK_PARAMS = {}


def _block_params(layer):
    ff1, ff2, att, cv, bn = layer.feed_forward1, layer.feed_forward2, layer.self_attn, layer.conv, layer.conv.batch_norm
    watch = (ff1.linear1.weight, ff1.linear2.weight, att.linear_q.weight, att.linear_k.weight, att.linear_v.weight,
             att.linear_pos.weight, att.linear_out.weight, cv.pointwise_conv1.weight, cv.pointwise_conv2.weight,
             ff2.linear1.weight, ff2.linear2.weight, att.linear_q.bias, att.linear_k.bias, att.linear_v.bias,
             cv.depthwise_conv.weight, cv.pointwise_conv1.bias)
    ver = tuple(p._version for p in watch) + tuple(p.data_ptr() for p in watch) + \
        ((WEIGHT_EPOCH,) if any(p.requires_grad for p in watch) else ()) + \
        (layer.dropout.p, ff1.dropout.p, ff2.dropout.p, att.dropout_rate)
    hit = _BLOCK_PARAMS.get(id(layer))
    if hit is not None and hit[0] == ver and _same(hit[3], watch):
        return hit[1]
    d = ff1.linear1.weight.shape[1]
    keep = dict(
        w_ff1a=bf16_shadow(ff1.linear1.weight), w_ff1b=bf16_shadow(ff1.linear2.weight),
        w_qkv=bf16_shadow(att.linear_q.weight, att.linear_k.weight, att.linear_v.weight), w_pos=bf16_shadow(att.linear_pos.weight),
        w_out=bf16_shadow(att.linear_out.weight), w_pw1=bf16_shadow(cv.pointwise_conv1.weight),
        w_pw2=bf16_shadow(cv.pointwise_conv2.weight), w_ff2a=bf16_shadow(ff2.linear1.weight), w_ff2b=bf16_shadow(ff2.linear2.weight),
        b_ff1a=ff1.linear1.bias, b_ff1b=ff1.linear2.bias, b_qkv=f32_cat(att.linear_q.bias, att.linear_k.bias, att.linear_v.bias),
        b_out=att.linear_out.bias, b_pw1=cv.pointwise_conv1.bias, b_pw2=cv.pointwise_conv2.bias, b_ff2a=ff2.linear1.bias,
        b_ff2b=ff2.linear2.bias,
        ln_ff1_g=layer.norm_feed_forward1.weight, ln_ff1_b=layer.norm_feed_forward1.bias, ln_att_g=layer.norm_self_att.weight,
        ln_att_b=layer.norm_self_att.bias, ln_conv_g=layer.norm_conv.weight, ln_conv_b=layer.norm_conv.bias,
        ln_ff2_g=layer.norm_feed_forward2.weight, ln_ff2_b=layer.norm_feed_forward2.bias, ln_out_g=layer.norm_out.weight,
        ln_out_b=layer.norm_out.bias, pos_u=att.pos_bias_u, pos_v=att.pos_bias_v, dw_w=cv.depthwise_conv.weight,
        dw_b=cv.depthwise_conv.bias, bn_g=bn.weight, bn_b=bn.bias, bn_rm=bn.running_mean, bn_rv=bn.running_var,
        bn_nbt=bn.num_batches_tracked)
    frozen_pw1 = not (cv.pointwise_conv1.weight.requires_grad or cv.pointwise_conv1.bias.requires_grad)
    glu = glu_regrouped(cv.pointwise_conv1.weight, cv.pointwise_conv1.bias) if frozen_pw1 else None
    if glu is not None:
        keep["w_pw1_glu"], keep["b_pw1_glu"] = glu
    bp = _lib.BlockParams()
    for k, t in keep.items():
        setattr(bp, k, t.data_ptr())
    bp.ln_eps, bp.bn_eps = float(layer.norm_out.eps), float(bn.eps)
    bp.bn_momentum = float(bn.momentum if bn.momentum is not None else 0.1)
    bp.p_drop, bp.p_ff, bp.p_att = float(layer.dropout.p), float(ff1.dropout.p), float(att.dropout_rate)
    bp.fc_factor = float(layer.fc_factor)
    bp.d, bp.d_ff, bp.n_heads, bp.ksz = d, ff1.linear1.weight.shape[0], att.h, cv.depthwise_conv.weight.shape[-1]
    _BLOCK_PARAMS[id(layer)] = (ver, bp, keep, _refs(_BLOCK_PARAMS, id(layer), watch))
    return bp
# ... 67 lines not shown
```

indic_cl_asr_amd/ops/joint.py:

```python
import math

import os

import torch

from .. import _lib

JOINT_MAX_V = 272
MFMA_PROFILE_HOOK = None
USE_FUSED_DH = True
DW_SKIP_DEAD_FRAMES = os.environ.get("IA_DW_SKIP", "1") != "0"
USE_FUSED_DW = True
LAST_GRAD_KERNEL_EVENT = None


def fused_joint_supported(H, V, device):
    return device.type == "cuda" and H % 64 == 0 and H >= 64 and V <= JOINT_MAX_V


def _kappa_for(scale_hint):
    s = abs(float(scale_hint)) if scale_hint else 1.0
    return float(2.0 ** math.floor(-math.log2(s))) if s > 0 else 1.0


# ... 176 lines not shown
                        _kappa_for(scale_hint), f.dtype, g.dtype, W.dtype, bias.dtype, nbytes)
        return costs, (torch.zeros((), dtype=torch.float32, device=dev) if stash is not None else None)

    @staticmethod
    def _rnnt_gradient(ctx, L, rl, gcosts, logits, ws, labels, act_lens, label_lens, fused_dw, kappa, skip_dead=False):
        B, T, U1, H, V, LD, blank, p, seed, fastemit, _, fdt, gdt, wdt, bdt, nbytes = ctx.meta
        dev = logits.device
        cells = B * T * U1
        cg = gcosts.reshape(-1).float().contiguous()
        GT, S, Kc = None, 0, 0
        if not fused_dw:
            S = 64
            Kc = ((cells + S - 1) // S + 63) // 64 * 64
            GT = torch.empty(S, LD, Kc, dtype=torch.float16, device=dev)
        hook = None
        if rl.PROFILE_HOOK is not None:
            hook = rl.PROFILE_HOOK(B, T, U1, V, 2, 2 if fused_dw else 3, "joint_grad_h_db_kernel" if fused_dw else "joint_grad_h_t_kernel",
                                   bool(skip_dead))
        ev0, ev1 = hook if hook is not None else (None, None)
        dbk = dbscr = None
        if fused_dw:
            dbk = torch.empty(LD, dtype=torch.float32, device=dev)
            dbscr = torch.empty(L.ia_joint_backward_g_dbias_scratch_elems(LD), dtype=torch.float32, device=dev)
        st = L.ia_joint_backward_g_skip(_lib.ptr(logits), _lib.ptr(labels), _lib.ptr(act_lens), _lib.ptr(label_lens), B, T, U1, V,
                                        LD, blank, fastemit, _lib.ptr(cg), kappa, _lib.ptr(GT), S, Kc, _lib.ptr(dbk), _lib.ptr(dbscr),
                                        _lib.ptr(ws), nbytes, int(bool(skip_dead)), _lib.stream_ptr(), ev0, ev1)
        _lib.check(st, "ia_joint_backward_g_skip")
        global LAST_GRAD_KERNEL_EVENT
        LAST_GRAD_KERNEL_EVENT = torch.cuda.Event()
        LAST_GRAD_KERNEL_EVENT.record()
        G = logits
        return G, dbk, GT, S, Kc

    @staticmethod
    def backward(ctx, gcosts, gtoken):
        from ..losses import rnnt as rl
        L = _lib.lib()
        stash = ctx.stash
        E = stash.pending_E if (stash is not None and gtoken is not None) else None
        if gcosts is None and E is None:
            return (None,) * 17
        if ctx.saved is None:
            raise RuntimeError("fused joint+loss: trying to backward through the graph a second time -- the saved lattice "
                               "was overwritten in place by the first backward (the fused path does not support "
                               "retain_graph=True; run the forward again)")
        f16, g16, Wp, logits, ws, labels, act_lens, label_lens = ctx.saved
        B, T, U1, H, V, LD, blank, p, seed, fastemit, kappa, fdt, gdt, wdt, bdt, nbytes = ctx.meta
        ctx.saved = None
        dev = f16.device
        cells = B * T * U1
        fused_dw = USE_FUSED_DW and cells < 2 ** 31 and L.ia_joint_dw_fused_supported(U1, H, LD)
        if stash is not None:
            stash.logits = None
        if E is not None:
            kappa = stash.kappa
            stash.pending_E = None
            if not (fused_dw and USE_FUSED_DH and L.ia_joint_dh_fused_supported(U1, H, LD)):
                raise RuntimeError("fused joint: the continual-learning terms need the fused hidden- and weight-gradient "
                                   "kernels (H % 320 == 0); set joint.use_fused = False for this shape")
        have_rnnt = gcosts is not None
        dbk = None
        if not have_rnnt:
            G = E
            dbk = torch.sum(E, 0, dtype=torch.float32)
            GT, S, Kc = None, 0, 0
        else:
            skip_dead = (E is None and fused_dw and DW_SKIP_DEAD_FRAMES and USE_FUSED_DH
                         and bool(L.ia_joint_dh_fused_supported(U1, H, LD)))
            G, dbk, GT, S, Kc = _FusedJointRNNT._rnnt_gradient(ctx, L, rl, gcosts, logits, ws, labels, act_lens, label_lens,
                                                               fused_dw, kappa, skip_dead)
            if E is not None:
                st = L.ia_lattice_add_f16(_lib.ptr(G), _lib.ptr(E), G.numel(), _lib.stream_ptr())
                _lib.check(st, "ia_lattice_add_f16")
                dbk = dbk + torch.sum(E, 0, dtype=torch.float32)
        if E is not None:
            act_lens, label_lens = stash.box_t, stash.box_um1
        del E
        LDH = H + 8
        dh_fused = bool(USE_FUSED_DH and L.ia_joint_dh_fused_supported(U1, H, LD))
        proj_mode = ctx.proj is not None
        dfb = dgb = None
        if dh_fused and proj_mode:
            df = dg = None
            dfb = torch.empty(B * T, H, dtype=torch.bfloat16, device=dev)
            dgb = torch.empty(B * U1, H, dtype=torch.bfloat16, device=dev)
        else:
            df = torch.zeros(B, T, H, dtype=torch.float32, device=dev)
            dg = torch.zeros(B, U1, H, dtype=torch.float32, device=dev)
        if dh_fused:
            Wt = ctx.Wt
            if Wt is None:
                Wt = torch.zeros(H, L.ia_joint_dh_k(), dtype=torch.float16, device=dev)
                Wt[:, :JOINT_MAX_V] = Wp.t()
            scr = torch.empty(L.ia_joint_dh_fused_scratch_bytes(B, T, U1, H), dtype=torch.uint8, device=dev)
            ev = MFMA_PROFILE_HOOK(2.0 * cells * H * LD) if MFMA_PROFILE_HOOK is not None else None
            if ev is not None:
                ev[0].record()
            st = L.ia_joint_dh_fused_ex(_lib.ptr(G), _lib.ptr(Wt), _lib.ptr(f16), _lib.ptr(g16), _lib.ptr(act_lens),
                                        _lib.ptr(label_lens), _lib.ptr(df), _lib.ptr(dg), _lib.ptr(dfb), _lib.ptr(dgb),
                                        1 if dfb is not None else 0, B, T, U1, H, LD, 1.0 / kappa, p, seed, _lib.ptr(scr),
                                        _lib.stream_ptr())
            _lib.check(st, "ia_joint_dh_fused_ex")
            if ev is not None:
                ev[1].record()
        else:
            dH = torch.mm(G, Wp[:LD])
            scr = torch.empty(L.ia_joint_dh_reduce_scratch_bytes(B, T, U1, H), dtype=torch.uint8, device=dev)
            st = L.ia_joint_dh_reduce(_lib.ptr(dH), _lib.ptr(f16), _lib.ptr(g16), _lib.ptr(act_lens), _lib.ptr(label_lens),
                                      _lib.ptr(df), _lib.ptr(dg), B, T, U1, H, 1.0 / kappa, p, seed, _lib.ptr(scr),
                                      _lib.stream_ptr())
            _lib.check(st, "ia_joint_dh_reduce")
            del dH
        if fused_dw:
            dWk = torch.empty(LD, H, dtype=torch.float32, device=dev)
            scr = torch.empty(L.ia_joint_dw_fused_scratch_elems(B, T, U1, H, LD), dtype=torch.float32, device=dev)
            st = L.ia_joint_dw_fused_ex(_lib.ptr(G), _lib.ptr(f16), _lib.ptr(g16), _lib.ptr(act_lens) if DW_SKIP_DEAD_FRAMES else None,
                                        _lib.ptr(label_lens) if DW_SKIP_DEAD_FRAMES else None, B, T, U1, H, LD, p, seed,
                                        _lib.ptr(dWk), _lib.ptr(scr), _lib.stream_ptr())
            _lib.check(st, "ia_joint_dw_fused_ex")
            dW_src, dW_scale = dWk[:V], 1.0 / (kappa * (1.0 - p))
            db_src, db_scale = dbk[:V], 1.0 / kappa
        else:
            HT = torch.empty(S, LDH, Kc, dtype=torch.float16, device=dev)
            st = L.ia_joint_hidden_t(_lib.ptr(f16), _lib.ptr(g16), _lib.ptr(HT), B, T, U1, H, LDH, S, Kc, p, seed,
                                     _lib.stream_ptr())
            _lib.check(st, "ia_joint_hidden_t")
            dWx = torch.bmm(GT, HT.transpose(1, 2), out_dtype=torch.float32).sum(0)
            dW_src, dW_scale = dWx[:V, :H].contiguous(), 1.0 / (kappa * (1.0 - p))
            db_src, db_scale = dWx[:V, H].contiguous(), 1.0 / kappa
        from . import fast, tail
        Wh, bh = ctx.head
        need = ctx.needs_input_grad
        plist = [(Wh, dW_src if need[2] else None, dW_scale), (bh, db_src if need[3] else None, db_scale)]
        if ctx.proj is None:
            outs = tail.accumulate_or_return(plist)
            return (df.to(fdt), dg.to(gdt)) + outs + (None,) * 13
        xb, gb, We16, Wg16, g_time_major, d, Hp, We, be, Wg, bg = ctx.proj
        ctx.proj = None
        if dfb is None:
            dfb = df.view(B * T, H).to(torch.bfloat16)
            dgb = dg.view(B * U1, H).to(torch.bfloat16)
        WeT, WgT = fast.transpose16_multi([We16, Wg16])
        dx = dgin = None
        if need[0]:
            dx = torch.empty(B * T, d, dtype=torch.float32, device=dev)
            fast.gemm(dfb, WeT, out_f32=dx, want_bf16=False)
            dx = dx.view(B, T, d).to(fdt)
        if need[1]:
            dgm = fast.gemm(dgb, WgT)[1].view(B, U1, Hp)
            if g_time_major:
                dgin = fast.swap01_cast(dgm, torch.float32 if gdt == torch.float32 else torch.bfloat16).transpose(0, 1).to(gdt)
            else:
                dgin = dgm.to(gdt)
        (dWe, dbe), (dWg, dbg) = fast.gemm_tn_grouped([(dfb, xb), (dgb, gb)])
        plist += [(We, dWe if need[13] else None, 1.0), (be, dbe if need[14] else None, 1.0),
                  (Wg, dWg if need[15] else None, 1.0), (bg, dbg if need[16] else None, 1.0)]
        outs = tail.accumulate_or_return(plist)
        return (dx, dgin) + outs[:2] + (None,) * 9 + outs[2:]


def _make_stash(req, logits, geom, dev):
    import numpy as np
    B, T, U1, V, LD = geom
    sub, h_enc, h_tgt = int(req["sub"]), req["h_enc"], req["h_tgt"]
    n_sub = (B + sub - 1) // sub
    ints = np.empty((3, B), dtype=np.int64)
    w = np.empty((2, B), dtype=np.float32)
    for b0 in range(0, B, sub):
        b1 = min(b0 + sub, B)
        mt, mu1 = min(max(h_enc[b0:b1]), T), min(max(h_tgt[b0:b1]) + 1, U1)
        ints[0, b0:b1], ints[1, b0:b1], ints[2, b0:b1] = mt, mu1, mu1 - 1
        w[0, b0:b1] = 1.0 / (n_sub * (b1 - b0) * mt * mu1)
        w[1, b0:b1] = 1.0 / (n_sub * (b1 - b0))
    di = torch.from_numpy(ints).pin_memory().to(dev, non_blocking=True)
    dw = torch.from_numpy(w).pin_memory().to(dev, non_blocking=True)
    st = LatticeStash(logits, geom, (di[0], di[1], di[2]), (dw[0], dw[1]), n_sub, sub, None, bool(req.get("detach")))
    st.host_boxes = (ints[0].tolist(), ints[1].tolist())
    st.host_weights = (float(w[0].max()), float(w[1].max()))
    return st


def fused_joint_rnnt(f, g, W, bias, labels, act_lens, label_lens, blank, dropout_p=0.0, seed=0, fastemit_lambda=0.0,
                     scale_hint=1.0, stash_req=None, enc_proj=None, pred_proj=None):
    extra = (None, None, None, None)
    if enc_proj is not None:
        extra = (enc_proj[0], enc_proj[1], pred_proj[0], pred_proj[1])
    costs, token = _FusedJointRNNT.apply(f, g, W, bias, labels.contiguous(), act_lens.contiguous(), label_lens.contiguous(),
                                         blank, dropout_p, seed, fastemit_lambda, scale_hint, stash_req, *extra)
    if stash_req is not None and not stash_req.get("detach") and token is not None and token.requires_grad:
        stash_req["out"].token = token
    return costs
```

Before: 3760 utterances/s.

## Accumulate weight gradients directly into param.grad from grouped TN GEMM

```diff
diff --git a/include/indicasr.h b/include/indicasr.h
--- a/include/indicasr.h
+++ b/include/indicasr.h
@@ -252,6 +252,13 @@
 } ia_tn_problem;
 int64_t ia_gemm_tn_grouped_scratch_elems(const ia_tn_problem* problems, int count);
 int ia_gemm_tn_bf16_grouped(const ia_tn_problem* problems, int count, float* scratch, ia_stream_t stream);
+#define IA_TN_ACCUMULATE 1
+typedef struct ia_tn_problem_ex {
+    const void* dY; const void* X; float* dW; float* db;
+    int ldy, ldx, M, n, k, flags;
+} ia_tn_problem_ex;
+int64_t ia_gemm_tn_grouped_ex_scratch_elems(const ia_tn_problem_ex* problems, int count);
+int ia_gemm_tn_bf16_grouped_ex(const ia_tn_problem_ex* problems, int count, float* scratch, ia_stream_t stream);
 int64_t ia_gemm_tn_scratch_elems(int M, int n, int k);
 int ia_gemm_tn_bf16(const void* dY, int ldy, const void* X, int ldx, int M, int n, int k, float* dW, float* db,
                     float* scratch, ia_stream_t stream);
@@ -326,6 +333,18 @@
                              const float* x0, const void* pos_emb, int pos_rows, const void* dqkv, const void* dpl, int B,
                              int T, unsigned seed, void* workspace, size_t workspace_bytes, float* dx0,
                              const void* add_table, int n_add, ia_stream_t stream);
+typedef struct ia_block_grad_dst {
+    float *w_ff1a, *b_ff1a, *w_ff1b, *b_ff1b, *w_q, *b_q, *w_k, *b_k, *w_v, *b_v, *w_pos, *w_out, *b_out, *w_pw1, *b_pw1;
+    float *w_pw2, *b_pw2, *w_ff2a, *b_ff2a, *w_ff2b, *b_ff2b;
+} ia_block_grad_dst;
+int ia_conformer_block_bwd_a_acc(const struct ia_block_params* layer, const ia_block_saved* saved, const ia_block_grads* grads,
+                                 const ia_block_grad_dst* dst, const float* dout, const int64_t* lens, int B, int T,
+                                 unsigned seed, void* workspace, size_t workspace_bytes, float** dx2_out, void** dctx_out,
+                                 int phase, const float* bn_S12, ia_stream_t stream);
+int ia_conformer_block_bwd_b_acc(const struct ia_block_params* layer, const ia_block_saved* saved, const ia_block_grads* grads,
+                                 const ia_block_grad_dst* dst, const float* x0, const void* pos_emb, int pos_rows,
+                                 const void* dqkv, const void* dpl, int B, int T, unsigned seed, void* workspace,
+                                 size_t workspace_bytes, float* dx0, const void* add_table, int n_add, ia_stream_t stream);
 
 int ia_layernorm_bwd(const float* x, int ldx, const float* dy_f32, const void* dy_bf16, int ldy, int N, int d,
                      const float* gamma, float eps, const float* dx_in, float* dx_out, int lddx, float* dgamma,
diff --git a/indic_cl_asr_amd/_lib.py b/indic_cl_asr_amd/_lib.py
--- a/indic_cl_asr_amd/_lib.py
+++ b/indic_cl_asr_amd/_lib.py
@@ -32,6 +32,19 @@
 class TnProblem(_c.Structure):
     _fields_ = [("dY", _c.c_void_p), ("X", _c.c_void_p), ("dW", _c.c_void_p), ("db", _c.c_void_p),
                 ("ldy", _c.c_int), ("ldx", _c.c_int), ("M", _c.c_int), ("n", _c.c_int), ("k", _c.c_int)]
+
+
+TN_ACCUMULATE = 1
+
+
+class TnProblemEx(_c.Structure):
+    _fields_ = TnProblem._fields_ + [("flags", _c.c_int)]
+
+
+class BlockGradDst(_c.Structure):
+    _fields_ = [(n, _c.c_void_p) for n in (
+        "w_ff1a", "b_ff1a", "w_ff1b", "b_ff1b", "w_q", "b_q", "w_k", "b_k", "w_v", "b_v", "w_pos", "w_out", "b_out", "w_pw1", "b_pw1",
+        "w_pw2", "b_pw2", "w_ff2a", "b_ff2a", "w_ff2b", "b_ff2b")]
 
 
 class BlockGrads(_c.Structure):
@@ -98,6 +111,8 @@
     "ia_gemm_fp8": (_i, [_vp, _i, _vp, _vp, _i, _vp, _i, _i, _i, _vp, _i, _f, _c.c_uint, _f, _vp, _i, _vp, _i, _vp, _i, _vp]),
     "ia_gemm_tn_grouped_scratch_elems": (_i64, [_vp, _i]),
     "ia_gemm_tn_bf16_grouped": (_i, [_vp, _i, _vp, _vp]),
+    "ia_gemm_tn_grouped_ex_scratch_elems": (_i64, [_vp, _i]),
+    "ia_gemm_tn_bf16_grouped_ex": (_i, [_vp, _i, _vp, _vp]),
     "ia_greedy_decode_lds_bytes": (_i, [_i, _i, _i]),
     "ia_greedy_rnnt_decode": (_i, [_vp, _vp, _vp, _vp, _vp, _vp, _vp, _vp, _i, _i, _i, _i, _i, _i, _i, _i, _i, _vp, _i, _vp, _vp, _vp]),
     "ia_greedy_rnnt_decode_bf16w": (_i, [_vp, _vp, _vp, _vp, _vp, _vp, _vp, _vp, _i, _i, _i, _i, _i, _i, _i, _i, _i, _vp, _i, _vp, _vp, _vp]),
@@ -193,6 +208,8 @@
     "ia_conformer_block_bwd_a": (_i, [_vp, _vp, _vp, _vp, _vp, _i, _i, _c.c_uint, _vp, _sz, _vp, _vp, _vp]),
     "ia_conformer_block_bwd_a_phase": (_i, [_vp, _vp, _vp, _vp, _vp, _i, _i, _c.c_uint, _vp, _sz, _vp, _vp, _i, _vp, _vp]),
     "ia_conformer_block_bwd_b": (_i, [_vp, _vp, _vp, _vp, _vp, _i, _vp, _vp, _i, _i, _c.c_uint, _vp, _sz, _vp, _vp, _i, _vp]),
+    "ia_conformer_block_bwd_a_acc": (_i, [_vp, _vp, _vp, _vp, _vp, _vp, _i, _i, _c.c_uint, _vp, _sz, _vp, _vp, _i, _vp, _vp]),
+    "ia_conformer_block_bwd_b_acc": (_i, [_vp, _vp, _vp, _vp, _vp, _vp, _i, _vp, _vp, _i, _i, _c.c_uint, _vp, _sz, _vp, _vp, _i, _vp]),
     "ia_layernorm_bwd": (_i, [_vp, _i, _vp, _vp, _i, _i, _i, _vp, _f, _vp, _vp, _i, _vp, _vp, _vp, _vp]),
     "ia_layernorm_bwd_drop": (_i, [_vp, _i, _vp, _vp, _i, _i, _i, _vp, _f, _vp, _vp, _i, _vp, _vp, _f, _f, _c.c_uint, _vp, _i, _vp, _vp]),
     "ia_layernorm_bwd_partial_rows": (_i, [_i]),
diff --git a/indic_cl_asr_amd/csrc/block_train.hip b/indic_cl_asr_amd/csrc/block_train.hip
--- a/indic_cl_asr_amd/csrc/block_train.hip
+++ b/indic_cl_asr_amd/csrc/block_train.hip
@@ -141,21 +141,21 @@
     }
     scr = max3(scr, (size_t)ia_bn_silu_bwd_scratch_elems((int64_t)N, d), (size_t)ia_dwconv_scratch_elems(B, T, d, ksz));
     {
-        const ia_tn_problem ga[5] = {{nullptr, nullptr, nullptr, nullptr, d, d_ff, (int)N, d, d_ff},
+        const ia_tn_problem_ex ga[5] = {{nullptr, nullptr, nullptr, nullptr, d, d_ff, (int)N, d, d_ff},
                                      {nullptr, nullptr, nullptr, nullptr, d_ff, d, (int)N, d_ff, d},
                                      {nullptr, nullptr, nullptr, nullptr, d, d, (int)N, d, d},
                                      {nullptr, nullptr, nullptr, nullptr, 2 * d, d, (int)N, 2 * d, d},
                                      {nullptr, nullptr, nullptr, nullptr, d, d, (int)N, d, d}};
-        const ia_tn_problem gb[4] = {{nullptr, nullptr, nullptr, nullptr, 3 * d, d, (int)N, 3 * d, d},
+        const ia_tn_problem_ex gb[4] = {{nullptr, nullptr, nullptr, nullptr, 3 * d, d, (int)N, 3 * d, d},
                                      {nullptr, nullptr, nullptr, nullptr, d, d, (int)(N > (size_t)64 * 512 ? N : (size_t)64 * 512), d, d},
                                      {nullptr, nullptr, nullptr, nullptr, d, d_ff, (int)N, d, d_ff},
                                      {nullptr, nullptr, nullptr, nullptr, d_ff, d, (int)N, d_ff, d}};
-        scr = max3(scr, (size_t)ia_gemm_tn_grouped_scratch_elems(ga, 5), (size_t)ia_gemm_tn_grouped_scratch_elems(gb, 4));
-        scr = max3(scr, (size_t)ia_gemm_tn_grouped_scratch_elems(gb, 2), (size_t)ia_gemm_tn_grouped_scratch_elems(gb + 2, 2));
-        ia_tn_problem gall[9];
+        scr = max3(scr, (size_t)ia_gemm_tn_grouped_ex_scratch_elems(ga, 5), (size_t)ia_gemm_tn_grouped_ex_scratch_elems(gb, 4));
+        scr = max3(scr, (size_t)ia_gemm_tn_grouped_ex_scratch_elems(gb, 2), (size_t)ia_gemm_tn_grouped_ex_scratch_elems(gb + 2, 2));
+        ia_tn_problem_ex gall[9];
         for (int i = 0; i < 5; ++i) gall[i] = ga[i];
         for (int i = 0; i < 4; ++i) gall[5 + i] = gb[i];
-        scr = scr > (size_t)ia_gemm_tn_grouped_scratch_elems(gall, 9) ? scr : (size_t)ia_gemm_tn_grouped_scratch_elems(gall, 9);
+        scr = scr > (size_t)ia_gemm_tn_grouped_ex_scratch_elems(gall, 9) ? scr : (size_t)ia_gemm_tn_grouped_ex_scratch_elems(gall, 9);
     }
     w.scr = o;  o = up256(o + scr * 4);
     w.total = o;
@@ -175,17 +175,38 @@
     static const bool on = [] { const char* e = getenv("IA_TN_GROUPED"); return !(e && e[0] == '0'); }();
     return on;
 }
-int flush_group(const ia_tn_problem* grp, int ngrp, float* scr, ia_stream_t stream) {
-    if (tn_grouping_enabled()) return ia_gemm_tn_bf16_grouped(grp, ngrp, scr, stream);
-    for (int i = 0; i < ngrp; ++i)
+int flush_group(const ia_tn_problem_ex* grp, int ngrp, float* scr, ia_stream_t stream) {
+    if (tn_grouping_enabled()) return ia_gemm_tn_bf16_grouped_ex(grp, ngrp, scr, stream);
+    for (int i = 0; i < ngrp; ++i) {
+        if (grp[i].flags) return IA_UNSUPPORTED;
         IA_TRY(ia_gemm_tn_bf16(grp[i].dY, grp[i].ldy, grp[i].X, grp[i].ldx, grp[i].M, grp[i].n, grp[i].k, grp[i].dW, grp[i].db, scr, stream));
+    }
+    return IA_OK;
+}
+inline ia_tn_problem_ex wgrad_problem(const void* dY, int ldy, const void* X, int M, int n, int k, float* dW, float* db, float* accW,
+                                      float* accb) {
+    if (accW) return ia_tn_problem_ex{dY, X, accW, db ? accb : nullptr, ldy, k, M, n, k, IA_TN_ACCUMULATE};
+    return ia_tn_problem_ex{dY, X, dW, db, ldy, k, M, n, k, 0};
+}
+const ia_block_grad_dst kNoDst = {};
+int check_dst(const ia_block_grad_dst& D) {
+    const float* const pairs[][2] = {{D.w_ff1a, D.b_ff1a}, {D.w_ff1b, D.b_ff1b}, {D.w_q, D.b_q}, {D.w_k, D.b_k}, {D.w_v, D.b_v},
+                                     {D.w_out, D.b_out}, {D.w_pw1, D.b_pw1}, {D.w_pw2, D.b_pw2}, {D.w_ff2a, D.b_ff2a},
+                                     {D.w_ff2b, D.b_ff2b}};
+    bool any = D.w_pos != nullptr;
+    for (const auto& pr : pairs) {
+        if ((pr[0] != nullptr) != (pr[1] != nullptr)) return IA_INVALID_VALUE;
+        any = any || pr[0];
+    }
+    if ((D.w_q != nullptr) != (D.w_k != nullptr) || (D.w_q != nullptr) != (D.w_v != nullptr)) return IA_INVALID_VALUE;
+    if (any && !tn_grouping_enabled()) return IA_UNSUPPORTED;
     return IA_OK;
 }
 int linear_bwd_deferred(const void* dY, const void* X, const void* W, int M, int n, int k, void* dX, float* dW, float* db, const void* wt,
-                        ia_tn_problem* grp, int* ngrp, ia_stream_t stream) {
+                        float* accW, float* accb, ia_tn_problem_ex* grp, int* ngrp, ia_stream_t stream) {
     (void)W;
     if (dX) IA_TRY(ia_gemm_bf16(dY, n, wt, n, M, k, n, nullptr, 0, 0.f, 0, 1.f, nullptr, 0, nullptr, 0, dX, k, stream));
-    grp[*ngrp] = ia_tn_problem{dY, X, dW, db, n, k, M, n, k};
+    grp[*ngrp] = wgrad_problem(dY, n, X, M, n, k, dW, db, accW, accb);
     ++*ngrp;
     return IA_OK;
 }
@@ -211,7 +232,7 @@
     }
     return c.ok ? &c : nullptr;
 }
-struct PendingGroup { ia_tn_problem grp[8]; int n = 0; const void* ws = nullptr; };
+struct PendingGroup { ia_tn_problem_ex grp[8]; int n = 0; const void* ws = nullptr; };
 PendingGroup* pending_group() {
     static PendingGroup pg[16];
     int dev = 0;
@@ -292,19 +313,29 @@
 extern "C" int ia_conformer_block_bwd_a(const ia_block_params* Lp, const ia_block_saved* Sp, const ia_block_grads* Gp,
                                         const float* dout, const int64_t* lens, int B, int T, unsigned seed, void* workspace,
                                         size_t workspace_bytes, float** dx2_out, void** dctx_out, ia_stream_t stream) {
-    return ia_conformer_block_bwd_a_phase(Lp, Sp, Gp, dout, lens, B, T, seed, workspace, workspace_bytes, dx2_out, dctx_out, 0, nullptr,
-                                          stream);
+    return ia_conformer_block_bwd_a_acc(Lp, Sp, Gp, nullptr, dout, lens, B, T, seed, workspace, workspace_bytes, dx2_out, dctx_out, 0,
+                                        nullptr, stream);
 }
 
 extern "C" int ia_conformer_block_bwd_a_phase(const ia_block_params* Lp, const ia_block_saved* Sp, const ia_block_grads* Gp,
                                               const float* dout, const int64_t* lens, int B, int T, unsigned seed,
                                               void* workspace, size_t workspace_bytes, float** dx2_out, void** dctx_out,
                                               int phase, const float* bn_S12, ia_stream_t stream) {
+    return ia_conformer_block_bwd_a_acc(Lp, Sp, Gp, nullptr, dout, lens, B, T, seed, workspace, workspace_bytes, dx2_out, dctx_out, phase,
+                                        bn_S12, stream);
+}
+
+extern "C" int ia_conformer_block_bwd_a_acc(const ia_block_params* Lp, const ia_block_saved* Sp, const ia_block_grads* Gp,
+                                            const ia_block_grad_dst* Dp, const float* dout, const int64_t* lens, int B, int T,
+                                            unsigned seed, void* workspace, size_t workspace_bytes, float** dx2_out,
+                                            void** dctx_out, int phase, const float* bn_S12, ia_stream_t stream) {
     if (phase < 0 || phase > 2 || (phase == 2 && !bn_S12)) return IA_INVALID_VALUE;
     if (!Lp || !Sp || !Gp || !dout || !lens || !workspace || !dx2_out || !dctx_out || B <= 0 || T <= 0) return IA_INVALID_VALUE;
     const ia_block_params& L = *Lp;
     const ia_block_saved& S = *Sp;
     const ia_block_grads& G = *Gp;
+    const ia_block_grad_dst& D = Dp ? *Dp : kNoDst;
+    IA_TRY(check_dst(D));
     const int d = L.d, d_ff = L.d_ff, ksz = L.ksz, N = B * T;
     const BwdWs w = bwd_ws(B, T, d, d_ff, ksz);
     if (workspace_bytes < w.total) return IA_WORKSPACE_TOO_SMALL;
@@ -315,7 +346,7 @@
     void *dB = ws + w.dB, *dB1 = ws + w.dB1, *dB2 = ws + w.dB2, *dhp = ws + w.dhp, *dy = ws + w.dy, *dc3 = ws + w.dc3, *dc2 = ws + w.dc2,
          *dctx = ws + w.dctx, *wt = ws + w.wt;
     const float p = L.p_drop, pff = L.p_ff;
-    ia_tn_problem grp[8];
+    ia_tn_problem_ex grp[8];
     int ngrp = 0;
     char* wtb = (char*)wt;
     void *wt_ff2b = wtb, *wt_ff2a = wtb + (size_t)d * d_ff * 2, *wt_pw2 = wtb + (size_t)2 * d * d_ff * 2,
@@ -331,11 +362,11 @@
                                  L.fc_factor, p, seed + 6, dB, d, lnp + 0 * lnp_set, stream));
     IA_TRY(ia_gemm_bf16_ex(dB, d, wt_ff2b, d, N, d_ff, d, nullptr, 3, pff, seed + 5, 1.f, nullptr, 0, nullptr, 0, dhp, d_ff, nullptr, 0,
                            S.h4p, d_ff, stream));
-    IA_TRY(linear_bwd_deferred(dB, S.h4, L.w_ff2b, N, d, d_ff, nullptr, G.w_ff2b, G.b_ff2b, wt_ff2b, grp, &ngrp, stream));
-    IA_TRY(linear_bwd_deferred(dhp, S.y4, L.w_ff2a, N, d_ff, d, dy, G.w_ff2a, G.b_ff2a, wt_ff2a, grp, &ngrp, stream));
+    IA_TRY(linear_bwd_deferred(dB, S.h4, L.w_ff2b, N, d, d_ff, nullptr, G.w_ff2b, G.b_ff2b, wt_ff2b, D.w_ff2b, D.b_ff2b, grp, &ngrp, stream));
+    IA_TRY(linear_bwd_deferred(dhp, S.y4, L.w_ff2a, N, d_ff, d, dy, G.w_ff2a, G.b_ff2a, wt_ff2a, D.w_ff2a, D.b_ff2a, grp, &ngrp, stream));
     IA_TRY(ia_layernorm_bwd_drop(S.x3, d, nullptr, dy, d, N, d, L.ln_ff2_g, L.ln_eps, dxa, dxb, d, nullptr, nullptr, 1.f, p,
                                  seed + 4, dB1, d, lnp + 1 * lnp_set, stream));
-    IA_TRY(linear_bwd_deferred(dB1, S.c3, L.w_pw2, N, d, d, dc3, G.w_pw2, G.b_pw2, wt_pw2, grp, &ngrp, stream));
+    IA_TRY(linear_bwd_deferred(dB1, S.c3, L.w_pw2, N, d, d, dc3, G.w_pw2, G.b_pw2, wt_pw2, D.w_pw2, D.b_pw2, grp, &ngrp, stream));
     if (phase == 0)
         IA_TRY(ia_bn_silu_bwd(S.z, dc3, N, d, S.sums, S.sums + d, L.bn_g, L.bn_b, L.bn_eps, G.bn_b, G.bn_g, dz, scr, stream));
     else
@@ -356,10 +387,10 @@
     } else {
         IA_TRY(ia_dwconv_glu_wgrad(S.c2, lens, dz, B, T, d, ksz, G.dw_w, G.dw_b, scr, stream));
     }
-    IA_TRY(linear_bwd_deferred(dc2, S.y3, L.w_pw1, N, 2 * d, d, dy, G.w_pw1, G.b_pw1, wt_pw1, grp, &ngrp, stream));
+    IA_TRY(linear_bwd_deferred(dc2, S.y3, L.w_pw1, N, 2 * d, d, dy, G.w_pw1, G.b_pw1, wt_pw1, D.w_pw1, D.b_pw1, grp, &ngrp, stream));
     IA_TRY(ia_layernorm_bwd_drop(S.x2, d, nullptr, dy, d, N, d, L.ln_conv_g, L.ln_eps, dxb, dxa, d, nullptr, nullptr, 1.f, p,
                                  seed + 3, dB2, d, lnp + 2 * lnp_set, stream));
-    IA_TRY(linear_bwd_deferred(dB2, S.ctxv, L.w_out, N, d, d, dctx, G.w_out, G.b_out, wt_out, grp, &ngrp, stream));
+    IA_TRY(linear_bwd_deferred(dB2, S.ctxv, L.w_out, N, d, d, dctx, G.w_out, G.b_out, wt_out, D.w_out, D.b_out, grp, &ngrp, stream));
     if (side) {
         IA_TRY(stream_after(main, side->s, side->ev[1]));
         IA_TRY(flush_group(grp, ngrp, scr, (ia_stream_t)side->s));
@@ -381,10 +412,21 @@
                                         const float* x0, const void* pos_emb, int pos_rows, const void* dqkv, const void* dpl,
                                         int B, int T, unsigned seed, void* workspace, size_t workspace_bytes, float* dx0,
                                         const void* add_table, int n_add, ia_stream_t stream) {
+    return ia_conformer_block_bwd_b_acc(Lp, Sp, Gp, nullptr, x0, pos_emb, pos_rows, dqkv, dpl, B, T, seed, workspace, workspace_bytes, dx0,
+                                        add_table, n_add, stream);
+}
+
+extern "C" int ia_conformer_block_bwd_b_acc(const ia_block_params* Lp, const ia_block_saved* Sp, const ia_block_grads* Gp,
+                                            const ia_block_grad_dst* Dp, const float* x0, const void* pos_emb, int pos_rows,
+                                            const void* dqkv, const void* dpl, int B, int T, unsigned seed, void* workspace,
+                                            size_t workspace_bytes, float* dx0, const void* add_table, int n_add,
+                                            ia_stream_t stream) {
     if (!Lp || !Sp || !Gp || !x0 || !pos_emb || !dqkv || !dpl || !workspace || !dx0 || B <= 0 || T <= 0) return IA_INVALID_VALUE;
     const ia_block_params& L = *Lp;
     const ia_block_saved& S = *Sp;
     const ia_block_grads& G = *Gp;
+    const ia_block_grad_dst& D = Dp ? *Dp : kNoDst;
+    IA_TRY(check_dst(D));
     const int d = L.d, d_ff = L.d_ff, ksz = L.ksz, N = B * T;
     const BwdWs w = bwd_ws(B, T, d, d_ff, ksz);
     if (workspace_bytes < w.total) return IA_WORKSPACE_TOO_SMALL;
@@ -396,7 +438,7 @@
     const bool carried = pg && pg->n > 0 && pg->ws == workspace;
     void *dB = ws + (carried ? w.dB3 : w.dB), *dhp = ws + (carried ? w.dh : w.dhp), *dy = ws + w.dy, *wt = ws + w.wt;
     const float p = L.p_drop, pff = L.p_ff;
-    ia_tn_problem grp[12];
+    ia_tn_problem_ex grp[12];
     int ngrp = 0;
     if (carried) {
         for (int i = 0; i < pg->n; ++i) grp[ngrp++] = pg->grp[i];
@@ -411,8 +453,16 @@
     }
     SideCtx* side = carried ? nullptr : side_ctx();
     hipStream_t main = (hipStream_t)stream;
-    IA_TRY(linear_bwd_deferred(dqkv, S.y2, L.w_qkv, N, 3 * d, d, dy, G.w_qkv, G.b_qkv, wt_qkv, grp, &ngrp, stream));
-    grp[ngrp++] = ia_tn_problem{dpl, pos_emb, G.w_pos, nullptr, d, d, pos_rows, d, d};
+    if (D.w_q) {
+        IA_TRY(ia_gemm_bf16(dqkv, 3 * d, wt_qkv, 3 * d, N, d, 3 * d, nullptr, 0, 0.f, 0, 1.f, nullptr, 0, nullptr, 0, dy, d, stream));
+        float* const aw[3] = {D.w_q, D.w_k, D.w_v};
+        float* const ab[3] = {D.b_q, D.b_k, D.b_v};
+        for (int j = 0; j < 3; ++j)
+            grp[ngrp++] = wgrad_problem((const __hip_bfloat16*)dqkv + (size_t)j * d, 3 * d, S.y2, N, d, d, nullptr, ab[j], aw[j], ab[j]);
+    } else {
+        IA_TRY(linear_bwd_deferred(dqkv, S.y2, L.w_qkv, N, 3 * d, d, dy, G.w_qkv, G.b_qkv, wt_qkv, nullptr, nullptr, grp, &ngrp, stream));
+    }
+    grp[ngrp++] = wgrad_problem(dpl, d, pos_emb, pos_rows, d, d, G.w_pos, nullptr, D.w_pos, nullptr);
     if (side) {
         IA_TRY(stream_after(main, side->s, side->ev[3]));
         IA_TRY(flush_group(grp, ngrp, scr, (ia_stream_t)side->s));
@@ -426,15 +476,15 @@
                                  p, seed + 2, dB, d, lnp + 3 * lnp_set, stream));
     IA_TRY(ia_gemm_bf16_ex(dB, d, wt_ff1b, d, N, d_ff, d, nullptr, 3, pff, seed + 1, 1.f, nullptr, 0, nullptr, 0, dhp, d_ff, nullptr, 0,
                            S.h1p, d_ff, stream));
-    IA_TRY(linear_bwd_deferred(dB, S.h1, L.w_ff1b, N, d, d_ff, nullptr, G.w_ff1b, G.b_ff1b, wt_ff1b, grp, &ngrp, stream));
+    IA_TRY(linear_bwd_deferred(dB, S.h1, L.w_ff1b, N, d, d_ff, nullptr, G.w_ff1b, G.b_ff1b, wt_ff1b, D.w_ff1b, D.b_ff1b, grp, &ngrp, stream));
     if (side) {
-        grp[ngrp++] = ia_tn_problem{dhp, S.y1, G.w_ff1a, G.b_ff1a, d_ff, d, N, d_ff, d};
+        grp[ngrp++] = wgrad_problem(dhp, d_ff, S.y1, N, d_ff, d, G.w_ff1a, G.b_ff1a, D.w_ff1a, D.b_ff1a);
         IA_TRY(stream_after(main, side->s, side->ev[4]));
         IA_TRY(flush_group(grp, ngrp, scr, (ia_stream_t)side->s));
         ngrp = 0;
         IA_TRY(ia_gemm_bf16(dhp, d_ff, wt_ff1a, d_ff, N, d, d_ff, nullptr, 0, 0.f, 0, 1.f, nullptr, 0, nullptr, 0, dy, d, stream));
     } else {
-        IA_TRY(linear_bwd_deferred(dhp, S.y1, L.w_ff1a, N, d_ff, d, dy, G.w_ff1a, G.b_ff1a, wt_ff1a, grp, &ngrp, stream));
+        IA_TRY(linear_bwd_deferred(dhp, S.y1, L.w_ff1a, N, d_ff, d, dy, G.w_ff1a, G.b_ff1a, wt_ff1a, D.w_ff1a, D.b_ff1a, grp, &ngrp, stream));
     }
     IA_TRY(ia_layernorm_bwd(x0, d, nullptr, dy, d, N, d, L.ln_ff1_g, L.ln_eps, dxb, dx0, d, nullptr, nullptr, lnp + 4 * lnp_set, stream));
     if (side) {
diff --git a/indic_cl_asr_amd/csrc/gemm_tn.hip b/indic_cl_asr_amd/csrc/gemm_tn.hip
--- a/indic_cl_asr_amd/csrc/gemm_tn.hip
+++ b/indic_cl_asr_amd/csrc/gemm_tn.hip
@@ -194,7 +194,7 @@
 constexpr int TN_MAX_GROUP = 12;
 struct TnProblem {
     const __bf16* dY; const __bf16* X; float* part; float* part_b; float* dW; float* db;
-    size_t row_stride; int ldy, ldx, M, n, k, rps, S, tiles, wg_begin; int64_t out_begin;
+    size_t row_stride; int ldy, ldx, M, n, k, rps, S, tiles, wg_begin, acc; int64_t out_begin;
 };
 struct TnGroup { TnProblem p[TN_MAX_GROUP]; int count; };
 
@@ -229,7 +229,16 @@
             a.x += x.x; a.y += x.y; a.z += x.z; a.w += x.w;
         }
         float* dst = off < nk ? P.dW + off : P.db + (off - nk);
-        *reinterpret_cast<float4*>(dst) = a;
+        if ((reinterpret_cast<uintptr_t>(dst) & 15) == 0) {
+            if (P.acc) {
+                const float4 o = *reinterpret_cast<const float4*>(dst);
+                a.x = o.x + a.x; a.y = o.y + a.y; a.z = o.z + a.z; a.w = o.w + a.w;
+            }
+            *reinterpret_cast<float4*>(dst) = a;
+        } else {
+            if (P.acc) { a.x = dst[0] + a.x; a.y = dst[1] + a.y; a.z = dst[2] + a.z; a.w = dst[3] + a.w; }
+            dst[0] = a.x; dst[1] = a.y; dst[2] = a.z; dst[3] = a.w;
+        }
     }
 }
 
@@ -275,13 +284,14 @@
 }
 
 namespace {
-inline int tn_group_plan(const ia_tn_problem* pr, int count, TnGroup* g, int64_t* scratch_elems, int64_t* out_elems, int* blocks) {
+inline int tn_group_plan(const ia_tn_problem_ex* pr, int count, TnGroup* g, int64_t* scratch_elems, int64_t* out_elems, int* blocks) {
     if (!pr || count <= 0 || count > TN_MAX_GROUP) return IA_INVALID_VALUE;
     int tiles_total = 0;
     for (int i = 0; i < count; ++i) {
-        const ia_tn_problem& q = pr[i];
+        const ia_tn_problem_ex& q = pr[i];
         if (q.M <= 0 || q.n <= 0 || q.k <= 0) return IA_INVALID_VALUE;
         if (q.n % 8 != 0 || q.k % 8 != 0 || q.ldy % 8 != 0 || q.ldx % 8 != 0) return IA_UNSUPPORTED;
+        if (q.flags & ~IA_TN_ACCUMULATE) return IA_INVALID_VALUE;
         tiles_total += ((q.n + TN_BN - 1) / TN_BN) * ((q.k + TN_BK - 1) / TN_BK);
     }
     int S0 = 512 / tiles_total;
@@ -290,7 +300,7 @@
     int wg = 0;
     g->count = count;
     for (int i = 0; i < count; ++i) {
-        const ia_tn_problem& q = pr[i];
+        const ia_tn_problem_ex& q = pr[i];
         TnProblem& P = g->p[i];
         const int cap = (q.M + TN_MS - 1) / TN_MS;
         int rps;
@@ -299,7 +309,7 @@
         P.rps = rps; P.S = S; P.tiles = ((q.n + TN_BN - 1) / TN_BN) * ((q.k + TN_BK - 1) / TN_BK);
         P.row_stride = (size_t)q.n * q.k + q.n;
         P.part = nullptr; P.part_b = nullptr;
-        P.dW = q.dW; P.db = q.db;
+        P.dW = q.dW; P.db = q.db; P.acc = (q.flags & IA_TN_ACCUMULATE) ? 1 : 0;
         P.wg_begin = wg; wg += tn_wgs(P.tiles, S);
         P.out_begin = oo; oo += (int64_t)P.row_stride;
         P.part = reinterpret_cast<float*>(so * sizeof(float));
@@ -311,21 +321,45 @@
 }
 }
 
+namespace {
+inline int tn_widen(const ia_tn_problem* pr, int count, ia_tn_problem_ex* ex) {
+    if (!pr || count <= 0 || count > TN_MAX_GROUP) return IA_INVALID_VALUE;
+    for (int i = 0; i < count; ++i)
+        ex[i] = ia_tn_problem_ex{pr[i].dY, pr[i].X, pr[i].dW, pr[i].db, pr[i].ldy, pr[i].ldx, pr[i].M, pr[i].n, pr[i].k, 0};
+    return IA_OK;
+}
+}
+
 extern "C" int64_t ia_gemm_tn_grouped_scratch_elems(const ia_tn_problem* problems, int count) {
+    ia_tn_problem_ex ex[TN_MAX_GROUP];
+    if (tn_widen(problems, count, ex) != IA_OK) return 0;
+    return ia_gemm_tn_grouped_ex_scratch_elems(ex, count);
+}
+
+extern "C" int ia_gemm_tn_bf16_grouped(const ia_tn_problem* problems, int count, float* scratch, ia_stream_t stream) {
+    ia_tn_problem_ex ex[TN_MAX_GROUP];
+    const int rc = tn_widen(problems, count, ex);
+    if (rc != IA_OK) return rc;
+    for (int i = 0; i < count; ++i)
+        if (!ia_is_aligned(ex[i].dW, 16) || (ex[i].db && !ia_is_aligned(ex[i].db, 16))) return IA_INVALID_VALUE;
+    return ia_gemm_tn_bf16_grouped_ex(ex, count, scratch, stream);
+}
+
+extern "C" int64_t ia_gemm_tn_grouped_ex_scratch_elems(const ia_tn_problem_ex* problems, int count) {
     TnGroup g; int64_t so = 0, oo = 0; int blocks = 0;
     if (tn_group_plan(problems, count, &g, &so, &oo, &blocks) != IA_OK) return 0;
     return so;
 }
 
-extern "C" int ia_gemm_tn_bf16_grouped(const ia_tn_problem* problems, int count, float* scratch, ia_stream_t stream) {
+extern "C" int ia_gemm_tn_bf16_grouped_ex(const ia_tn_problem_ex* problems, int count, float* scratch, ia_stream_t stream) {
     if (!scratch) return IA_INVALID_VALUE;
     TnGroup g; int64_t so = 0, oo = 0; int blocks = 0;
     const int rc = tn_group_plan(problems, count, &g, &so, &oo, &blocks);
     if (rc != IA_OK) return rc;
     for (int i = 0; i < count; ++i) {
         TnProblem& P = g.p[i];
-        if (!P.dY || !P.X || !P.dW || !ia_is_aligned(P.dY, 16) || !ia_is_aligned(P.X, 16) || !ia_is_aligned(P.dW, 16) ||
-            (P.db && !ia_is_aligned(P.db, 16)))
+        if (!P.dY || !P.X || !P.dW || !ia_is_aligned(P.dY, 16) || !ia_is_aligned(P.X, 16) || !ia_is_aligned(P.dW, 4) ||
+            (P.db && !ia_is_aligned(P.db, 4)))
             return IA_INVALID_VALUE;
         P.part = scratch + reinterpret_cast<size_t>(P.part) / sizeof(float);
         P.part_b = P.db ? P.part + (size_t)P.n * P.k : nullptr;
diff --git a/indic_cl_asr_amd/ops/block.py b/indic_cl_asr_amd/ops/block.py
--- a/indic_cl_asr_amd/ops/block.py
+++ b/indic_cl_asr_amd/ops/block.py
@@ -262,6 +262,7 @@
 
 USE_NATIVE_BLOCKS = True
 
+_DST_FIELDS = frozenset(n for n, _ in _lib.BlockGradDst._fields_)
 _SAVED_FIELDS = ("y1", "h1p", "h1", "x1", "y2", "qkv", "pl", "ctxv", "x2", "y3", "c2", "z", "sums", "c3", "x3", "y4", "h4p", "h4", "x4", "lse")
 
 
@@ -319,19 +320,43 @@
             (layer.norm_feed_forward2.weight, "ln_ff2_g", 0), (layer.norm_feed_forward2.bias, "ln_ff2_b", 0),
             (layer.norm_out.weight, "ln_out_g", 0), (layer.norm_out.bias, "ln_out_b", 0)]
         self._table_key, self._table = None, None
+        self.dst = _lib.BlockGradDst()
 
     def add_table(self):
         key = tuple((q.grad.data_ptr() if (q.requires_grad and q.grad is not None) else 0) for q, _, _ in self.param_src)
         if key != self._table_key:
             rows = []
             base = self.arena.data_ptr()
+            direct = self._direct_fields(key)
+            self.dst = _lib.BlockGradDst()
             for (q, blk, sub), gp in zip(self.param_src, key):
-                if gp:
+                f = self._dst_field(blk, sub)
+                if gp and f in direct:
+                    setattr(self.dst, f, gp)
+                elif gp:
                     rows.append((gp, base + 4 * (self.off[blk][0] + sub), q.numel()))
             self._table = torch.tensor(rows, dtype=torch.int64).to(self.arena.device) if rows else None
             self._table_key = key
             self._n_rows = len(rows)
         return self._table, (self._n_rows if self._table is not None else 0)
+
+    def _dst_field(self, blk, sub):
+        if blk in ("w_qkv", "b_qkv"):
+            return blk[:2] + "qkv"[sub // (self.d * self.d if blk == "w_qkv" else self.d)]
+        return blk if blk in _DST_FIELDS else None
+
+    def _direct_fields(self, key):
+        import os
+        if os.environ.get("IA_TN_GROUPED", "1")[:1] == "0":
+            return set()
+        ok = {}
+        for (q, blk, sub), gp in zip(self.param_src, key):
+            f = self._dst_field(blk, sub)
+            if f is not None:
+                ok[f] = bool(gp) and q.grad.dtype == torch.float32 and q.grad.is_contiguous() and gp % 4 == 0
+        good = {f for f in ok if ok[f] and ok.get("b" + f[1:], True) and ok.get("w" + f[1:], True)}
+        qkv = {"w_q", "b_q", "w_k", "b_k", "w_v", "b_v"}
+        return good if qkv <= good else good - qkv
 
 
 _RUNTIMES = {}
@@ -406,19 +431,21 @@
         dout = dout.float().contiguous()
         dx2_p, dctx_p = ctypes.c_void_p(), ctypes.c_void_p()
         sp = _lib.stream_ptr()
-        a_args = (ctypes.addressof(bp), ctypes.addressof(saved), ctypes.addressof(rt.grads), _ptr(dout), _ptr(lens), B, T,
+        table, n_rows = rt.add_table() if DIRECT_ACCUMULATE else (None, 0)
+        dst = ctypes.addressof(rt.dst) if DIRECT_ACCUMULATE else None
+        a_args = (ctypes.addressof(bp), ctypes.addressof(saved), ctypes.addressof(rt.grads), dst, _ptr(dout), _ptr(lens), B, T,
                   int(seed) & 0xFFFFFFFF, _ptr(ws), n_ws, ctypes.addressof(dx2_p), ctypes.addressof(dctx_p))
         if ctx.group is None:
-            _lib.check(L.ia_conformer_block_bwd_a(*a_args, sp), "ia_conformer_block_bwd_a")
+            _lib.check(L.ia_conformer_block_bwd_a_acc(*a_args, 0, None, sp), "ia_conformer_block_bwd_a_acc")
         else:
             import torch.distributed as dist
-            _lib.check(L.ia_conformer_block_bwd_a_phase(*a_args, 1, None, sp), "ia_conformer_block_bwd_a_phase")
+            _lib.check(L.ia_conformer_block_bwd_a_acc(*a_args, 1, None, sp), "ia_conformer_block_bwd_a_acc")
             ob, og = rt.off["bn_b"][0], rt.off["bn_g"][0]
             Sg = torch.cat([rt.arena[ob:ob + d], rt.arena[og:og + d], torch.full((1,), float(N), dtype=torch.float32, device=dev)])
             fast.SYNC_BN_COLLECTIVES += 1
             dist.all_reduce(Sg, group=ctx.group)
             Sg = (Sg[:2 * d] * (float(N) / Sg[2 * d])).contiguous()
-            _lib.check(L.ia_conformer_block_bwd_a_phase(*a_args, 2, _ptr(Sg), sp), "ia_conformer_block_bwd_a_phase")
+            _lib.check(L.ia_conformer_block_bwd_a_acc(*a_args, 2, _ptr(Sg), sp), "ia_conformer_block_bwd_a_acc")
         def view(buf, off, shape, dtype):
             n = 1
             for s_ in shape:
@@ -433,11 +460,10 @@
         dqkv, dpl, du, dv = fast.relpos_attention_flash_bwd(qkv, pl, att.pos_bias_u, att.pos_bias_v, lens, ctxv, dctx, lse, B, T, att.h,
                                                             att.d_k, patt, seed + 7, dub_out=(rt.pos_u, rt.pos_v))
         dx0 = torch.empty(N, d, dtype=torch.float32, device=dev)
-        table, n_rows = rt.add_table() if DIRECT_ACCUMULATE else (None, 0)
-        st = L.ia_conformer_block_bwd_b(ctypes.addressof(bp), ctypes.addressof(saved), ctypes.addressof(rt.grads), _ptr(x0), _ptr(pe), pe.shape[0],
-                                        _ptr(dqkv), _ptr(dpl), B, T, int(seed) & 0xFFFFFFFF, _ptr(ws), n_ws, _ptr(dx0), _ptr(table),
-                                        n_rows, sp)
-        _lib.check(st, "ia_conformer_block_bwd_b")
+        st = L.ia_conformer_block_bwd_b_acc(ctypes.addressof(bp), ctypes.addressof(saved), ctypes.addressof(rt.grads), dst, _ptr(x0), _ptr(pe),
+                                            pe.shape[0], _ptr(dqkv), _ptr(dpl), B, T, int(seed) & 0xFFFFFFFF, _ptr(ws), n_ws, _ptr(dx0),
+                                            _ptr(table), n_rows, sp)
+        _lib.check(st, "ia_conformer_block_bwd_b_acc")
         outs = []
         by_id = {id(q): (blk, sub) for q, blk, sub in rt.param_src}
         for r, q in zip(req, params):
diff --git a/indic_cl_asr_amd/ops/fast.py b/indic_cl_asr_amd/ops/fast.py
--- a/indic_cl_asr_amd/ops/fast.py
+++ b/indic_cl_asr_amd/ops/fast.py
@@ -528,23 +528,32 @@
     return dW, db
 
 
-def gemm_tn_grouped(pairs):
+def gemm_tn_grouped(pairs, into=None):
     import ctypes
     L = _lib.lib()
     n_ = len(pairs)
-    arr = (_lib.TnProblem * n_)()
+    arr = (_lib.TnProblemEx * n_)()
     outs = []
     dev = pairs[0][0].device
     for i, (dy, x) in enumerate(pairs):
         M, N = dy.shape
         K = x.shape[1]
-        buf = torch.empty(N * K + N, dtype=torch.float32, device=dev)
-        outs.append((buf[:N * K].view(N, K), buf[N * K:]))
-        arr[i].dY, arr[i].X, arr[i].dW, arr[i].db = dy.data_ptr(), x.data_ptr(), buf.data_ptr(), buf.data_ptr() + 4 * N * K
+        acc = into[i] if into is not None else None
+        if acc is not None:
+            aw, ab = acc
+            assert aw.dtype == ab.dtype == torch.float32 and aw.is_contiguous() and ab.is_contiguous()
+            assert aw.numel() == N * K and ab.numel() == N
+            outs.append(None)
+            arr[i].dW, arr[i].db, arr[i].flags = aw.data_ptr(), ab.data_ptr(), _lib.TN_ACCUMULATE
+        else:
+            buf = torch.empty(N * K + N, dtype=torch.float32, device=dev)
+            outs.append((buf[:N * K].view(N, K), buf[N * K:]))
+            arr[i].dW, arr[i].db = buf.data_ptr(), buf.data_ptr() + 4 * N * K
+        arr[i].dY, arr[i].X = dy.data_ptr(), x.data_ptr()
         arr[i].ldy, arr[i].ldx, arr[i].M, arr[i].n, arr[i].k = dy.stride(0), x.stride(0), M, N, K
-    scr = scratch(dev, L.ia_gemm_tn_grouped_scratch_elems(ctypes.addressof(arr), n_))
-    st = L.ia_gemm_tn_bf16_grouped(ctypes.addressof(arr), n_, _lib.ptr(scr), _lib.stream_ptr())
-    _lib.check(st, "ia_gemm_tn_bf16_grouped")
+    scr = scratch(dev, L.ia_gemm_tn_grouped_ex_scratch_elems(ctypes.addressof(arr), n_))
+    st = L.ia_gemm_tn_bf16_grouped_ex(ctypes.addressof(arr), n_, _lib.ptr(scr), _lib.stream_ptr())
+    _lib.check(st, "ia_gemm_tn_bf16_grouped_ex")
     return outs
 
 
diff --git a/indic_cl_asr_amd/ops/joint.py b/indic_cl_asr_amd/ops/joint.py
--- a/indic_cl_asr_amd/ops/joint.py
+++ b/indic_cl_asr_amd/ops/joint.py
@@ -352,9 +352,13 @@
                 dgin = fast.swap01_cast(dgm, torch.float32 if gdt == torch.float32 else torch.bfloat16).transpose(0, 1).to(gdt)
             else:
                 dgin = dgm.to(gdt)
-        (dWe, dbe), (dWg, dbg) = fast.gemm_tn_grouped([(dfb, xb), (dgb, gb)])
-        plist += [(We, dWe if need[13] else None, 1.0), (be, dbe if need[14] else None, 1.0),
-                  (Wg, dWg if need[15] else None, 1.0), (bg, dbg if need[16] else None, 1.0)]
+        def own(w, b, iw, ib):
+            return need[iw] and need[ib] and w.requires_grad and b.requires_grad and tail._direct(w) and tail._direct(b)
+        into = [(We.grad, be.grad) if own(We, be, 13, 14) else None, (Wg.grad, bg.grad) if own(Wg, bg, 15, 16) else None]
+        res = fast.gemm_tn_grouped([(dfb, xb), (dgb, gb)], into=into)
+        for (w, b, iw, ib), r in zip(((We, be, 13, 14), (Wg, bg, 15, 16)), res):
+            dWp, dbp = r if r is not None else (None, None)
+            plist += [(w, dWp if need[iw] else None, 1.0), (b, dbp if need[ib] else None, 1.0)]
         outs = tail.accumulate_or_return(plist)
         return (dx, dgin) + outs[:2] + (None,) * 9 + outs[2:]
 
```

Measured after the change: 3730 utterances/s (median of 2 runs). Within noise of the previous version (-0.8%).
